# borangundogan/PPO-2DGrid

Measured on AMD Instinct MI355X. Metric: env-steps/sec (rollout+GAE+PPO update), 4096 envs, 16x16 mediumhard, higher is better.
Workload: dtype fp32

## Files before the change

include/merlin_hip.h:

```cpp
#ifndef MERLIN_HIP_H
#define MERLIN_HIP_H

#include <stdint.h>

#ifdef __cplusplus
extern "C" {
#endif

#define MERLIN_ABI_VERSION 3

#define MERLIN_OK 0
#define MERLIN_E_INVALID 1
#define MERLIN_E_HIP 2
#define MERLIN_E_DEVICE 3
#define MERLIN_E_UNSUPPORTED 4

#define MERLIN_EASY 0
#define MERLIN_MEDIUM 1
#define MERLIN_MEDIUMHARD 2
#define MERLIN_HARD 3
#define MERLIN_HARDEST 4

#define MERLIN_DEVERR_BAD_ACTION 1u
#define MERLIN_DEVERR_PLACE_OBJ 2u
#define MERLIN_DEVERR_SLOT_EMPTY 8u
#define MERLIN_DEVERR_BAD_TILE 4u
#define MERLIN_DEVERR_BAD_FRAME 16u

#define MERLIN_LAYOUT_NCHW 0
#define MERLIN_LAYOUT_NHWC 1

#define MERLIN_OBS_WORDS 8
#define MERLIN_OBS_TILES 5
#define MERLIN_TILE_PX 8
#define MERLIN_VIEW 7

typedef struct merlin_env merlin_env;

typedef struct {
    int32_t num_envs;
    int32_t size;
    int32_t difficulty;
    int32_t max_steps;
    int32_t stuck_penalty;
    int32_t max_stay;
    double penalty;
    int32_t exploration_bonus;
    double bonus;
    int32_t reseed_each_reset;
} merlin_env_config;

#define MERLIN_ENV_CONFIG_FIELDS 10
int64_t merlin_env_config_layout(int64_t *offsets_host, int32_t n_fields);

int merlin_version(void);
const char *merlin_last_error(void);
int merlin_tile_atlas(uint8_t *out_host);

int merlin_env_create(const merlin_env_config *cfg, merlin_env **out);
int merlin_env_destroy(merlin_env *env);
int merlin_env_seed(merlin_env *env, const uint64_t *seeds_host, int32_t n, void *stream);
int merlin_env_set_difficulties(merlin_env *env, const int32_t *diff_host, int32_t n, void *stream);
int merlin_env_reset(merlin_env *env, const uint8_t *mask_dev, uint32_t *obs_dev, void *stream);
int merlin_env_step(merlin_env *env, const int64_t *actions_dev, int32_t n_steps,
                    int64_t action_stride, uint32_t *obs_dev, float *reward_dev,
                    uint8_t *terminated_dev, uint8_t *truncated_dev, float *done_dev,
                    double *ep_return_dev, int32_t *ep_length_dev, int32_t autoreset,
                    void *stream);
int merlin_env_act_step(merlin_env *env, const float *head_part_dev, int32_t n_parts, const float *b_actor_dev,
                        const float *b_critic_dev, int32_t act_dim, int32_t deterministic, uint64_t seed,
                        const int64_t *epoch_dev, int64_t step, int64_t env_offset, int64_t *action_dev,
                        float *logp_dev, float *value_dev, uint32_t *obs_dev, float *reward_dev,
                        uint8_t *terminated_dev, uint8_t *truncated_dev, float *done_dev, double *ep_return_dev,
                        int32_t *ep_length_dev, void *stream);
int merlin_group_act(const uint32_t *codes_dev, int32_t groups, const float *T2_dev, const float *b2_dev,
                     const float *W3t_dev, const float *b3_dev, const float *W4p_dev, const float *b4_dev,
                     const float *Wa_dev, const float *ba_dev, const float *Wc_dev, const float *bc_dev,
                     int32_t act_dim, float *a3_ws_dev, float *head_part_dev, int32_t shared_weights, void *stream);
int merlin_env_set_refill_interval(merlin_env *env, int32_t every);
int merlin_env_refill(merlin_env *env, void *stream);
int merlin_env_set_step_fallback(merlin_env *env, int32_t on);
int merlin_env_set_lookahead_depth(merlin_env *env, int32_t depth);
int merlin_env_full_obs(merlin_env *env, uint8_t *out_dev, void *stream);
int merlin_env_get_state(merlin_env *env, uint32_t *walls_host, int32_t *agent_host,
                         uint64_t *rng_host, void *stream);
#define MERLIN_FRAME_TILES 22
int merlin_frame_atlas(int32_t tile_size, uint8_t *out_host);
int merlin_render_frames(const uint32_t *walls_dev, const int32_t *goal_dev, const int32_t *agent_dev,
                         const int32_t *map_index_dev, int64_t n_frames, int32_t size, int32_t tile_size,
                         int32_t highlight, uint8_t *out_dev, void *stream);
int merlin_env_render(merlin_env *env, const int64_t *index_dev, int64_t n, int32_t tile_size,
                      int32_t highlight, uint8_t *out_dev, void *stream);
int merlin_env_snapshot(merlin_env *env, uint32_t *walls_dev, int32_t *goal_dev, int32_t *agent_dev,
                        void *stream);
int merlin_shortest_paths(const uint32_t *walls_dev, const int32_t *goal_dev, const int32_t *agent_dev,
                          const int32_t *map_index_dev, int64_t n, int32_t size, int32_t *dist_dev,
                          int16_t *field_dev, void *stream);
int merlin_env_optimal_steps(merlin_env *env, int32_t *dist_dev, int16_t *field_dev, void *stream);
int merlin_shortest_paths_host(const uint32_t *walls, const int32_t *goal, const int32_t *agent, int64_t n,
                               int32_t size, int32_t *dist, int16_t *field);
int merlin_view_codes(const uint32_t *walls_dev, const int32_t *goal_dev, const int32_t *agent_dev,
                      const int32_t *map_index_dev, int64_t n, int32_t size, uint32_t *codes_dev, void *stream);
int merlin_policy_paths(const uint32_t *walls_dev, const int32_t *goal_dev, const int8_t *action_dev,
                        int64_t n_maps, int32_t size, int16_t *steps_dev, void *stream);
int merlin_policy_paths_host(const uint32_t *walls, const int32_t *goal, const int8_t *action, int64_t n_maps,
                             int32_t size, int16_t *steps);
int merlin_policy_chain(const uint32_t *walls_dev, const int32_t *goal_dev, const float *probs_dev, int64_t n_maps,
                        int32_t size, int32_t horizon, double gamma, double *success_dev, double *ret_dev,
                        double *steps_dev, double *disc_dev, void *stream);
int merlin_policy_occupancy(const uint32_t *walls_dev, const int32_t *goal_dev, const float *probs_dev,
                            const int32_t *agent_dev, int64_t n_maps, int32_t size, int32_t horizon,
                            double *visits_dev, double *hit_dev, void *stream);
int merlin_policy_chain_host(const uint32_t *walls, const int32_t *goal, const float *probs, int64_t n_maps,
                             int32_t size, int32_t horizon, double gamma, double *success, double *ret,
                             double *steps, double *disc);
int merlin_policy_occupancy_host(const uint32_t *walls, const int32_t *goal, const float *probs,
                                 const int32_t *agent, int64_t n_maps, int32_t size, int32_t horizon,
                                 double *visits, double *hit);
int merlin_env_errors(merlin_env *env, uint32_t *flags_host, uint32_t *fallbacks_host,
                      void *stream);
int merlin_env_num_envs(const merlin_env *env);
int merlin_env_size(const merlin_env *env);

int merlin_obs_expand_f32(const uint32_t *codes_dev, const int64_t *index_dev, int64_t n,
                          float *out_dev, float scale, int32_t layout, void *stream);
int merlin_obs_expand_u8(const uint32_t *codes_dev, const int64_t *index_dev, int64_t n,
                         uint8_t *out_dev, void *stream);

int merlin_gae(const float *reward_dev, const float *value_dev, const float *done_dev,
               const float *last_value_dev, float *adv_dev, float *ret_dev, int32_t T, int32_t N,
               double gamma, double lam, double *stats_dev, void *stream);
int merlin_adv_normalize(const float *adv_dev, int64_t n, const double *stats_dev, float *out_dev,
                         void *stream);

int merlin_conv1_lut_fwd(const uint32_t *codes_dev, const int64_t *index_dev, int64_t n,
                         const float *tables_dev, const float *bias_dev, int32_t towers,
                         float *out_dev, void *stream);
int merlin_conv1_lut_bwd(const uint32_t *codes_dev, const int64_t *index_dev, int64_t n,
                         const float *act_dev, const float *grad_dev, int32_t towers,
                         float *dtables_dev, float *dbias_dev, void *stream);

int merlin_tower_conv2_im2col_fwd(const uint32_t *codes_dev, const int64_t *index_dev, int64_t n,
                                  const float *tables_dev, const float *bias_dev, int32_t towers,
                                  float *A2_dev, void *stream);
int merlin_tower_conv2_im2col_bwd(const uint32_t *codes_dev, const int64_t *index_dev, int64_t n,
                                  const float *tables_dev, const float *bias_dev,
                                  const float *dA2_dev, int32_t towers, float *dtables_dev,
                                  float *dbias_dev, void *stream);
int merlin_tower_conv3_im2col_fwd(const float *Z2_dev, const float *b2_dev, int64_t n,
                                  int32_t towers, float *A3_dev, void *stream);
int merlin_tower_conv3_col2im_bwd(const float *dA3_dev, const float *Z2_dev, const float *b2_dev,
                                  int64_t n, int32_t towers, float *dZ2_dev, void *stream);
int merlin_tower_conv3_col2im_bwd_chunked(const float *dA3_dev, const float *Z2_dev,
                                          const float *b2_dev, int64_t n, int32_t towers,
                                          float *dZ2c_dev, uint32_t *absmax_dev, void *stream);

int merlin_tower_conv2_lut_rows(void);
int merlin_tower_conv2_lut_fwd(const uint32_t *codes_dev, const int64_t *index_dev, int64_t n,
                               const float *tables_dev, int32_t towers, float *Z2_dev,
                               void *stream);
int merlin_tower_conv2_lut_bwd(const uint32_t *codes_dev, int64_t n, const float *dZ2c_dev,
                               const uint32_t *absmax_dev, int32_t towers, float *dtables_dev,
                               void *stream);
int merlin_tower_conv2_lut_fwd_grouped(const uint32_t *codes_dev, int64_t n, int64_t group_frames,
                                       const float *tables_dev, int32_t towers, float *Z2_dev, void *stream);
int64_t merlin_tower_conv2_lut_slab_bytes(int32_t towers, int64_t group_frames);
int merlin_tower_conv2_lut_bwd_grouped(const uint32_t *codes_dev, int64_t group_frames, const float *dZ2c_dev,
                                       const uint32_t *absmax_dev, int32_t towers, float *dtables_dev,
                                       void *slabs_dev, void *stream);

int merlin_tower_window_lut(const int32_t *rows_dev, int64_t n_windows, const float *tables_dev,
                            int32_t towers, float *Z2w_dev, void *stream);
int merlin_minibatch_patch_maps(const int32_t *kid_dev, const int64_t *group_keys_dev, int64_t n_groups,
                                int64_t n_frames, const int64_t *group_offsets_dev, int32_t n_patches, int32_t *kmap_dev,
                                int32_t *rmap_dev, int32_t *rep_row_dev, void *stream);
int merlin_tower_window_lut_bias_relu(const int32_t *rows_dev, int64_t n_windows, const float *tables_dev,
                                      int32_t towers, const float *b2_dev, float *a2w_dev, void *stream);
int merlin_tower_window_conv3(const float *Q_dev, int64_t n_windows, const int32_t *wid_dev,
                              const int64_t *groups_dev, int64_t n, const float *b3_dev,
                              int32_t towers, float *Y3_dev, void *stream);
int64_t merlin_tower_all_windows(void);
int merlin_tower_codes_conv3(const uint32_t *codes_dev, int64_t n, const float *Qall_dev,
                             const float *b3_dev, int32_t towers, float *Y3_dev, void *stream);
int merlin_tower_codes_conv3_amax(const uint32_t *codes_dev, int64_t n, const float *Qall_dev,
                                  const float *b3_dev, int32_t towers, float *Y3_dev, uint32_t *amax_dev,
                                  void *stream);
int merlin_tower_errors(uint32_t *flags, void *stream);
int merlin_tower_window_conv3_bits(const float *Q_dev, int64_t n_windows, const int32_t *wid_dev,
                                   const int64_t *groups_dev, int64_t n, const float *b3_dev,
                                   int32_t towers, float *Y3_dev, uint64_t *relu_bits_dev, uint32_t *amax_dev,
                                   void *stream);
int merlin_tower_window_conv3_reuse(const float *Q_dev, int64_t n_windows, const int32_t *wid_dev,
                                    const int64_t *groups_dev, int64_t n, const float *b3_dev,
                                    int32_t towers, float *Y3_dev, uint64_t *relu_bits_dev, uint32_t *amax_dev,
                                    const int32_t *rep_row_dev, int32_t copy, void *stream);
int merlin_tower_window_conv3_planes(const float *Q_dev, int64_t nw, const int32_t *wid_dev, const int64_t *groups_dev,
                                     int64_t n, const float *b3_dev, int32_t towers, void *Y3_planes_dev,
                                     uint64_t *relu_bits_dev, const int32_t *rep_row_dev, uint32_t *colmax_ws_dev,
                                     uint32_t *bound_dev, void *stream);
int merlin_segment_sum(const float *src_dev, int64_t src_rows, const int32_t *idx_dev,
                       const int32_t *key_dev, int64_t nnz, const int32_t *slot_dev, int32_t sub,
                       int64_t item_len, const int32_t *fix_dev, int64_t n_fix, int32_t towers,
                       float *out_dev, int64_t out_rows, float *carry_dev, int32_t accumulate,
                       void *stream);
#define MERLIN_SEG_ACCUMULATE 1
#define MERLIN_SEG_NO_FILL 2
#define MERLIN_SEG_MASK_BITS 4
#define MERLIN_SEG_ROLE_SHIFT 8
#define MERLIN_SEG_ROLE_MASK (7 << MERLIN_SEG_ROLE_SHIFT)
int merlin_segment_sum_masked(const float *src_dev, const void *mask_dev, int64_t src_rows,
                              const int32_t *idx_dev, const int32_t *key_dev, int64_t nnz,
                              const int32_t *slot_dev, int32_t sub, int64_t item_len,
                              const int32_t *fix_dev, int64_t n_fix, int32_t towers, float *out_dev,
                              int64_t out_rows, float *carry_dev, int32_t flags, void *stream);
int merlin_segment_sum_marked(const float *src_dev, const void *mask_dev, int64_t src_rows,
                              const int32_t *idx_dev, const int32_t *key_dev, int64_t nnz,
                              const int32_t *slot_dev, int32_t sub, int64_t item_len,
                              const int32_t *fix_dev, int64_t n_fix, int32_t towers, float *out_dev,
                              int64_t out_rows, float *carry_dev, int32_t flags, int32_t *mark_dev,
                              void *stream);
int merlin_segment_sum_fused(const float *src_dev, const void *mask_dev, int64_t src_rows,
                             const int32_t *idx_dev, const int32_t *key_dev, int64_t nnz,
                             const int32_t *slot_dev, int32_t sub, int64_t item_len,
                             const int32_t *fix_dev, int64_t n_fix, int32_t towers, float *out_dev,
                             int64_t out_rows, float *carry_dev, int32_t flags, int32_t *mark_dev,
                             const int32_t *head_fix_dev, int32_t *counters_dev, void *stream);
int merlin_segment_sum_mask_rows(const float *src_dev, const void *mask_dev, int64_t src_rows, const int32_t *idx_dev,
                                 const int32_t *key_dev, int64_t nnz, const int32_t *slot_dev, int32_t sub,
                                 int64_t item_len, const int32_t *fix_dev, int64_t n_fix, int32_t towers, float *out_dev,
                                 int64_t out_rows, float *carry_dev, int32_t flags, int32_t *mark_dev,
                                 const int32_t *head_fix_dev, int32_t *counters_dev, const int32_t *mask_rows_dev,
                                 void *stream);

int merlin_act_heads(const float *z_dev, const float *b4_dev, int64_t n, int32_t hidden,
                     const float *w_actor_dev, const float *b_actor_dev, const float *w_critic_dev,
                     const float *b_critic_dev, int32_t act_dim, int32_t deterministic, uint64_t seed,
                     const int64_t *epoch_dev, int64_t step, int64_t env_offset, int64_t *action_dev,
                     float *logp_dev,
                     float *value_dev, void *stream);

int64_t merlin_ppo_loss_workspace(int64_t n_samples);
int merlin_ppo_loss(const float *logits_dev, const float *value_dev, const float *bias_actor_dev,
                    const float *bias_critic_dev, int64_t n_frames, int32_t act_dim, const int32_t *offs_dev,
                    const int32_t *order_dev, const int64_t *frame_of_dev, int64_t n_samples,
                    const int64_t *sample_index_dev, const int64_t *actions_dev, const float *logp_old_dev,
                    const float *adv_dev, const float *ret_dev, double clip_eps, double vf_coef, double ent_coef,
                    float *dlogits_dev, float *dvalue_dev, float *dbias_actor_dev, float *dbias_critic_dev,
                    float *loss_dev, double *stats_dev, double *workspace_dev, void *stream);
int merlin_ppo_loss_absmax(const float *logits_dev, const float *value_dev, const float *bias_actor_dev,
                           const float *bias_critic_dev, int64_t n_frames, int32_t act_dim, const int32_t *offs_dev,
                           const int32_t *order_dev, const int64_t *frame_of_dev, int64_t n_samples,
                           const int64_t *sample_index_dev, const int64_t *actions_dev, const float *logp_old_dev,
                           const float *adv_dev, const float *ret_dev, double clip_eps, double vf_coef,
                           double ent_coef, float *dlogits_dev, float *dvalue_dev, float *dbias_actor_dev,
                           float *dbias_critic_dev, float *loss_dev, double *stats_dev, double *workspace_dev,
                           uint32_t *grad_absmax_dev, void *stream);

int merlin_tower_bias_relu(float *z_dev, const float *bias_dev, int64_t rows, int32_t cols, int32_t towers,
                           void *stream);
int merlin_tower_relu_bwd(const float *y_dev, const float *dy_dev, float *dz_dev, int64_t rows, int32_t cols,
                          int32_t towers, float *dbias_dev, void *stream);
int merlin_tower_colsum(const float *x_dev, int64_t rows, int32_t cols, int64_t row_stride, int64_t tower_stride,
                        int32_t towers, float *out_dev, void *stream);
int merlin_tower_head_bwd(const float *h_dev, const float *dlogits_dev, const float *dvalue_dev,
                          const float *w_actor_dev, const float *w_critic_dev, int64_t n, int32_t hidden,
                          int32_t act_dim, float *dz_dev, float *dbias_dev, float *dw_actor_dev,
                          float *dw_critic_dev, uint32_t *amax_dev, void *stream);
int merlin_tower_head_bwd_planes(const float *h_dev, const float *dlogits_dev, const float *dvalue_dev,
                                 const float *w_actor_dev, const float *w_critic_dev, int64_t n, int32_t hidden,
                                 int32_t act_dim, void *dz_planes_dev, float *dbias_dev, float *dw_actor_dev,
                                 float *dw_critic_dev, const uint32_t *grad_absmax_dev, uint32_t *dz_bound_dev,
                                 void *stream);
int merlin_tower_heads_fwd(const float *h_dev, int64_t n, int32_t hidden, const float *w_actor_dev,
                           int32_t act_dim, const float *w_critic_dev, const float *b_actor_dev,
                           const float *b_critic_dev, float *logits_dev, float *value_dev, void *stream);

int merlin_x6_split(const float *x_dev, int64_t n, void *planes_dev, void *stream);
int merlin_x6_join(const void *planes_dev, int64_t n, float *x_dev, void *stream);
int merlin_x6_gemm_nt(const float *A_dev, const void *B_dev, int64_t M, int32_t N, int32_t K, int32_t towers,
                      int64_t a_stride, int64_t b_stride, const float *bias_dev, float *C_dev, int64_t c_stride,
                      int32_t cfg, void *stream);
int64_t merlin_x6_tn_slab_floats(int32_t M, int32_t N, int32_t towers, int32_t splits);
int merlin_x6_gemm_tn(const float *A_dev, const float *B_dev, int64_t Kd, int32_t M, int32_t N, int32_t towers,
                      int64_t a_stride, int64_t b_stride, int32_t splits, float *slab_dev, float *out_dev, int32_t cfg,
                      void *stream);

int merlin_h3_amax(const float *x_dev, int64_t n, int32_t towers, int64_t stride, uint32_t *amax_dev, void *stream);
int merlin_h3_split(const float *x_dev, int64_t n, int32_t towers, const uint32_t *amax_dev, void *planes_dev,
                    void *stream);
int merlin_h3_gemm_nt(const float *A_dev, const uint32_t *amax_a_dev, const void *B_dev, const uint32_t *amax_b_dev,
                      int64_t M, int32_t N, int32_t K, int32_t towers, int64_t a_stride, int64_t b_stride,
                      const float *bias_dev, float *C_dev, int64_t c_stride, void *a_planes_dev, int32_t cfg,
                      void *stream);
int merlin_h3_gemm_tn(const float *A_dev, const uint32_t *amax_a_dev, const float *B_dev, const uint32_t *amax_b_dev,
                      int64_t Kd, int32_t M, int32_t N, int32_t towers, int64_t a_stride, int64_t b_stride,
                      int32_t splits, float *slab_dev, float *out_dev, int32_t cfg, void *stream);
int merlin_h3_gemm_tn_planes(const void *A_planes_dev, const uint32_t *amax_a_dev, const void *B_planes_dev,
                             const uint32_t *amax_b_dev, int64_t Kd, int32_t M, int32_t N, int32_t towers,
                             int64_t a_stride, int64_t b_stride, int32_t splits, float *slab_dev, float *out_dev,
                             int32_t cfg, void *stream);
int merlin_h3_gemm_nt_gather(const float *A_dev, const uint32_t *amax_a_dev, const void *B_dev,
                             const uint32_t *amax_b_dev, int64_t M, int32_t N, int32_t K, int32_t towers,
                             int64_t a_stride, int64_t b_stride, const float *bias_dev, float *C_dev, int64_t c_stride,
                             const int32_t *a_rows_dev, int32_t cfg, void *stream);
int merlin_h3_gemm_nt_heads(const float *A_dev, const uint32_t *amax_a_dev, const void *B_dev,
                            const uint32_t *amax_b_dev, int64_t M, int32_t N, int32_t K, int64_t a_stride,
                            int64_t b_stride, const float *bias_dev, float *C_dev, int64_t c_stride,
                            const int32_t *a_rows_dev, const float *head_w0_dev, int32_t n_actions,
                            const float *head_w1_dev, float *head_partials_dev, int32_t cfg, void *stream);
int32_t merlin_h3_heads_parts(int32_t N, int32_t cfg);
int merlin_h3_walk_blocks(int32_t blocks);
int merlin_h3_gemm_nt_planes(const void *A_planes_dev, const uint32_t *amax_a_dev, const void *B_dev,
                             const uint32_t *amax_b_dev, int64_t M, int32_t N, int32_t K, int32_t towers,
                             int64_t a_stride, int64_t b_stride, const float *bias_dev, float *C_dev, int64_t c_stride,
                             int32_t cfg, void *stream);
int merlin_h3_gemm_nt_heads_planes(const void *A_planes_dev, const uint32_t *amax_a_dev, const void *B_dev,
                                   const uint32_t *amax_b_dev, int64_t M, int32_t N, int32_t K, int64_t a_stride,
                                   int64_t b_stride, const float *bias_dev, float *C_dev, int64_t c_stride,
                                   const int32_t *a_rows_dev, const float *head_w0_dev, int32_t n_actions,
                                   const float *head_w1_dev, float *head_partials_dev, int32_t cfg, void *stream);
int merlin_h3_gemm_tn_gather_planes(const void *A_planes_dev, const uint32_t *amax_a_dev, const void *B_planes_dev,
                                    const uint32_t *amax_b_dev, int64_t Kd, int32_t M, int32_t N, int32_t towers,
                                    int64_t a_stride, int64_t b_stride, int32_t splits, float *slab_dev,
                                    float *out_dev, const int32_t *b_rows_dev, int32_t cfg, void *stream);
int merlin_h3_gemm_tn_gather_planes_a(const void *A_planes_dev, const uint32_t *amax_a_dev, const float *B_dev,
                                      const uint32_t *amax_b_dev, int64_t Kd, int32_t M, int32_t N, int32_t towers,
                                      int64_t a_stride, int64_t b_stride, int32_t splits, float *slab_dev,
                                      float *out_dev, const int32_t *b_rows_dev, int32_t cfg, void *stream);
// ... 73 lines not shown
```

ppo-2dgrid_amd/csrc/merlin_capi.hip:

```cpp
#include <math.h>
#include <string.h>

#include <mutex>
#include <string>
#include <vector>

#include <algorithm>

#include "merlin_internal.h"

struct merlin_env {
    merlin::EnvDev dev;
    int device;
    bool has_state;
    int steps_since_refill;
    int refill_every;
    bool no_fallback = false;
    bool seed_slots_full = false;
    uint8_t *diff_buf = nullptr;
    int32_t *level_log = nullptr;
};

namespace {

// ... 928 lines not shown
    return MERLIN_OK;
}

int merlin_gae(const float *rew, const float *val, const float *done, const float *last, float *adv,
               float *ret, int32_t T, int32_t N, double gamma, double lam, double *stats, void *stream) {
    if (!rew || !val || !done || !last || !adv || !ret) return fail(MERLIN_E_INVALID, "null argument");
    if (T <= 0 || N <= 0) return fail(MERLIN_E_INVALID, "T and N must be > 0");
    DeviceWs *ws = nullptr;
    int rc = device_ws(&ws);
    if (rc) return rc;
    if (stats && merlin::gae_partials_needed(T, N) > ws->max_partials)
        return fail(MERLIN_E_UNSUPPORTED, "too many envs for the GAE stats workspace");
    HIP_TRY(merlin::launch_gae(rew, val, done, last, adv, ret, T, N, gamma, lam, stats, ws->partials,
                               ws->max_partials, (hipStream_t)stream));
    return MERLIN_OK;
}

int merlin_adv_normalize(const float *adv, int64_t n, const double *stats, float *out, void *stream) {
    if (!adv || !stats || !out) return fail(MERLIN_E_INVALID, "null argument");
    HIP_TRY(merlin::launch_adv_normalize(adv, n, stats, out, (hipStream_t)stream));
    return MERLIN_OK;
}

int merlin_conv1_lut_fwd(const uint32_t *codes, const int64_t *index, int64_t n, const float *tables,
                         const float *bias, int32_t towers, float *out, void *stream) {
    if ((!codes || !tables || !bias || !out) && n > 0) return fail(MERLIN_E_INVALID, "null argument");
    if (towers < 1 || towers > 2) return fail(MERLIN_E_INVALID, "towers must be 1 or 2");
    HIP_TRY(merlin::launch_conv1_lut_fwd(codes, index, n, tables, bias, towers, out, (hipStream_t)stream));
    return MERLIN_OK;
}

int merlin_conv1_lut_bwd(const uint32_t *codes, const int64_t *index, int64_t n, const float *act,
                         const float *grad, int32_t towers, float *dtables, float *dbias, void *stream) {
    if (!dtables || !dbias || ((!codes || !act || !grad) && n > 0)) return fail(MERLIN_E_INVALID, "null argument");
    if (towers < 1 || towers > 2) return fail(MERLIN_E_INVALID, "towers must be 1 or 2");
    DeviceWs *ws = nullptr;
    int rc = device_ws(&ws);
    if (rc) return rc;
    HIP_TRY(merlin::launch_conv1_lut_bwd(codes, index, n, act, grad, towers, dtables, dbias, ws->conv1_slabs,
                                         ws->max_slabs, (hipStream_t)stream));
    return MERLIN_OK;
}

int merlin_tower_conv2_im2col_fwd(const uint32_t *codes, const int64_t *index, int64_t n, const float *tables,
                                  const float *bias, int32_t towers, float *A2, void *stream) {
    if ((!codes || !tables || !bias || !A2) && n > 0) return fail(MERLIN_E_INVALID, "null argument");
    if (towers < 1 || towers > 2) return fail(MERLIN_E_INVALID, "towers must be 1 or 2");
    HIP_TRY(merlin::launch_conv1_im2col_fwd(codes, index, n, tables, bias, towers, A2, (hipStream_t)stream));
    return MERLIN_OK;
}

int merlin_tower_conv2_im2col_bwd(const uint32_t *codes, const int64_t *index, int64_t n, const float *tables,
                                  const float *bias, const float *dA2, int32_t towers, float *dtables,
                                  float *dbias, void *stream) {
    if (!dtables || !dbias || ((!codes || !tables || !bias || !dA2) && n > 0))
        return fail(MERLIN_E_INVALID, "null argument");
    if (towers < 1 || towers > 2) return fail(MERLIN_E_INVALID, "towers must be 1 or 2");
    DeviceWs *ws = nullptr;
    int rc = device_ws(&ws);
    if (rc) return rc;
    HIP_TRY(merlin::launch_conv1_im2col_bwd(codes, index, n, tables, bias, dA2, towers, dtables, dbias,
                                            ws->conv1_slabs, ws->max_slabs, (hipStream_t)stream));
    return MERLIN_OK;
}

int merlin_tower_conv3_im2col_fwd(const float *Z2, const float *b2, int64_t n, int32_t towers, float *A3,
                                  void *stream) {
    if ((!Z2 || !b2 || !A3) && n > 0) return fail(MERLIN_E_INVALID, "null argument");
    HIP_TRY(merlin::launch_im2col3_fwd(Z2, b2, n, towers, A3, (hipStream_t)stream));
    return MERLIN_OK;
}

int merlin_tower_conv3_col2im_bwd(const float *dA3, const float *Z2, const float *b2, int64_t n, int32_t towers,
                                  float *dZ2, void *stream) {
    if ((!dA3 || !Z2 || !b2 || !dZ2) && n > 0) return fail(MERLIN_E_INVALID, "null argument");
    HIP_TRY(merlin::launch_col2im3_bwd(dA3, Z2, b2, n, towers, 0, dZ2, nullptr, (hipStream_t)stream));
    return MERLIN_OK;
}

int merlin_tower_conv3_col2im_bwd_chunked(const float *dA3, const float *Z2, const float *b2, int64_t n,
                                          int32_t towers, float *dZ2c, uint32_t *absmax, void *stream) {
    if (!absmax || ((!dA3 || !Z2 || !b2 || !dZ2c) && n > 0)) return fail(MERLIN_E_INVALID, "null argument");
    if (towers < 1) return fail(MERLIN_E_INVALID, "towers must be >= 1");
    HIP_TRY(merlin::launch_col2im3_bwd(dA3, Z2, b2, n, towers, 1, dZ2c, absmax, (hipStream_t)stream));
    return MERLIN_OK;
}

int merlin_tower_conv2_lut_rows(void) { return merlin::conv2_lut_rows(); }

int merlin_tower_conv2_lut_fwd(const uint32_t *codes, const int64_t *index, int64_t n, const float *tables,
                               int32_t towers, float *Z2, void *stream) {
    if ((!codes || !tables || !Z2) && n > 0) return fail(MERLIN_E_INVALID, "null argument");
    if (towers < 1 || towers > 2) return fail(MERLIN_E_INVALID, "towers must be 1 or 2");
    HIP_TRY(merlin::launch_conv2_lut_fwd(codes, index, n, tables, towers, Z2, (hipStream_t)stream));
    return MERLIN_OK;
}

int merlin_tower_conv2_lut_bwd(const uint32_t *codes, int64_t n, const float *dZ2c, const uint32_t *absmax,
                               int32_t towers, float *dtables, void *stream) {
    if (!dtables || ((!codes || !dZ2c || !absmax) && n > 0)) return fail(MERLIN_E_INVALID, "null argument");
    if (towers < 1 || towers > 2) return fail(MERLIN_E_INVALID, "towers must be 1 or 2");
    DeviceWs *ws = nullptr;
    int rc = device_ws(&ws);
    if (rc) return rc;
    HIP_TRY(merlin::launch_conv2_lut_bwd(codes, n, dZ2c, absmax, towers, dtables, ws->lut2_slabs,
                                         (hipStream_t)stream));
    return MERLIN_OK;
}

int merlin_tower_conv2_lut_fwd_grouped(const uint32_t *codes, int64_t n, int64_t group_frames, const float *tables,
                                       int32_t towers, float *Z2, void *stream) {
    if ((!codes || !tables || !Z2) && n > 0) return fail(MERLIN_E_INVALID, "null argument");
    if (towers < 2 || towers % 2 || group_frames <= 0) return fail(MERLIN_E_INVALID, "bad grouping");
    if (n != (int64_t)(towers / 2) * group_frames) return fail(MERLIN_E_INVALID, "n != groups * group_frames");
    HIP_TRY(merlin::launch_conv2_lut_fwd(codes, nullptr, n, tables, towers, Z2, (hipStream_t)stream, group_frames));
    return MERLIN_OK;
}

int64_t merlin_tower_conv2_lut_slab_bytes(int32_t towers, int64_t group_frames) {
    return (int64_t)merlin::conv2_lut_slab_bytes(towers, merlin::conv2_lut_fblocks(group_frames));
}

int merlin_tower_conv2_lut_bwd_grouped(const uint32_t *codes, int64_t group_frames, const float *dZ2c,
                                       const uint32_t *absmax, int32_t towers, float *dtables, void *slabs,
                                       void *stream) {
    if (!dtables || ((!codes || !dZ2c || !absmax || !slabs) && group_frames > 0))
        return fail(MERLIN_E_INVALID, "null argument");
    if (towers < 2 || towers % 2) return fail(MERLIN_E_INVALID, "bad grouping");
    HIP_TRY(merlin::launch_conv2_lut_bwd(codes, group_frames, dZ2c, absmax, towers, dtables, slabs,
                                         (hipStream_t)stream, group_frames));
    return MERLIN_OK;
}

int merlin_tower_window_lut(const int32_t *rows, int64_t nw, const float *tables, int32_t towers, float *Z2w,
                            void *stream) {
    if ((!rows || !tables || !Z2w) && nw > 0) return fail(MERLIN_E_INVALID, "null argument");
    if (towers < 1 || towers > 2) return fail(MERLIN_E_INVALID, "towers must be 1 or 2");
    HIP_TRY(merlin::launch_window_lut(rows, nw, tables, towers, Z2w, (hipStream_t)stream));
    return MERLIN_OK;
}

int merlin_minibatch_patch_maps(const int32_t *kid, const int64_t *group_keys, int64_t n_groups, int64_t n_frames,
                                const int64_t *group_offsets, int32_t n_patches, int32_t *kmap, int32_t *rmap,
                                int32_t *rep_row, void *stream) {
    if (n_groups < 0 || n_frames < 1 || n_patches < 1) return fail(MERLIN_E_INVALID, "bad shape");
    if (n_groups > 0 && (!kid || !group_keys || !group_offsets || !kmap || !rmap || !rep_row))
        return fail(MERLIN_E_INVALID, "null argument");
    if (n_groups * 9 > INT32_MAX) return fail(MERLIN_E_UNSUPPORTED, "more than 2^31 rows");
    HIP_TRY(merlin::launch_patch_maps(kid, group_keys, n_groups, n_frames, group_offsets, n_patches, kmap, rmap,
                                      rep_row, (hipStream_t)stream));
    return MERLIN_OK;
}

int merlin_tower_window_lut_bias_relu(const int32_t *rows, int64_t nw, const float *tables, int32_t towers,
                                      const float *b2, float *a2w, void *stream) {
    if ((!rows || !tables || !a2w || !b2) && nw > 0) return fail(MERLIN_E_INVALID, "null argument");
    if (towers < 1 || towers > 2) return fail(MERLIN_E_INVALID, "towers must be 1 or 2");
    HIP_TRY(merlin::launch_window_lut(rows, nw, tables, towers, a2w, (hipStream_t)stream, b2));
    return MERLIN_OK;
}

int merlin_tower_window_conv3(const float *Q, int64_t nw, const int32_t *wid, const int64_t *groups, int64_t n,
                              const float *b3, int32_t towers, float *Y3, void *stream) {
    if ((!Q || !wid || !b3 || !Y3) && n > 0) return fail(MERLIN_E_INVALID, "null argument");
    if (towers < 1 || towers > 2) return fail(MERLIN_E_INVALID, "towers must be 1 or 2");
    HIP_TRY(merlin::launch_window_conv3(Q, nw, wid, groups, n, b3, towers, Y3, nullptr, nullptr, nullptr, 0,
                                        (hipStream_t)stream));
    return MERLIN_OK;
}

int merlin_tower_window_conv3_bits(const float *Q, int64_t nw, const int32_t *wid, const int64_t *groups, int64_t n,
                                   const float *b3, int32_t towers, float *Y3, uint64_t *relu_bits, uint32_t *amax,
                                   void *stream) {
    if ((!Q || !wid || !b3 || !Y3 || !relu_bits) && n > 0) return fail(MERLIN_E_INVALID, "null argument");
    if (towers < 1 || towers > 2) return fail(MERLIN_E_INVALID, "towers must be 1 or 2");
    HIP_TRY(merlin::launch_window_conv3(Q, nw, wid, groups, n, b3, towers, Y3, relu_bits, amax, nullptr, 0,
                                        (hipStream_t)stream));
    return MERLIN_OK;
}

int merlin_tower_window_conv3_reuse(const float *Q, int64_t nw, const int32_t *wid, const int64_t *groups, int64_t n,
                                    const float *b3, int32_t towers, float *Y3, uint64_t *relu_bits, uint32_t *amax,
                                    const int32_t *rep_row, int32_t copy, void *stream) {
    if ((!rep_row || !Y3 || (!(copy & 4) && (!Q || !wid || !b3))) && n > 0)
        return fail(MERLIN_E_INVALID, "null argument");
    if (towers < 1 || towers > 2) return fail(MERLIN_E_INVALID, "towers must be 1 or 2");
    if (copy < 0 || copy > 7) return fail(MERLIN_E_INVALID, "copy must be 0..7");
    HIP_TRY(merlin::launch_window_conv3(Q, nw, wid, groups, n, b3, towers, Y3, relu_bits, amax, rep_row, copy,
                                        (hipStream_t)stream));
    return MERLIN_OK;
}

int merlin_tower_window_conv3_planes(const float *Q, int64_t nw, const int32_t *wid, const int64_t *groups, int64_t n,
                                     const float *b3, int32_t towers, void *Y3_planes, uint64_t *relu_bits,
                                     const int32_t *rep_row, uint32_t *colmax_ws, uint32_t *bound, void *stream) {
    if ((!rep_row || !Y3_planes || !Q || !wid || !b3 || !relu_bits || !colmax_ws || !bound) && n > 0)
        return fail(MERLIN_E_INVALID, "null argument");
    if (towers < 1 || towers > 2) return fail(MERLIN_E_INVALID, "towers must be 1 or 2");
    if (n > 0 && nw <= 0) return fail(MERLIN_E_INVALID, "no windows");
    HIP_TRY(merlin::launch_window_conv3(Q, nw, wid, groups, n, b3, towers, static_cast<float *>(Y3_planes), relu_bits,
                                        nullptr, rep_row, 0, (hipStream_t)stream, colmax_ws, bound));
    return MERLIN_OK;
}

int64_t merlin_tower_all_windows(void) { return 458752; }

int merlin_tower_codes_conv3_amax(const uint32_t *codes, int64_t n, const float *Qall, const float *b3,
                                  int32_t towers, float *Y3, uint32_t *amax, void *stream) {
    if ((!codes || !Qall || !b3 || !Y3) && n > 0) return fail(MERLIN_E_INVALID, "null argument");
    if (towers < 1 || towers > 2) return fail(MERLIN_E_INVALID, "towers must be 1 or 2");
    DeviceWs *ws = nullptr;
    if (int r = device_ws(&ws)) return r;
    HIP_TRY(merlin::launch_codes_conv3(codes, n, Qall, b3, towers, Y3, amax, ws->tower_err, (hipStream_t)stream));
    return MERLIN_OK;
}

int merlin_tower_errors(uint32_t *flags, void *stream) {
    DeviceWs *ws = nullptr;
    if (int r = device_ws(&ws)) return r;
    hipStream_t s = (hipStream_t)stream;
    uint32_t h = 0;
    HIP_TRY(hipMemcpyAsync(&h, ws->tower_err, sizeof(h), hipMemcpyDeviceToHost, s));
    HIP_TRY(hipStreamSynchronize(s));
    HIP_TRY(merlin::zero_async(ws->tower_err, sizeof(h), s));
    if (flags) *flags = h;
    return MERLIN_OK;
}

int merlin_tower_codes_conv3(const uint32_t *codes, int64_t n, const float *Qall, const float *b3, int32_t towers,
                             float *Y3, void *stream) {
    return merlin_tower_codes_conv3_amax(codes, n, Qall, b3, towers, Y3, nullptr, stream);
}

static int segment_sum_fused(const float *src, const void *mask, int64_t src_rows, const int32_t *idx,
                             const int32_t *key, int64_t nnz, const int32_t *slot, int32_t sub, int64_t item_len,
                             const int32_t *fix, int64_t n_fix, int32_t towers, float *out, int64_t out_rows,
                             float *carry, int32_t flags, int32_t *mark, const int32_t *head_fix, int32_t *counters,
                             const int32_t *mask_rows, void *stream) {
    if (!out && out_rows > 0) return fail(MERLIN_E_INVALID, "null output");
    if (nnz > 0 && (!src || !idx || !key || !carry)) return fail(MERLIN_E_INVALID, "null argument");
    if (n_fix > 0 && !fix) return fail(MERLIN_E_INVALID, "null fix-up list");
    if ((head_fix == nullptr) != (counters == nullptr)) return fail(MERLIN_E_INVALID, "head_fix and counters go together");
    if (counters && nnz > 0 && n_fix != (nnz + item_len - 1) / item_len)
        return fail(MERLIN_E_INVALID, "in-launch fix-ups need one fix row per item");
    if (towers < 1 || towers > 2) return fail(MERLIN_E_INVALID, "towers must be 1 or 2");
    if (item_len <= 0 || sub <= 0) return fail(MERLIN_E_INVALID, "item_len and sub must be > 0");
    if (flags & ~(MERLIN_SEG_ACCUMULATE | MERLIN_SEG_NO_FILL | MERLIN_SEG_MASK_BITS | MERLIN_SEG_ROLE_MASK))
        return fail(MERLIN_E_INVALID, "unknown flags");
    HIP_TRY(merlin::launch_seg_sum(src, mask, (flags & MERLIN_SEG_MASK_BITS) ? 1 : 0, src_rows, idx, key, nnz, slot,
                                   sub, item_len, fix, n_fix, towers, out, out_rows, carry,
                                   (flags & MERLIN_SEG_ACCUMULATE) ? 1 : 0, (flags & MERLIN_SEG_NO_FILL) ? 0 : 1,
                                   (flags & MERLIN_SEG_ROLE_MASK) >> MERLIN_SEG_ROLE_SHIFT, mark, head_fix, counters,
                                   (hipStream_t)stream, mask_rows));
    return MERLIN_OK;
}

int merlin_segment_sum_fused(const float *src, const void *mask, int64_t src_rows, const int32_t *idx,
                             const int32_t *key, int64_t nnz, const int32_t *slot, int32_t sub, int64_t item_len,
                             const int32_t *fix, int64_t n_fix, int32_t towers, float *out, int64_t out_rows,
                             float *carry, int32_t flags, int32_t *mark, const int32_t *head_fix, int32_t *counters,
                             void *stream) {
    return segment_sum_fused(src, mask, src_rows, idx, key, nnz, slot, sub, item_len, fix, n_fix, towers, out,
                             out_rows, carry, flags, mark, head_fix, counters, nullptr, stream);
}

int merlin_segment_sum_mask_rows(const float *src, const void *mask, int64_t src_rows, const int32_t *idx,
                                 const int32_t *key, int64_t nnz, const int32_t *slot, int32_t sub, int64_t item_len,
                                 const int32_t *fix, int64_t n_fix, int32_t towers, float *out, int64_t out_rows,
                                 float *carry, int32_t flags, int32_t *mark, const int32_t *head_fix,
                                 int32_t *counters, const int32_t *mask_rows, void *stream) {
    if (nnz > 0 && (!mask || !mask_rows || !(flags & MERLIN_SEG_MASK_BITS)))
        return fail(MERLIN_E_INVALID, "mask_rows needs MERLIN_SEG_MASK_BITS words");
    return segment_sum_fused(src, mask, src_rows, idx, key, nnz, slot, sub, item_len, fix, n_fix, towers, out,
                             out_rows, carry, flags, mark, head_fix, counters, mask_rows, stream);
}

int merlin_segment_sum_marked(const float *src, const void *mask, int64_t src_rows, const int32_t *idx,
                              const int32_t *key, int64_t nnz, const int32_t *slot, int32_t sub, int64_t item_len,
                              const int32_t *fix, int64_t n_fix, int32_t towers, float *out, int64_t out_rows,
                              float *carry, int32_t flags, int32_t *mark, void *stream) {
    return merlin_segment_sum_fused(src, mask, src_rows, idx, key, nnz, slot, sub, item_len, fix, n_fix, towers, out,
                                    out_rows, carry, flags, mark, nullptr, nullptr, stream);
}

int merlin_segment_sum_masked(const float *src, const void *mask, int64_t src_rows, const int32_t *idx,
                              const int32_t *key, int64_t nnz, const int32_t *slot, int32_t sub, int64_t item_len,
                              const int32_t *fix, int64_t n_fix, int32_t towers, float *out, int64_t out_rows,
                              float *carry, int32_t flags, void *stream) {
    return merlin_segment_sum_marked(src, mask, src_rows, idx, key, nnz, slot, sub, item_len, fix, n_fix, towers, out,
                                     out_rows, carry, flags, nullptr, stream);
}

int merlin_segment_sum(const float *src, int64_t src_rows, const int32_t *idx, const int32_t *key, int64_t nnz,
                       const int32_t *slot, int32_t sub, int64_t item_len, const int32_t *fix, int64_t n_fix,
                       int32_t towers, float *out, int64_t out_rows, float *carry, int32_t accumulate,
                       void *stream) {
    return merlin_segment_sum_masked(src, nullptr, src_rows, idx, key, nnz, slot, sub, item_len, fix, n_fix, towers,
                                     out, out_rows, carry, accumulate ? MERLIN_SEG_ACCUMULATE : 0, stream);
}

int merlin_act_heads(const float *z, const float *b4, int64_t n, int32_t hidden, const float *w_actor,
                     const float *b_actor, const float *w_critic, const float *b_critic, int32_t act_dim,
                     int32_t deterministic, uint64_t seed, const int64_t *epoch, int64_t step, int64_t env_offset,
                     int64_t *action, float *logp, float *value, void *stream) {
    if (n < 0) return fail(MERLIN_E_INVALID, "negative size");
    if (act_dim < 1 || act_dim > 8) return fail(MERLIN_E_INVALID, "act_dim must be in [1, 8]");
// ... 540 lines not shown
```

ppo-2dgrid_amd/csrc/merlin_internal.h:

```cpp
#pragma once

#include <hip/hip_runtime.h>
#include <stdint.h>

#include "merlin_hip.h"

namespace merlin {

struct EnvDev {
    int n, size, sp, difficulty, max_steps;
    int stuck_on, max_stay;
    double penalty;
    int explore_on;
    double bonus;
    int reseed;
    uint32_t *walls;
    uint4 *agent;
    ulonglong2 *rng_s;
    ulonglong2 *rng_i;
    uint2 *rng_b;
    double *ep_ret;
    int32_t *ep_len;
    uint32_t *visited;
    uint32_t *err;
// ... 179 lines not shown
        ty = ay - 3;
    } else {
        tx = ax - 3;
        ty = ay - 6;
    }
    const uint64_t hi_ones = ~0ULL << (S + 8);
    uint32_t win[7];
#pragma unroll
    for (int r = 0; r < 7; r++) {
        const int y = ty + r;
        const bool in = (y >= 0) && (y < S);
        const uint32_t bits = in ? row(in ? y : 0) : 0xffffffffu;
        const uint64_t w = ((uint64_t)bits << 8) | 0xffULL | hi_ones;
        win[r] = (uint32_t)(w >> (tx + 8)) & 0x7fu;
    }
    uint32_t tr[7];
#pragma unroll
    for (int x = 0; x < 7; x++) {
        uint32_t v = 0u;
#pragma unroll
        for (int y = 0; y < 7; y++) v |= ((win[y] >> x) & 1u) << y;
        tr[x] = v;
    }
    const int k = (dir + 1) & 3;
    const bool odd = k & 1, flip = (k == 1) || (k == 2), rev = (k >= 2);
#pragma unroll
    for (int b = 0; b < 7; b++) {
        uint32_t t = flip ? (odd ? tr[6 - b] : win[6 - b]) : (odd ? tr[b] : win[b]);
        V[b] = rev ? bitrev7(t) : t;
    }
#pragma unroll
    for (int j = 0; j < 7; j++) m[j] = 0u;
    m[6] = 1u << 3;
#pragma unroll
    for (int j = 6; j >= 0; j--) {
        const uint32_t T = ~V[j] & 0x7fu;
        uint32_t M = m[j];
#pragma unroll
        for (int s = 0; s < 6; s++) M |= (M & T & 0x3fu) << 1;
        const uint32_t e1 = M & T & 0x3fu;
#pragma unroll
        for (int s = 0; s < 6; s++) M |= (M & T & 0x7eu) >> 1;
        const uint32_t e2 = M & T & 0x7eu;
        m[j] = M;
        if (j > 0) m[j - 1] |= e1 | (e1 << 1) | e2 | (e2 >> 1);
    }
}

struct StepOut {
    const int64_t *actions;
    int64_t action_stride;
    int n_steps;
    int autoreset;
    uint32_t *obs;
    float *reward;
    uint8_t *term;
    uint8_t *trunc;
    float *done;
    double *ep_ret_out;
    int32_t *ep_len_out;
    ActIn act;
    int no_fallback;
    int32_t *level_log;
};

hipError_t zero_async(void *p, size_t bytes, hipStream_t s);
hipError_t launch_group_act(const uint32_t *codes, int G, const float *T2, const float *b2, const float *W3t,
                            const float *b3, const float *W4p, const float *b4, const float *Wa, const float *ba,
                            const float *Wc, const float *bc, int A, float *a3, float *part, bool shared, hipStream_t s);
hipError_t launch_h3p_gemm_nt(const void *A, const uint32_t *amaxA, const void *B, const uint32_t *amaxB, int64_t M,
                              int N, int K, int T, int64_t a_stride, int64_t b_stride, const float *bias, float *C,
                              int64_t c_stride, int cfg, hipStream_t s, const int32_t *a_rows = nullptr,
                              const float *head_w0 = nullptr, int n_actions = 0, const float *head_w1 = nullptr,
                              float *head_part = nullptr);
void set_h3p_walk_blocks(int n);
hipError_t launch_h3p_gemm_tn_gather(const void *A, const uint32_t *amaxA, const void *B, const uint32_t *amaxB,
                                     int64_t Kd, int M, int N, int T, int64_t a_stride, int64_t b_stride, int splits,
                                     float *slab, const int32_t *b_rows, int cfg, int *S_out, hipStream_t s);
hipError_t launch_env_reset(const EnvDev &E, const uint8_t *mask, uint32_t *obs, bool refill, hipStream_t s);
hipError_t launch_env_step(const EnvDev &E, const StepOut &O, bool refill, hipStream_t s);
hipError_t launch_env_full_obs(const EnvDev &E, uint8_t *out, hipStream_t s);
hipError_t launch_env_refill(const EnvDev &E, bool full, hipStream_t s);
hipError_t launch_level_bind(const EnvDev &E, const uint32_t *walls, const int32_t *goal, const int32_t *agent,
                             hipStream_t s);
hipError_t launch_env_levels(const EnvDev &E, int32_t *cur, uint32_t *count, hipStream_t s);
hipError_t launch_level_scores(const float *adv, const int32_t *level, int T, int N, int L, int kind, int64_t *sum,
                               int64_t *count, int accumulate, hipStream_t s);
void level_scores_host(const float *adv, const int32_t *level, int T, int N, int L, int kind, int64_t *sum,
                       int64_t *count, int accumulate);
hipError_t upload_atlas(const uint8_t *atlas_host);
hipError_t launch_render_frames(const uint32_t *walls, const int32_t *goal, const int32_t *agent,
                                const int32_t *map_index, int64_t n_frames, int size, int ts, int highlight,
                                const uint8_t *atlas, uint8_t *out, uint32_t *err, hipStream_t s);
hipError_t launch_env_render(const EnvDev &E, const int64_t *index, int64_t n_frames, int ts, int highlight,
                             const uint8_t *atlas, uint8_t *out, hipStream_t s);
hipError_t launch_env_snapshot(const EnvDev &E, uint32_t *walls, int32_t *goal, int32_t *agent, hipStream_t s);
hipError_t launch_shortest_paths(const uint32_t *walls, const int32_t *goal, const int32_t *agent,
                                 const int32_t *map_index, int64_t n, int size, int32_t *dist, int16_t *field,
                                 hipStream_t s);
hipError_t launch_env_optimal_steps(const EnvDev &E, int32_t *dist, int16_t *field, hipStream_t s);
void shortest_paths_host(const uint32_t *walls, const int32_t *goal, const int32_t *agent, int64_t n, int S,
                         int32_t *dist, int16_t *field);
hipError_t launch_view_codes(const uint32_t *walls, const int32_t *goal, const int32_t *agent,
                             const int32_t *map_index, int64_t n, int size, uint32_t *codes, uint32_t *err,
                             hipStream_t s);
hipError_t launch_policy_paths(const uint32_t *walls, const int32_t *goal, const int8_t *action, int64_t n_maps,
                               int size, int16_t *steps, hipStream_t s);
void policy_paths_host(const uint32_t *walls, const int32_t *goal, const int8_t *action, int64_t n_maps, int S,
                       int16_t *steps);
hipError_t launch_policy_chain(const uint32_t *walls, const int32_t *goal, const float *probs, int64_t n_maps, int size,
                               int horizon, double gamma, double *success, double *ret, double *steps, double *disc,
                               hipStream_t s);
hipError_t launch_policy_occupancy(const uint32_t *walls, const int32_t *goal, const float *probs,
                                   const int32_t *agent, int64_t n_maps, int size, int horizon, double *visits,
                                   double *hit, uint32_t *err, hipStream_t s);
void policy_chain_host(const uint32_t *walls, const int32_t *goal, const float *probs, int64_t n_maps, int S, int T,
                       double gamma, double *success, double *ret, double *steps, double *disc);
void policy_occupancy_host(const uint32_t *walls, const int32_t *goal, const float *probs, const int32_t *agent,
                           int64_t n_maps, int S, int T, double *visits, double *hit);
hipError_t launch_obs_expand_f32(const uint32_t *codes, const int64_t *index, int64_t n, float *out,
                                 float scale, int layout, hipStream_t s);
hipError_t launch_obs_expand_u8(const uint32_t *codes, const int64_t *index, int64_t n, uint8_t *out,
                                hipStream_t s);
hipError_t launch_gae(const float *rew, const float *val, const float *done, const float *last,
                      float *adv, float *ret, int T, int N, double gamma, double lam, double *stats,
                      double *partials, int max_partials, hipStream_t s);
hipError_t launch_adv_normalize(const float *adv, int64_t n, const double *stats, float *out,
                                hipStream_t s);
int gae_partials_needed(int T, int N);
int conv1_slab_floats(int towers);
hipError_t launch_conv1_lut_fwd(const uint32_t *codes, const int64_t *index, int64_t n, const float *tables,
                                const float *bias, int towers, float *out, hipStream_t s);
hipError_t launch_conv1_lut_bwd(const uint32_t *codes, const int64_t *index, int64_t n, const float *act,
                                const float *grad, int towers, float *dtables, float *dbias, float *slabs,
                                int max_slabs, hipStream_t s);
hipError_t launch_conv1_im2col_fwd(const uint32_t *codes, const int64_t *index, int64_t n, const float *tables,
                                   const float *bias, int T, float *A2, hipStream_t s);
hipError_t launch_conv1_im2col_bwd(const uint32_t *codes, const int64_t *index, int64_t n, const float *tables,
                                   const float *bias, const float *dA2, int T, float *dtables, float *dbias,
                                   float *slabs, int max_slabs, hipStream_t s);
hipError_t launch_im2col3_fwd(const float *Z2, const float *b2, int64_t n, int T, float *A3, hipStream_t s);
hipError_t launch_col2im3_bwd(const float *dA3, const float *Z2, const float *b2, int64_t n, int T, int chunked,
                              float *dZ2, uint32_t *absmax, hipStream_t s);
int conv2_lut_rows();
int conv2_lut_fblocks(int64_t n);
size_t conv2_lut_slab_bytes(int towers, int fblocks);
hipError_t launch_conv2_lut_fwd(const uint32_t *codes, const int64_t *index, int64_t n, const float *tables,
                                int towers, float *Z2, hipStream_t s, int64_t gstride = 0);
hipError_t launch_conv2_lut_bwd(const uint32_t *codes, int64_t n, const float *dZ2c, const uint32_t *absmax,
                                int towers, float *dT, void *slabs, hipStream_t s, int64_t gstride = 0);

hipError_t launch_patch_maps(const int32_t *kid, const int64_t *gkey, int64_t G, int64_t F, const int64_t *goff, int K,
                             int32_t *kmap, int32_t *rmap, int32_t *rep_row, hipStream_t s);
hipError_t launch_window_lut(const int32_t *rows, int64_t nw, const float *tab, int T, float *Z2w, hipStream_t s,
                             const float *b2 = nullptr);
hipError_t launch_window_conv3(const float *Q, int64_t nw, const int32_t *wid, const int64_t *groups, int64_t n,
                               const float *b3, int T, float *Y3, uint64_t *bits, uint32_t *amax,
                               const int32_t *rrow, int copy, hipStream_t s, uint32_t *colmax = nullptr,
                               uint32_t *bound = nullptr);
hipError_t launch_act_heads(const float *z, const float *b4, int64_t n, int H, const float *wa, const float *ba,
                            const float *wc, const float *bc, int A, int det, uint64_t seed, const int64_t *epoch,
                            int64_t step, int64_t env_offset, int64_t *action, float *logp, float *value,
                            hipStream_t s);
hipError_t launch_act_draw(const float *part, int P, int64_t n, const float *ba, const float *bc, int A, int det,
                           uint64_t seed, const int64_t *epoch, int64_t step, int64_t env_offset, int64_t *action,
                           float *logp, float *value, hipStream_t s);
int64_t ppo_loss_workspace_doubles(int64_t n_samples);
hipError_t launch_ppo_loss(const float *logits, const float *value, const float *bias_a, const float *bias_c,
                           int64_t U, int A, const int32_t *offs, const int32_t *order, const int64_t *inv, int64_t n,
                           const int64_t *sample_index, const int64_t *actions, const float *lp_old, const float *adv,
                           const float *ret, double clip_eps, double vf_coef, double ent_coef, float *dlogits,
                           float *dvalue, float *dbias_a, float *dbias_c, float *loss, double *stats,
                           double *workspace, hipStream_t s, uint32_t *dmax = nullptr);
hipError_t launch_codes_conv3(const uint32_t *codes, int64_t n, const float *Q, const float *b3, int T, float *Y3,
                              uint32_t *amax, uint32_t *err, hipStream_t s);
hipError_t launch_x6_gemm_nt32(const float *A, const void *B, int64_t M, int N, int K, int T, int64_t a_stride,
                               int64_t b_stride, const float *bias, float *C, int64_t c_stride, int cfg, hipStream_t s);
hipError_t launch_x6_gemm_tn32(const float *A, const float *B, int64_t Kd, int M, int N, int T, int64_t a_stride,
                               int64_t b_stride, int splits, float *slab, int cfg, hipStream_t s, int *S_out);
hipError_t launch_stage_fwd(const float *W1, const float *b1, const float *W2, const float *atlas, const int16_t *idx,
                            int T, float *HT, float *T2, hipStream_t s);
hipError_t launch_stage_bwd(const float *W2, const float *HT, const float *dT2, const float *atlas,
                            const int16_t *koff, const int16_t *kv, int T, float *dH, float *dW1, float *db1,
                            float *dW2, double *ws, hipStream_t s);
hipError_t launch_stage_fwd_planes(const float *W1, const float *b1, const float *W2, const float *atlas,
                                   const int16_t *idx, int T, float *HT, float *T2, const float *x0, const float *x1,
                                   int64_t n, const uint32_t *amax, void *planes0, void *planes1, hipStream_t s);
hipError_t launch_stage_bwd_scatter(const float *W2, const float *HT, const float *dT2, const float *atlas,
                                    const int16_t *koff, const int16_t *kv, int T, float *dH, float *DG, int64_t w1,
                                    int64_t b1, int64_t w2, const int32_t *map, int64_t n, float *flat, double *ws,
                                    hipStream_t s);
hipError_t launch_stage_gather(const float *src, const int32_t *map, int64_t n, float *dst, hipStream_t s);
int64_t winbwd_work_floats(int T, int64_t nw);
hipError_t launch_winbwd(const float *a2w, const float *dQ, const float *W3r, int T, int64_t nw, float *da2w,
                         float *db2, float *dW3r, float *work, hipStream_t s, float *db3 = nullptr);
hipError_t launch_winfwd(const float *a2w, const float *W3r, int T, int64_t nw, float *Q, hipStream_t s);
constexpr size_t STAGE_WS_DOUBLES = 2 * 4 * 10 * 2048;
hipError_t launch_heads_fwd(const float *h, int64_t n, int H, const float *wa, int A, const float *wc, const float *ba,
                            const float *bc, float *logits, float *value, hipStream_t s);
hipError_t launch_seg_sum(const float *src, const void *mask, int mask_bits, int64_t src_rows, const int32_t *idx,
                          const int32_t *key, int64_t nnz, const int32_t *slot, int S, int64_t L, const int32_t *fix,
                          int64_t nfix, int T, float *out, int64_t out_rows, float *carry, int acc_out, int fill, int role,
                          int32_t *mark, const int32_t *hfix, int32_t *cnt, hipStream_t s,
                          const int32_t *mrow = nullptr);

constexpr int EPI_MAX_BLOCKS = 512;
size_t epilogue_work_floats();
bool epilogue_cols_ok(int cols);
int epilogue_max_act();
hipError_t launch_bias_relu(float *Z, const float *b, int64_t rows, int cols, int T, hipStream_t s);
hipError_t launch_relu_bwd_colsum(const float *Y, const float *dY, float *dZ, int64_t rows, int cols, int T,
                                  float *dbias, float *work, hipStream_t s);
hipError_t launch_colsum(const float *X, int64_t rows, int cols, int64_t row_stride, int64_t tower_stride, int T,
                         float *out, float *work, hipStream_t s);
hipError_t launch_head_bwd(const float *h, const float *dlogits, const float *dvalue, const float *wa,
                           const float *wc, int64_t n, int H, int A, float *dz, float *db4, float *dwa, float *dwc,
                           float *work, uint32_t *amax, hipStream_t s, const uint32_t *dmax = nullptr,
                           void *dz_planes = nullptr);

__device__ __forceinline__ void block_amax2(const uint32_t mx[2], int T, uint32_t *amax) {
    __shared__ uint32_t red[2][4];
    uint32_t m0 = mx[0], m1 = mx[1];
    for (int o = 32; o > 0; o >>= 1) {
        m0 = max(m0, (uint32_t)__shfl_xor((int)m0, o));
        m1 = max(m1, (uint32_t)__shfl_xor((int)m1, o));
    }
    if ((threadIdx.x & 63) == 0) {
        red[0][threadIdx.x >> 6] = m0;
        red[1][threadIdx.x >> 6] = m1;
    }
    __syncthreads();
    if (threadIdx.x < (unsigned)T) {
        const uint32_t *r = red[threadIdx.x];
        const uint32_t m = max(max(r[0], r[1]), max(r[2], r[3]));
        if (m && m > __hip_atomic_load(amax + threadIdx.x, __ATOMIC_RELAXED, __HIP_MEMORY_SCOPE_AGENT))
            atomicMax(amax + threadIdx.x, m);
    }
}

constexpr float H3_LO_SCALE = 2048.0f, H3_LO_INV = 1.0f / H3_LO_SCALE;
__device__ __forceinline__ int h3_exp(uint32_t amax) {
    if (amax == 0u) return 0;
    const int e = (int)((amax >> 23) & 0xffu) - 127;
    return min(max(14 - e, -120), 115);
}
__device__ __forceinline__ float pow2f(int e) { return __uint_as_float((uint32_t)(e + 127) << 23); }
__device__ __forceinline__ uint32_t load_amax(const uint32_t *p) {
    return __hip_atomic_load(p, __ATOMIC_RELAXED, __HIP_MEMORY_SCOPE_AGENT);
}
__device__ __forceinline__ int xcd_tile(int b, int nb) {
    const int xcd = b & 7, q = nb >> 3, r = nb & 7;
    return (xcd < r ? xcd * (q + 1) : r * (q + 1) + (xcd - r) * q) + (b >> 3);
}

__device__ __forceinline__ void h3_pair(float a, float b, float sc, float sc2, uint32_t &hi, uint32_t &lo) {
    const float m2048 = -H3_LO_SCALE, za = a * sc2, zb = b * sc2;
    uint32_t h, l;
    asm("v_fma_mixlo_f16 %0, %1, %2, 0" : "=v"(h) : "v"(a), "v"(sc));
    asm("v_fma_mixhi_f16 %0, %1, %2, 0" : "+v"(h) : "v"(b), "v"(sc));
    asm("v_fma_mixlo_f16 %0, %1, %2, %3 op_sel_hi:[1,0,0]" : "=v"(l) : "v"(h), "v"(m2048), "v"(za));
    asm("v_fma_mixhi_f16 %0, %1, %2, %3 op_sel:[1,0,0] op_sel_hi:[1,0,0]" : "+v"(l) : "v"(h), "v"(m2048), "v"(zb));
    hi = h;
    lo = l;
}

__device__ __forceinline__ void h3_store4(uint2 *__restrict__ row, int q, const float4 v, float sc, float sc2) {
    uint32_t h0, h1, l0, l1;
    h3_pair(v.x, v.y, sc, sc2, h0, l0);
    h3_pair(v.z, v.w, sc, sc2, h1, l1);
    const int o = 4 * (q >> 1) + (q & 1);
    row[o] = make_uint2(h0, h1);
    row[o + 2] = make_uint2(l0, l1);
}

__device__ __forceinline__ void h3_store4_pair(uint4 *__restrict__ row, int q, const float4 v, float sc, float sc2) {
    uint32_t h0, h1, l0, l1;
    h3_pair(v.x, v.y, sc, sc2, h0, l0);
    h3_pair(v.z, v.w, sc, sc2, h1, l1);
    const bool odd = q & 1;
    const uint32_t r0 = (uint32_t)__shfl_xor((int)(odd ? h0 : l0), 1);
    const uint32_t r1 = (uint32_t)__shfl_xor((int)(odd ? h1 : l1), 1);
    row[q] = odd ? make_uint4(r0, r1, l0, l1) : make_uint4(h0, h1, r0, r1);
}

hipError_t launch_x6_split(const float *x, int64_t n, void *planes, hipStream_t s);
hipError_t launch_x6_join(const void *planes, int64_t n, float *x, hipStream_t s);
hipError_t launch_x6_gemm_nt(const float *A, const void *B, int64_t M, int N, int K, int T, int64_t a_stride,
                             int64_t b_stride, const float *bias, float *C, int64_t c_stride, int cfg, hipStream_t s);
hipError_t launch_x6_gemm_tn(const float *A, const float *B, int64_t Kd, int M, int N, int T, int64_t a_stride,
                             int64_t b_stride, int splits, float *slab, float *out, int cfg, hipStream_t s);
int x6_tn_max_splits();
hipError_t launch_x6_fold(const float *slab, int S, int64_t total, float *out, hipStream_t s);
hipError_t launch_h3_amax(const float *x, int64_t n, int T, int64_t stride, uint32_t *amax, hipStream_t s);
hipError_t launch_h3_split(const float *x, int64_t n, int T, const uint32_t *amax, void *planes, hipStream_t s);
hipError_t launch_h3_gemm_nt(const float *A, const uint32_t *amaxA, const void *B, const uint32_t *amaxB, int64_t M,
                             int N, int K, int T, int64_t a_stride, int64_t b_stride, const float *bias, float *C,
                             int64_t c_stride, void *a_planes, int cfg, hipStream_t s,
                             const int32_t *a_rows = nullptr, const float *head_w0 = nullptr, int n_actions = 0,
                             const float *head_w1 = nullptr, float *head_part = nullptr, bool a_is_planes = false);
int h3_heads_parts(int N, int cfg);
hipError_t launch_heads_combine(const float *part, int P, int64_t M, int na, float *logits, float *value,
                                hipStream_t s);
hipError_t launch_h3_gemm_tn(const void *A, const uint32_t *amaxA, const void *B, const uint32_t *amaxB, int64_t Kd,
                             int M, int N, int T, int64_t a_stride, int64_t b_stride, int splits, float *slab,
                             float *out, bool planes, int cfg, hipStream_t s, const int32_t *b_rows = nullptr,
                             bool a_planes = false, bool b_planes = false);
// ... 33 lines not shown
```

ppo-2dgrid_amd/merlin/_native.py:

```python
from __future__ import annotations

import contextlib
import ctypes as C
import gc
import os

import torch

PKG_ROOT = os.path.dirname(os.path.dirname(os.path.abspath(__file__)))
LIB_PATH = os.environ.get("MERLIN_HIP_LIB", os.path.join(PKG_ROOT, "lib", "libmerlin_hip.so"))

MERLIN_OK = 0
E_INVALID, E_HIP, E_DEVICE, E_UNSUPPORTED = 1, 2, 3, 4
LAYOUT_NCHW = 0
LAYOUT_NHWC = 1
OBS_WORDS = 8
DEVERR_BAD_ACTION = 1
DEVERR_PLACE_OBJ = 2
DEVERR_BAD_TILE = 4
DEVERR_SLOT_EMPTY = 8
DEVERR_BAD_FRAME = 16
FRAME_TILES = 22

DIFFICULTY_IDS = {"easy": 0, "medium": 1, "mediumhard": 2, "hard": 3, "hardest": 4}


class MerlinNativeError(RuntimeError):
    code = None


class EnvConfig(C.Structure):
    _fields_ = [
        ("num_envs", C.c_int32),
        ("size", C.c_int32),
        ("difficulty", C.c_int32),
        ("max_steps", C.c_int32),
        ("stuck_penalty", C.c_int32),
        ("max_stay", C.c_int32),
        ("penalty", C.c_double),
        ("exploration_bonus", C.c_int32),
        ("bonus", C.c_double),
        ("reseed_each_reset", C.c_int32),
    ]


_lib = None
ABI_VERSION = 3


def lib():
    global _lib
    if _lib is not None:
        return _lib
    if not os.path.exists(LIB_PATH):
        raise MerlinNativeError(
            f"HIP library not found at {LIB_PATH}; build it with "
            f"`make -C {PKG_ROOT}` (hipcc --offload-arch=gfx950)")
    try:
        L = C.CDLL(LIB_PATH)
    except OSError as e:
        raise MerlinNativeError(f"failed to load {LIB_PATH}: {e}") from e
    vp, i32, i64, u64p = C.c_void_p, C.c_int32, C.c_int64, C.POINTER(C.c_uint64)
    L.merlin_version.restype = C.c_int
    if L.merlin_version() != ABI_VERSION:
        raise MerlinNativeError(f"{LIB_PATH} has ABI version {L.merlin_version()}, this package binds version "
                                f"{ABI_VERSION} (include/merlin_hip.h MERLIN_ABI_VERSION); rebuild it")
    L.merlin_last_error.restype = C.c_char_p
    L.merlin_tile_atlas.argtypes = [vp]
    L.merlin_env_config_layout.argtypes = [C.POINTER(C.c_int64), i32]
    L.merlin_env_config_layout.restype = i64
    L.merlin_env_create.argtypes = [C.POINTER(EnvConfig), C.POINTER(vp)]
    L.merlin_env_destroy.argtypes = [vp]
    L.merlin_env_seed.argtypes = [vp, u64p, i32, vp]
    L.merlin_env_set_difficulties.argtypes = [vp, C.POINTER(C.c_int32), i32, vp]
    L.merlin_env_reset.argtypes = [vp, vp, vp, vp]
    L.merlin_env_step.argtypes = [vp, vp, i32, i64, vp, vp, vp, vp, vp, vp, vp, i32, vp]
    L.merlin_group_act.argtypes = [vp, i32, vp, vp, vp, vp, vp, vp, vp, vp, vp, vp, i32, vp, vp, i32, vp]
    L.merlin_env_act_step.argtypes = [vp, vp, i32, vp, vp, i32, i32, C.c_uint64, vp, i64, i64, vp, vp, vp, vp, vp,
                                      vp, vp, vp, vp, vp, vp]
    L.merlin_env_set_refill_interval.argtypes = [vp, i32]
    L.merlin_env_set_step_fallback.argtypes = [vp, i32]
    L.merlin_env_refill.argtypes = [vp, vp]
    L.merlin_env_set_lookahead_depth.argtypes = [vp, i32]
    L.merlin_env_get_state.argtypes = [vp, vp, vp, vp, vp]
    L.merlin_env_full_obs.argtypes = [vp, vp, vp]
    L.merlin_env_errors.argtypes = [vp, C.POINTER(C.c_uint32), C.POINTER(C.c_uint32), vp]
    L.merlin_obs_expand_f32.argtypes = [vp, vp, i64, vp, C.c_float, i32, vp]
    L.merlin_obs_expand_u8.argtypes = [vp, vp, i64, vp, vp]
    L.merlin_gae.argtypes = [vp, vp, vp, vp, vp, vp, i32, i32, C.c_double, C.c_double, vp, vp]
    L.merlin_adv_normalize.argtypes = [vp, i64, vp, vp, vp]
    L.merlin_conv1_lut_fwd.argtypes = [vp, vp, i64, vp, vp, i32, vp, vp]
    L.merlin_conv1_lut_bwd.argtypes = [vp, vp, i64, vp, vp, i32, vp, vp, vp]
    L.merlin_tower_conv2_im2col_fwd.argtypes = [vp, vp, i64, vp, vp, i32, vp, vp]
    L.merlin_tower_conv2_im2col_bwd.argtypes = [vp, vp, i64, vp, vp, vp, i32, vp, vp, vp]
    L.merlin_tower_conv3_im2col_fwd.argtypes = [vp, vp, i64, i32, vp, vp]
    L.merlin_tower_conv3_col2im_bwd.argtypes = [vp, vp, vp, i64, i32, vp, vp]
    L.merlin_tower_conv3_col2im_bwd_chunked.argtypes = [vp, vp, vp, i64, i32, vp, vp, vp]
    L.merlin_tower_conv2_lut_rows.restype = C.c_int
    L.merlin_tower_conv2_lut_fwd.argtypes = [vp, vp, i64, vp, i32, vp, vp]
    L.merlin_tower_conv2_lut_bwd.argtypes = [vp, i64, vp, vp, i32, vp, vp]
    L.merlin_tower_conv2_lut_fwd_grouped.argtypes = [vp, i64, i64, vp, i32, vp, vp]
    L.merlin_tower_conv2_lut_slab_bytes.argtypes = [i32, i64]
    L.merlin_tower_conv2_lut_slab_bytes.restype = i64
    L.merlin_tower_conv2_lut_bwd_grouped.argtypes = [vp, i64, vp, vp, i32, vp, vp, vp]
    L.merlin_tower_window_lut.argtypes = [vp, i64, vp, i32, vp, vp]
    L.merlin_tower_window_conv3.argtypes = [vp, i64, vp, vp, i64, vp, i32, vp, vp]
    L.merlin_tower_window_lut_bias_relu.argtypes = [vp, i64, vp, i32, vp, vp, vp]
    L.merlin_minibatch_patch_maps.argtypes = [vp, vp, i64, i64, vp, i32, vp, vp, vp, vp]
    L.merlin_tower_window_conv3_bits.argtypes = [vp, i64, vp, vp, i64, vp, i32, vp, vp, vp, vp]
    L.merlin_tower_window_conv3_reuse.argtypes = [vp, i64, vp, vp, i64, vp, i32, vp, vp, vp, vp, i32, vp]
    L.merlin_tower_all_windows.restype = i64
    L.merlin_tower_codes_conv3.argtypes = [vp, i64, vp, vp, i32, vp, vp]
    L.merlin_tower_codes_conv3_amax.argtypes = [vp, i64, vp, vp, i32, vp, vp, vp]
    L.merlin_tower_errors.argtypes = [C.POINTER(C.c_uint32), vp]
    L.merlin_segment_sum.argtypes = [vp, i64, vp, vp, i64, vp, i32, i64, vp, i64, i32, vp, i64, vp, i32, vp]
    L.merlin_segment_sum_masked.argtypes = [vp, vp, i64, vp, vp, i64, vp, i32, i64, vp, i64, i32, vp, i64, vp, i32,
                                            vp]
    L.merlin_tower_heads_fwd.argtypes = [vp, i64, i32, vp, i32, vp, vp, vp, vp, vp, vp]
    L.merlin_segment_sum_marked.argtypes = [vp, vp, i64, vp, vp, i64, vp, i32, i64, vp, i64, i32, vp, i64, vp, i32,
                                            vp, vp]
    L.merlin_segment_sum_fused.argtypes = [vp, vp, i64, vp, vp, i64, vp, i32, i64, vp, i64, i32, vp, i64, vp, i32,
                                           vp, vp, vp, vp]
    L.merlin_segment_sum_mask_rows.argtypes = [vp, vp, i64, vp, vp, i64, vp, i32, i64, vp, i64, i32, vp, i64, vp, i32,
                                               vp, vp, vp, vp, vp]
    L.merlin_tower_bias_relu.argtypes = [vp, vp, i64, i32, i32, vp]
    L.merlin_tower_relu_bwd.argtypes = [vp, vp, vp, i64, i32, i32, vp, vp]
    L.merlin_tower_colsum.argtypes = [vp, i64, i32, i64, i64, i32, vp, vp]
    L.merlin_tower_head_bwd.argtypes = [vp, vp, vp, vp, vp, i64, i32, i32, vp, vp, vp, vp, vp, vp]
    L.merlin_tower_head_bwd_planes.argtypes = [vp, vp, vp, vp, vp, i64, i32, i32, vp, vp, vp, vp, vp, vp, vp]
    L.merlin_act_heads.argtypes = [vp, vp, i64, i32, vp, vp, vp, vp, i32, i32, C.c_uint64, vp, i64, i64, vp, vp, vp,
                                   vp]
    L.merlin_ppo_loss_workspace.argtypes = [i64]
    L.merlin_ppo_loss_workspace.restype = i64
    L.merlin_clip_adam_workspace.argtypes = [i32, vp]
    L.merlin_clip_adam_workspace.restype = i64
    L.merlin_clip_adam.argtypes = [i32, vp, vp, vp, vp, vp, vp, C.c_double, C.c_double, C.c_double, C.c_double, C.c_float,
                                   vp, vp, vp]
    L.merlin_ppo_loss.argtypes = [vp, vp, vp, vp, i64, i32, vp, vp, vp, i64, vp, vp, vp, vp, vp, C.c_double,
                                  C.c_double, C.c_double, vp, vp, vp, vp, vp, vp, vp, vp]
    L.merlin_ppo_loss_absmax.argtypes = [vp, vp, vp, vp, i64, i32, vp, vp, vp, i64, vp, vp, vp, vp, vp, C.c_double,
                                         C.c_double, C.c_double, vp, vp, vp, vp, vp, vp, vp, vp, vp]
    L.merlin_x6_split.argtypes = [vp, i64, vp, vp]
    L.merlin_x6_join.argtypes = [vp, i64, vp, vp]
    L.merlin_x6_gemm_nt.argtypes = [vp, vp, i64, i32, i32, i32, i64, i64, vp, vp, i64, i32, vp]
    L.merlin_x6_tn_slab_floats.argtypes = [i32, i32, i32, i32]
    L.merlin_x6_tn_slab_floats.restype = i64
    L.merlin_x6_gemm_tn.argtypes = [vp, vp, i64, i32, i32, i32, i64, i64, i32, vp, vp, i32, vp]
    L.merlin_h3_amax.argtypes = [vp, i64, i32, i64, vp, vp]
    L.merlin_h3_split.argtypes = [vp, i64, i32, vp, vp, vp]
    L.merlin_h3_gemm_nt.argtypes = [vp, vp, vp, vp, i64, i32, i32, i32, i64, i64, vp, vp, i64, vp, i32, vp]
    L.merlin_h3_gemm_tn.argtypes = [vp, vp, vp, vp, i64, i32, i32, i32, i64, i64, i32, vp, vp, i32, vp]
    L.merlin_h3_gemm_tn_planes.argtypes = [vp, vp, vp, vp, i64, i32, i32, i32, i64, i64, i32, vp, vp, i32, vp]
    L.merlin_h3_gemm_nt_gather.argtypes = [vp, vp, vp, vp, i64, i32, i32, i32, i64, i64, vp, vp, i64, vp, i32, vp]
    L.merlin_h3_gemm_tn_gather.argtypes = [vp, vp, vp, vp, i64, i32, i32, i32, i64, i64, i32, vp, vp, vp, i32, vp]
    L.merlin_h3_gemm_tn_gather_planes_a.argtypes = [vp, vp, vp, vp, i64, i32, i32, i32, i64, i64, i32, vp, vp, vp, i32,
                                                    vp]
    L.merlin_h3_gemm_nt_planes.argtypes = [vp, vp, vp, vp, i64, i32, i32, i32, i64, i64, vp, vp, i64, i32, vp]
    L.merlin_h3_gemm_nt_heads_planes.argtypes = [vp, vp, vp, vp, i64, i32, i32, i64, i64, vp, vp, i64, vp, vp, i32,
                                                 vp, vp, i32, vp]
    L.merlin_h3_gemm_tn_gather_planes.argtypes = [vp, vp, vp, vp, i64, i32, i32, i32, i64, i64, i32, vp, vp, vp, i32,
                                                  vp]
    L.merlin_tower_window_conv3_planes.argtypes = [vp, i64, vp, vp, i64, vp, i32, vp, vp, vp, vp, vp, vp]
    L.merlin_h3_gemm_nt_heads.argtypes = [vp, vp, vp, vp, i64, i32, i32, i64, i64, vp, vp, i64, vp, vp, i32, vp, vp,
                                          i32, vp]
    L.merlin_h3_heads_parts.argtypes = [i32, i32]
    L.merlin_h3_heads_parts.restype = i32
    L.merlin_heads_combine.argtypes = [vp, i32, i64, i32, vp, vp, vp]
    L.merlin_act_draw.argtypes = [vp, i32, i64, vp, vp, i32, i32, C.c_uint64, vp, i64, i64, vp, vp, vp, vp]
    L.merlin_stage_tables_fwd.argtypes = [vp, vp, vp, vp, vp, i32, vp, vp, vp]
    L.merlin_stage_tables_bwd.argtypes = [vp, vp, vp, vp, vp, vp, i32, vp, vp, vp, vp, vp]
    L.merlin_stage_fwd_planes.argtypes = [vp, vp, vp, vp, vp, i32, vp, vp, vp, vp, i64, vp, vp, vp, vp]
    L.merlin_stage_bwd_scatter.argtypes = [vp, vp, vp, vp, vp, vp, i32, vp, vp, i64, i64, i64, vp, i64, vp, vp]
    L.merlin_gather_f32.argtypes = [vp, vp, i64, vp, vp]
    L.merlin_clip_adam_chain.argtypes = [i32, vp, vp, vp, vp, vp, vp, C.c_double, C.c_double, C.c_double, C.c_double,
                                         C.c_float, vp, vp, vp, i32, vp, i32, vp, i64, vp, vp, vp, vp, vp, vp]
    L.merlin_window_gemm_fwd.argtypes = [vp, vp, i32, i64, vp, vp]
    L.merlin_window_gemm_bwd_work.argtypes = [i32, i64]
    L.merlin_window_gemm_bwd_work.restype = i64
    L.merlin_window_gemm_bwd.argtypes = [vp, vp, vp, i32, i64, vp, vp, vp, vp, vp, i64, vp]
    L.merlin_group_clip_sgd_workspace.argtypes = [i32, vp, i32]
    L.merlin_group_clip_sgd_workspace.restype = i64
    L.merlin_group_clip_sgd.argtypes = [i32, vp, vp, vp, i32, C.c_float, C.c_float, vp, vp, vp]
    L.merlin_episode_loss.argtypes = [vp, vp, vp, vp, vp, i32, i32, C.c_double, C.c_double, vp, vp, vp]
    L.merlin_episode_class_stats.argtypes = [vp, vp, vp, vp, i32, i32, i32, vp, i32, vp]
    L.merlin_frame_atlas.argtypes = [i32, vp]
    L.merlin_render_frames.argtypes = [vp, vp, vp, vp, i64, i32, i32, i32, vp, vp]
    L.merlin_env_render.argtypes = [vp, vp, i64, i32, i32, vp, vp]
    L.merlin_env_snapshot.argtypes = [vp, vp, vp, vp, vp]
    L.merlin_shortest_paths.argtypes = [vp, vp, vp, vp, i64, i32, vp, vp, vp]
    L.merlin_env_optimal_steps.argtypes = [vp, vp, vp, vp]
    L.merlin_shortest_paths_host.argtypes = [vp, vp, vp, i64, i32, vp, vp]
    L.merlin_view_codes.argtypes = [vp, vp, vp, vp, i64, i32, vp, vp]
    L.merlin_policy_paths.argtypes = [vp, vp, vp, i64, i32, vp, vp]
    L.merlin_policy_paths_host.argtypes = [vp, vp, vp, i64, i32, vp]
    L.merlin_policy_chain.argtypes = [vp, vp, vp, i64, i32, i32, C.c_double, vp, vp, vp, vp, vp]
    L.merlin_policy_chain_host.argtypes = [vp, vp, vp, i64, i32, i32, C.c_double, vp, vp, vp, vp]
    L.merlin_policy_occupancy.argtypes = [vp, vp, vp, vp, i64, i32, i32, vp, vp, vp]
    L.merlin_policy_occupancy_host.argtypes = [vp, vp, vp, vp, i64, i32, i32, vp, vp]
    L.merlin_env_set_levels.argtypes = [vp, vp, vp, vp, i64, C.c_uint64, i64, vp]
    L.merlin_env_set_level_cdf.argtypes = [vp, vp, vp]
    L.merlin_env_levels.argtypes = [vp, vp, vp, vp]
    L.merlin_env_set_level_log.argtypes = [vp, vp]
    L.merlin_level_draw_host.argtypes = [C.c_uint64, i64, i64, i64, i64, vp, i64, vp]
    L.merlin_level_scores.argtypes = [vp, vp, i32, i32, i64, i32, vp, vp, i32, vp]
    L.merlin_level_scores_host.argtypes = [vp, vp, i32, i32, i64, i32, vp, vp, i32]
    check_env_config_layout(L)
    _lib = L
    return L


def env_config_layout(L=None):
    L = L or lib()
    nf = len(EnvConfig._fields_)
    offs = (C.c_int64 * nf)()
    size = int(L.merlin_env_config_layout(offs, nf))
    return size, [int(o) for o in offs]


def check_env_config_layout(L) -> None:
    size, offs = env_config_layout(L)
    mine = [getattr(EnvConfig, f).offset for f, _ in EnvConfig._fields_]
    if size != C.sizeof(EnvConfig) or offs != mine:
        raise MerlinNativeError(f"EnvConfig layout mismatch: C sizeof {size} offsets {offs}, "
                                f"ctypes sizeof {C.sizeof(EnvConfig)} offsets {mine}")


EXPORTED_SYMBOLS = (
    "merlin_version", "merlin_last_error", "merlin_tile_atlas", "merlin_env_config_layout", "merlin_env_create",
    "merlin_env_destroy", "merlin_env_seed", "merlin_env_reset", "merlin_env_step", "merlin_env_act_step", "merlin_group_act",
    "merlin_env_set_refill_interval", "merlin_env_refill", "merlin_env_set_lookahead_depth",
    "merlin_env_get_state", "merlin_env_full_obs", "merlin_env_errors", "merlin_env_set_step_fallback", "merlin_env_num_envs", "merlin_env_size",
    "merlin_obs_expand_f32", "merlin_obs_expand_u8", "merlin_gae", "merlin_adv_normalize",
    "merlin_conv1_lut_fwd", "merlin_conv1_lut_bwd", "merlin_tower_conv2_im2col_fwd",
    "merlin_tower_conv2_im2col_bwd", "merlin_tower_conv3_im2col_fwd", "merlin_tower_conv3_col2im_bwd",
    "merlin_tower_conv3_col2im_bwd_chunked", "merlin_tower_conv2_lut_rows", "merlin_tower_conv2_lut_fwd",
    "merlin_tower_conv2_lut_bwd", "merlin_tower_conv2_lut_fwd_grouped", "merlin_tower_conv2_lut_slab_bytes",
    "merlin_tower_conv2_lut_bwd_grouped", "merlin_tower_window_lut", "merlin_tower_window_lut_bias_relu", "merlin_minibatch_patch_maps", "merlin_segment_sum_mask_rows", "merlin_tower_window_conv3",
    "merlin_tower_window_conv3_bits", "merlin_tower_window_conv3_reuse", "merlin_tower_all_windows", "merlin_tower_codes_conv3",
    "merlin_tower_codes_conv3_amax", "merlin_tower_errors",
    "merlin_segment_sum", "merlin_segment_sum_masked", "merlin_segment_sum_marked", "merlin_segment_sum_fused", "merlin_tower_heads_fwd", "merlin_tower_bias_relu", "merlin_tower_relu_bwd", "merlin_tower_head_bwd",
    "merlin_tower_colsum",
    "merlin_ppo_loss_workspace", "merlin_ppo_loss", "merlin_act_heads",
    "merlin_x6_split", "merlin_x6_join", "merlin_x6_gemm_nt", "merlin_x6_tn_slab_floats", "merlin_x6_gemm_tn",
    "merlin_clip_adam_workspace", "merlin_clip_adam", "merlin_clip_adam_chain",
    "merlin_stage_fwd_planes", "merlin_stage_bwd_scatter", "merlin_gather_f32",
    "merlin_h3_amax", "merlin_h3_split", "merlin_h3_gemm_nt", "merlin_h3_gemm_tn",
    "merlin_h3_gemm_tn_planes", "merlin_h3_gemm_nt_gather", "merlin_h3_gemm_tn_gather",
    "merlin_h3_gemm_nt_heads", "merlin_h3_heads_parts", "merlin_heads_combine", "merlin_act_draw",
    "merlin_ppo_loss_absmax", "merlin_tower_head_bwd_planes", "merlin_h3_gemm_nt_planes",
    "merlin_h3_gemm_tn_gather_planes_a", "merlin_h3_gemm_nt_heads_planes", "merlin_h3_gemm_tn_gather_planes",
    "merlin_tower_window_conv3_planes", "merlin_window_gemm_bwd_work", "merlin_window_gemm_bwd",
    "merlin_window_gemm_fwd",
    "merlin_group_clip_sgd_workspace", "merlin_group_clip_sgd", "merlin_episode_loss",
    "merlin_env_set_difficulties", "merlin_episode_class_stats",
    "merlin_frame_atlas", "merlin_render_frames", "merlin_env_render", "merlin_env_snapshot",
    "merlin_shortest_paths", "merlin_env_optimal_steps", "merlin_shortest_paths_host",
    "merlin_h3_walk_blocks",
    "merlin_view_codes", "merlin_policy_paths", "merlin_policy_paths_host",
    "merlin_policy_chain", "merlin_policy_chain_host", "merlin_policy_occupancy", "merlin_policy_occupancy_host",
    "merlin_env_set_levels", "merlin_env_set_level_cdf", "merlin_env_levels", "merlin_env_set_level_log",
    "merlin_level_draw_host",
    "merlin_level_scores", "merlin_level_scores_host",
)


_CAPTURE_DEPTH = 0
_DEFERRED: list = []

_hip_rt = None
_cu_streams = []


def cu_masked_stream(device, keep) -> torch.cuda.ExternalStream:
    global _hip_rt
    if _hip_rt is None:
        _hip_rt = C.CDLL("libamdhip64.so")
        _hip_rt.hipExtStreamCreateWithCUMask.argtypes = [C.POINTER(C.c_void_p), C.c_uint32, C.POINTER(C.c_uint32)]
    dev = torch.device(device)
    n = torch.cuda.get_device_properties(dev).multi_processor_count
    words = (n + 31) // 32
    mask = (C.c_uint32 * words)()
    for i in range(n):
        if keep(i):
            mask[i // 32] |= 1 << (i % 32)
    if not any(mask):
        raise MerlinNativeError("cu_masked_stream: empty CU mask")
    h = C.c_void_p()
    with torch.cuda.device(dev):
        err = _hip_rt.hipExtStreamCreateWithCUMask(C.byref(h), words, mask)
    if err != 0:
        raise MerlinNativeError(f"hipExtStreamCreateWithCUMask failed ({err})")
    _cu_streams.append(h.value)
    return torch.cuda.ExternalStream(h.value, device=dev)



@contextlib.contextmanager
def capture_guard():
    global _CAPTURE_DEPTH
    drain_deferred()
    gc.collect()
    was_enabled = gc.isenabled()
    gc.disable()
    _CAPTURE_DEPTH += 1
    try:
        yield
    finally:
        _CAPTURE_DEPTH -= 1
        if _CAPTURE_DEPTH == 0:
            if was_enabled:
                gc.enable()
            run_deferred()


def capturing() -> bool:
    if _CAPTURE_DEPTH > 0:
        return True
    try:
        return torch.cuda.is_available() and torch.cuda.is_current_stream_capturing()
    except Exception:
        return False


def defer_release(fn) -> None:
    if capturing():
        _DEFERRED.append(fn)
    else:
        run_deferred()
        fn()


def run_deferred() -> None:
    while _DEFERRED:
        _DEFERRED.pop(0)()


def drain_deferred() -> None:
    if _DEFERRED and not capturing():
        run_deferred()


H3_SPANS: set = set()
X6_SPANS: set = set()


class KernelTimer:

    records: list | None = None
    every = 1
    counts: dict = {}

    @classmethod
    def start(cls, every: int = 1):
        cls.records, cls.every, cls.counts = [], max(1, int(every)), {}

    @classmethod
    def stop(cls):
        recs, cls.records = cls.records, None
        return [(n, e0, e1, nb() if callable(nb) else nb, fl) for n, e0, e1, nb, fl in (recs or [])]

    @classmethod
    def active(cls) -> bool:
        return cls.records is not None

    @classmethod
    def span(cls, name: str, nbytes: int, flops: int = 0):
        if cls.records is None or torch.cuda.is_current_stream_capturing():
            return _NULL_SPAN
        c = cls.counts.get(name, 0)
        cls.counts[name] = c + 1
        if c % cls.every:
            return _NULL_SPAN
        return _Span(name, nbytes, flops)


class _Span:
    def __init__(self, name, nbytes, flops=0):
        self.name, self.nbytes, self.flops = name, nbytes, flops

    def __enter__(self):
        self.e0 = torch.cuda.Event(enable_timing=True)
        self.e0.record()
        return self

    def __exit__(self, *exc):
        e1 = torch.cuda.Event(enable_timing=True)
        e1.record()
        KernelTimer.records.append((self.name, self.e0, e1, self.nbytes, self.flops))
        return False


class _NullSpan:
    def __enter__(self):
        return self

    def __exit__(self, *exc):
        return False


_NULL_SPAN = _NullSpan()


def check(rc: int, what: str = "") -> None:
    if rc != MERLIN_OK:
        msg = lib().merlin_last_error().decode(errors="replace")
        err = MerlinNativeError(f"{what or 'merlin call'} failed (code {rc}): {msg}")
        err.code = int(rc)
        raise err


def ptr(t: torch.Tensor | None):
    if t is None:
        return None
    if not t.is_cuda:
        raise MerlinNativeError("merlin HIP kernels need device (cuda/hip) tensors; got a CPU tensor")
# ... 420 lines not shown
    with KernelTimer.span("k_conv2_lut_fwd", n * (T * 25 * 64 * 4 + 32 + (8 if index is not None else 0))):
        check(lib().merlin_tower_conv2_lut_fwd(ptr(codes), ptr(index), n, ptr(tables), T, ptr(out),
                                               stream_of(codes)), "merlin_tower_conv2_lut_fwd")
    return out


def conv2_lut_fwd_grouped(codes, tables, group_frames: int):
    T = int(tables.shape[0])
    n = int(codes.shape[0])
    assert T % 2 == 0 and n == (T // 2) * group_frames, (T, n, group_frames)
    assert tables.shape == (T, LUT2_ROWS, 64) and tables.dtype == torch.float32 and tables.is_contiguous()
    assert codes.dtype == torch.int32 and codes.shape[-1] == OBS_WORDS and codes.is_contiguous()
    out = torch.empty((T, group_frames * 25, 64), dtype=torch.float32, device=codes.device)
    with KernelTimer.span("k_conv2_lut_fwd", n * (2 * 25 * 64 * 4 + 32)):
        check(lib().merlin_tower_conv2_lut_fwd_grouped(ptr(codes), n, int(group_frames), ptr(tables), T, ptr(out),
                                                       stream_of(codes)), "merlin_tower_conv2_lut_fwd_grouped")
    return out


_SLABS = {}


def conv2_lut_bwd_grouped(codes, dZ2c, absmax):
    T = int(dZ2c.shape[0])
    F = int(dZ2c.shape[2]) // 25
    assert codes.dtype == torch.int32 and codes.shape == ((T // 2) * F, OBS_WORDS) and codes.is_contiguous()
    nbytes = int(lib().merlin_tower_conv2_lut_slab_bytes(T, F))
    key = dZ2c.device
    slabs = _SLABS.get(key)
    if slabs is None or slabs.numel() < nbytes:
        slabs = _SLABS[key] = torch.empty(nbytes, dtype=torch.uint8, device=dZ2c.device)
    dt = torch.empty((T, LUT2_ROWS, 64), dtype=torch.float32, device=dZ2c.device)
    with KernelTimer.span("k_conv2_lut_hist", F * (T * 25 * 64 * 4 + 16 * T * 32)):
        check(lib().merlin_tower_conv2_lut_bwd_grouped(ptr(codes), F, ptr(dZ2c), ptr(absmax), T, ptr(dt), ptr(slabs),
                                                       stream_of(dZ2c)), "merlin_tower_conv2_lut_bwd_grouped")
    return dt


def conv2_lut_bwd(codes, dZ2c, absmax=None):
    T = int(dZ2c.shape[0])
    n = int(dZ2c.shape[2]) // 25
    assert codes.dtype == torch.int32 and codes.shape[-1] == OBS_WORDS and codes.shape[0] >= n
    if absmax is None:
        absmax = dZ2c.abs().amax().reshape(1).view(torch.int32) if dZ2c.numel() else \
            torch.zeros(1, dtype=torch.int32, device=dZ2c.device)
    dt = torch.empty((T, LUT2_ROWS, 64), dtype=torch.float32, device=dZ2c.device)
    with KernelTimer.span("k_conv2_lut_hist", n * (T * 25 * 64 * 4 + 16 * T * 32)):
        check(lib().merlin_tower_conv2_lut_bwd(ptr(codes), n, ptr(dZ2c), ptr(absmax), T, ptr(dt),
                                               stream_of(dZ2c)), "merlin_tower_conv2_lut_bwd")
    return dt


def window_lut(rows, tables, bias=None):
    T, nw = int(tables.shape[0]), int(rows.shape[0])
    assert tables.shape == (T, LUT2_ROWS, 64) and tables.dtype == torch.float32
    assert rows.dtype == torch.int32 and rows.shape == (nw, 16)
    out = torch.empty((T, nw, 64), dtype=torch.float32, device=tables.device)
    with KernelTimer.span("k_window_lut_all" if nw == ALL_WINDOWS else "k_window_lut", nw * (64 + T * 256)):
        if bias is not None:
            assert bias.shape == (T, 64) and bias.dtype == torch.float32 and bias.is_contiguous()
            check(lib().merlin_tower_window_lut_bias_relu(ptr(rows), nw, ptr(tables), T, ptr(bias), ptr(out),
                                                          stream_of(tables)), "merlin_tower_window_lut_bias_relu")
        else:
            check(lib().merlin_tower_window_lut(ptr(rows), nw, ptr(tables), T, ptr(out), stream_of(tables)),
                  "merlin_tower_window_lut")
    return out


_COLMAX_WS: dict = {}


def window_conv3_planes(Q, wid, groups, b3, rep_row, bound, n_reps=None):
    T, nw = int(Q.shape[0]), int(Q.shape[1])
    n = int(groups.numel())
    assert Q.shape[2] == 576 and Q.dtype == torch.float32 and Q.is_contiguous() and b3.shape == (T, 64) and T <= 2
    assert wid.dtype == torch.int32 and wid.shape[1] == 25 and groups.dtype == torch.int64
    assert rep_row.dtype == torch.int32 and rep_row.is_contiguous() and rep_row.numel() == n * 9
    assert bound.dtype == torch.int32 and bound.numel() >= T
    dev = Q.device
    ws = _COLMAX_WS.get(dev)
    if ws is None:
        ws = _COLMAX_WS[dev] = torch.empty(2 * 64 * 576, dtype=torch.int32, device=dev)
    out = torch.empty((T, n * 9, 128), dtype=torch.int16, device=dev)
    mask = torch.empty((T, n * 9), dtype=torch.int64, device=dev)
    if POISON_PARTIAL:
        out.fill_(-1)
        mask.fill_(-1)
    fixed = n * 144 + 2 * T * nw * 576 * 4
    nb = (lambda: T * int(n_reps) * 264 + fixed) if n_reps is not None else T * n * 9 * 264 + fixed
    with KernelTimer.span("k_window_conv3", nb):
        check(lib().merlin_tower_window_conv3_planes(ptr(Q), nw, ptr(wid), ptr(groups), n, ptr(b3), T, ptr(out),
                                                     ptr(mask), ptr(rep_row), ptr(ws), ptr(bound), stream_of(Q)),
              "merlin_tower_window_conv3_planes")
    return out, mask


def window_conv3(Q, wid, groups, b3, bits: bool = False, rows: int | None = None, amax=None, rep_row=None,
                 copy: int = 3, n_reps=None):
    T, nw = int(Q.shape[0]), int(Q.shape[1])
    n = int(groups.numel())
    R = n if rows is None else int(rows)
    assert Q.shape[2] == 576 and Q.dtype == torch.float32 and b3.shape == (T, 64) and R >= n
    assert wid.dtype == torch.int32 and wid.shape[1] == 25 and groups.dtype == torch.int64
    out = torch.empty((T, R * 9, 64), dtype=torch.float32, device=Q.device)
    if R > n:
        out[:, n * 9:].zero_()
    if rep_row is not None:
        assert bits and R == n and T <= 2
        assert rep_row.dtype == torch.int32 and rep_row.is_contiguous() and rep_row.numel() == n * 9
        mask = torch.empty((T, R * 9), dtype=torch.int64, device=Q.device)
        if POISON_PARTIAL and copy < 3:
            out.fill_(float("nan"))
            mask.fill_(-1)
        fixed = n * 144 + T * nw * 576 * 4
        if copy < 3 and n_reps is not None:
            nb = (lambda: T * int(n_reps) * 264 + fixed)
        else:
            nb = T * n * 9 * 264 + fixed
        with KernelTimer.span("k_window_conv3", nb):
            check(lib().merlin_tower_window_conv3_reuse(ptr(Q), nw, ptr(wid), ptr(groups), n, ptr(b3), T, ptr(out),
                                                        ptr(mask), ptr(amax), ptr(rep_row), int(copy),
                                                        stream_of(Q)),
                  "merlin_tower_window_conv3_reuse")
        return out, mask
    if bits:
        mask = torch.empty((T, R * 9), dtype=torch.int64, device=Q.device)
        with KernelTimer.span("k_window_conv3", T * n * 9 * 264 + n * 108 + T * nw * 576 * 4):
            check(lib().merlin_tower_window_conv3_bits(ptr(Q), nw, ptr(wid), ptr(groups), n, ptr(b3), T, ptr(out),
                                                       ptr(mask), ptr(amax), stream_of(Q)),
                  "merlin_tower_window_conv3_bits")
        return out, mask
    with KernelTimer.span("k_window_conv3", T * n * 9 * 256 + n * 108 + T * nw * 576 * 4):
        check(lib().merlin_tower_window_conv3(ptr(Q), nw, ptr(wid), ptr(groups), n, ptr(b3), T, ptr(out),
                                              stream_of(Q)), "merlin_tower_window_conv3")
    return out


ALL_WINDOWS = 4 ** 9 + 3 * 4 ** 8
POISON_PARTIAL = os.environ.get("MERLIN_POISON_PARTIAL", "0") == "1"


def minibatch_patch_maps(kid, group_keys, num_frames, group_offsets, nmb, num_patches):
    G, K = int(group_keys.numel()), int(num_patches)
    dev = group_keys.device
    assert kid.dtype == torch.int32 and kid.is_contiguous() and group_keys.dtype == torch.int64
    assert group_offsets.dtype == torch.int64 and group_offsets.numel() >= nmb
    kmap = torch.full((nmb, K), -1, dtype=torch.int32, device=dev)
    rmap = torch.empty((nmb, K), dtype=torch.int32, device=dev)
    rep_row = torch.empty(G * 9, dtype=torch.int32, device=dev)
    check(lib().merlin_minibatch_patch_maps(ptr(kid), ptr(group_keys), G, int(num_frames), ptr(group_offsets), K,
                                            ptr(kmap), ptr(rmap), ptr(rep_row), stream_of(group_keys)),
          "merlin_minibatch_patch_maps")
    return kmap, rep_row


def window_conv3_copy_masks(Y3, bits, rep_row):
    T, rows = int(bits.shape[0]), int(bits.shape[1])
    n = rows // 9
    assert bits.dtype == torch.int64 and rep_row.dtype == torch.int32 and rep_row.numel() == rows
    with KernelTimer.span("k_window_conv3_copy", T * rows * 12):
        check(lib().merlin_tower_window_conv3_reuse(None, 0, None, None, n, None, T, ptr(Y3), ptr(bits), None,
                                                    ptr(rep_row), 6, stream_of(bits)),
              "merlin_tower_window_conv3_reuse")
    return bits


def codes_conv3(codes, Qall, b3, amax=None):
    T, n = int(Qall.shape[0]), int(codes.shape[0])
    assert Qall.shape == (T, ALL_WINDOWS, 576) and Qall.dtype == torch.float32 and Qall.is_contiguous()
    assert codes.dtype == torch.int32 and codes.shape[1] == 8 and codes.is_contiguous() and b3.shape == (T, 64)
    if amax is not None:
        assert amax.dtype == torch.int32 and amax.numel() >= T
    out = torch.empty((T, n * 9, 64), dtype=torch.float32, device=Qall.device)
    with KernelTimer.span("k_codes_conv3", n * 32 + T * n * 9 * 256):
        check(lib().merlin_tower_codes_conv3_amax(ptr(codes), n, ptr(Qall), ptr(b3), T, ptr(out), ptr(amax),
                                                  stream_of(Qall)), "merlin_tower_codes_conv3_amax")
    return out


SEG_ACCUMULATE, SEG_NO_FILL, SEG_MASK_BITS = 1, 2, 4
SEG_ROLE_SHIFT = 8
SEG_ROLES = {"k_seg_sum_R": 1, "k_seg_sum_S": 2, "k_seg_sum_dQ": 3, "k_seg_sum_dT2": 4}


SEG_FUSED = True



def tower_errors(device=None, raise_on_error: bool = True) -> int:
    flags = C.c_uint32()
    dev = torch.device("cuda", torch.cuda.current_device()) if device is None else torch.device(device)
    with torch.cuda.device(dev):
        check(lib().merlin_tower_errors(C.byref(flags), C.c_void_p(torch.cuda.current_stream(dev).cuda_stream)),
              "merlin_tower_errors")
    if raise_on_error and flags.value & DEVERR_BAD_TILE:
        raise MerlinNativeError("merlin_tower_codes_conv3: a frame without the agent tile at view cell (3, 6), or with "
                                "it elsewhere -- not an observation; its windows were read as other windows")
    if raise_on_error and flags.value & DEVERR_BAD_FRAME:
        raise MerlinNativeError("merlin_render_frames: an agent outside the grid, on a wall or with a direction outside "
                                "0..3; its frame was drawn without the agent (merlin_view_codes: its codes are zero)")
    return flags.value

def segment_sum(src, plan, out_rows: int, slot=None, sub: int = 1, name: str = "k_seg_sum", out=None,
                accumulate: bool = False, carry=None, mask=None, fill: bool = True, mark=None, mask_rows=None):
    T, src_rows = int(src.shape[0]), int(src.shape[1])
    assert src.shape[2] == 64 and src.dtype == torch.float32 and src.is_contiguous()
    mask_bits = mask is not None and mask.dtype == torch.int64
    if mask_bits:
        assert mask.shape == (T, src_rows) and mask.is_contiguous()
    elif mask is not None:
        assert mask.shape == src.shape and mask.dtype == torch.float32 and mask.is_contiguous()
    if slot is not None:
        assert slot.dtype == torch.int32
    if out is None:
        assert not accumulate
        out = torch.empty((T, out_rows, 64), dtype=torch.float32, device=src.device)
    assert out.shape == (T, out_rows, 64) and out.dtype == torch.float32 and out.is_contiguous()
    need = T * max(plan.nitems, 1) * 128
    if carry is None or carry.numel() < need:
        carry = torch.empty(need, dtype=torch.float32, device=src.device)
    mrow = 0 if mask is None else (8 if mask_bits else 256)
    nb = plan.nnz * (8 + (4 if slot is not None else 0)) + T * (src_rows * (256 + mrow) + out_rows * 256)
    flags = (SEG_ACCUMULATE if accumulate else 0) | (0 if fill else SEG_NO_FILL) | (SEG_MASK_BITS if mask_bits else 0)
    flags |= SEG_ROLES.get(name, 0) << SEG_ROLE_SHIFT
    if mark is not None:
        assert mark.dtype == torch.int32 and mark.shape == (out_rows,) and mark.is_contiguous()
    fused = SEG_FUSED and getattr(plan, "counters", None) is not None
    if mask_rows is not None:
        assert mask_bits and mask_rows.dtype == torch.int32 and mask_rows.numel() == src_rows
        with KernelTimer.span(name, nb):
            check(lib().merlin_segment_sum_mask_rows(ptr(src), ptr(mask), src_rows, ptr(plan.idx), ptr(plan.key),
                                                     plan.nnz, ptr(slot), int(sub), plan.item_len, ptr(plan.fix),
                                                     int(plan.fix.shape[0]), T, ptr(out), int(out_rows), ptr(carry),
                                                     flags, ptr(mark), ptr(plan.head_fix) if fused else None,
                                                     ptr(plan.counters) if fused else None,
                                                     ptr(mask_rows), stream_of(src)), "merlin_segment_sum_mask_rows")
        return out
    with KernelTimer.span(name, nb):
        check(lib().merlin_segment_sum_fused(ptr(src), ptr(mask), src_rows, ptr(plan.idx), ptr(plan.key), plan.nnz,
                                             ptr(slot), int(sub), plan.item_len, ptr(plan.fix),
                                             int(plan.fix.shape[0]), T, ptr(out), int(out_rows), ptr(carry), flags,
                                             ptr(mark), ptr(plan.head_fix) if fused else None,
                                             ptr(plan.counters) if fused else None, stream_of(src)),
              "merlin_segment_sum_fused")
    return out


def bias_relu_(z, bias):
    T, rows, cols = (int(x) for x in z.shape)
    assert z.dtype == torch.float32 and bias.shape == (T, cols) and bias.dtype == torch.float32
    with KernelTimer.span("k_bias_relu", 2 * z.numel() * 4):
        check(lib().merlin_tower_bias_relu(ptr(z), ptr(bias), rows, cols, T, stream_of(z)), "merlin_tower_bias_relu")
    return z


def relu_bwd(y, dy, out=None, out_bias=None):
    T, rows, cols = (int(x) for x in y.shape)
    assert dy.shape == y.shape and y.dtype == dy.dtype == torch.float32
    dz = torch.empty_like(dy) if out is None else out
    db = torch.empty((T, cols), dtype=torch.float32, device=y.device) if out_bias is None else out_bias
    assert db.shape == (T, cols) and db.is_contiguous()
    with KernelTimer.span("k_relu_bwd_colsum", 3 * y.numel() * 4):
        check(lib().merlin_tower_relu_bwd(ptr(y), ptr(dy), ptr(dz), rows, cols, T, ptr(db), stream_of(y)),
              "merlin_tower_relu_bwd")
    return dz, db


def window_gemm_fwd(a2w, W3r, out=None):
    T, nw, ci = (int(v) for v in a2w.shape)
    assert ci == 64 and W3r.shape == (T, 64, 576) and a2w.dtype == W3r.dtype == torch.float32
    assert a2w.is_contiguous() and W3r.is_contiguous()
    Q = torch.empty((T, nw, 576), dtype=torch.float32, device=a2w.device) if out is None else out
    assert Q.shape == (T, nw, 576) and Q.is_contiguous()
    with KernelTimer.span("gemm_window_fwd", 0, flops=2 * T * nw * 64 * 576):
        check(lib().merlin_window_gemm_fwd(ptr(a2w), ptr(W3r), T, nw, ptr(Q), stream_of(a2w)),
              "merlin_window_gemm_fwd")
    return Q


_WINBWD_WORK = {}


def window_gemm_bwd(a2w, dQ, W3r, out_da2w=None, out_db2=None, out_dW3r=None, out_db3=None):
    T, nw, ci = (int(v) for v in a2w.shape)
    assert ci == 64 and dQ.shape == (T, nw, 576) and W3r.shape == (T, 64, 576)
    assert all(x.dtype == torch.float32 and x.is_contiguous() for x in (a2w, dQ, W3r))
    dev = a2w.device
    da2w = torch.empty_like(a2w) if out_da2w is None else out_da2w
    db2 = torch.empty((T, 64), dtype=torch.float32, device=dev) if out_db2 is None else out_db2
    dW3r = torch.empty((T, 64, 576), dtype=torch.float32, device=dev) if out_dW3r is None else out_dW3r
    assert da2w.shape == a2w.shape and db2.shape == (T, 64) and dW3r.shape == (T, 64, 576)
    assert all(x.dtype == torch.float32 and x.is_contiguous() for x in (da2w, db2, dW3r))
    need = int(lib().merlin_window_gemm_bwd_work(T, nw))
    key = (dev, T)
    work = _WINBWD_WORK.get(key)
    if work is None or work.numel() < need:
        work = _WINBWD_WORK[key] = torch.empty(max(need, 1 << 20), dtype=torch.float32, device=dev)
    with KernelTimer.span("k_winbwd", (2 * T * nw * (64 + 576) + T * 64 * 576) * 4):
        if out_db3 is not None:
            assert out_db3.shape == (T, 64) and out_db3.dtype == torch.float32 and out_db3.is_contiguous()
        check(lib().merlin_window_gemm_bwd(ptr(a2w), ptr(dQ), ptr(W3r), T, nw, ptr(da2w), ptr(db2), ptr(dW3r),
                                           ptr(out_db3), ptr(work), int(work.numel()), stream_of(a2w)),
              "merlin_window_gemm_bwd")
    return da2w, db2, dW3r


# ... 675 lines not shown
```

ppo-2dgrid_amd/merlin/ppo.py:

```python
from __future__ import annotations

import time

import warnings

import numpy as np
import torch
import torch.optim as optim

from . import _native as nat
from .actor_critic import CNNActorCritic, MLPActorCritic
from .distributed import DataParallel
from .envs import MerlinEnv, MerlinVecEnv
from .metrics.ppo_metrics import aggregate_ppo_update_metrics
from .rollout_buffer import CodeRolloutBuffer, RolloutBuffer
from .windows import deferred_fc1_wgrad

INV255 = 1.0 / 255.0


class _PPOLoss(torch.autograd.Function):

    @staticmethod
    def forward(ctx, logits, value, bias_actor, bias_critic, mb, sample_index, actions, logp_old, adv, ret, clip_eps,
# ... 259 lines not shown

    def _act(self, codes, pack, step, out=None):
        if pack is not None:
            return self.ac.act_codes_packed(codes, pack, seed=self._act_seed, epoch=self._act_epoch, step=step,
                                            out=out, env_offset=self.vec.env_offset)
        nat.expand_obs(codes, out=self._obs_step, scale=INV255)
        res = self.ac.act(self._obs_step, prescaled=True)
        if out is not None:
            for dst, src in zip(out, res):
                dst.copy_(src)
        return res

    def _record_episodes(self):
        done = self.buf.dones > 0
        rets = self.buf.ep_return[done]
        lens = self.buf.ep_length[done]
        self.episode_returns.extend(rets.cpu().tolist())
        self.episode_lengths.extend(int(x) for x in lens.cpu().tolist())

    def episode_class_stats(self, out=None, accumulate=False) -> torch.Tensor:
        if self.vec is None:
            raise ValueError("per-difficulty episode statistics need the vector env")
        buf = self.buf
        return nat.episode_class_stats(buf.dones, buf.ep_return, buf.ep_length, self.vec.class_ids,
                                       len(nat.DIFFICULTY_IDS), out=out, accumulate=accumulate)

    def episode_stats_by_difficulty(self) -> dict:
        rows = self.episode_class_stats().cpu().tolist()
        out = {}
        for name, cid in nat.DIFFICULTY_IDS.items():
            if name not in self.vec.difficulties:
                continue
            n, s1, s2, sl = rows[cid]
            if n > 0:
                mean = s1 / n
                out[name] = (int(n), mean, max(s2 / n - mean * mean, 0.0) ** 0.5, sl / n)
            else:
                out[name] = (0, float("nan"), float("nan"), float("nan"))
        return out

    def _collect_rollouts_single(self):
        state, _ = self.env.reset()
        total_steps, ep_return, ep_length = 0, 0.0, 0
        while total_steps < self.batch_size:
            state_t = self._obs_to_tensor(state)
            with torch.no_grad():
                action, logp, value = self.ac.act(state_t, deterministic=False)
            next_state, reward, terminated, truncated, _ = self.env.step(action.item())
            done = terminated or truncated
            self.buffer.add(state_t.squeeze(0), action.squeeze(), logp.squeeze(), value.squeeze(),
                            torch.tensor(reward, dtype=torch.float32, device=self.device),
                            torch.tensor(done, dtype=torch.float32, device=self.device))
            ep_return += reward
            ep_length += 1
            state = next_state
            total_steps += 1
            if done:
                self.episode_returns.append(ep_return)
                self.episode_lengths.append(ep_length)
                state, _ = self.env.reset()
                ep_return, ep_length = 0.0, 0
        with torch.no_grad():
            _, _, v = self.ac.act(self._obs_to_tensor(state))
        return v.item()

    def _flat_obs_at(self, t=None, index=None):
        buf = self.buf
        if self._full_obs is not None:
            x = self._full_obs[t] if index is None else self._full_obs[:buf.T].reshape(buf.T * buf.N, -1)[index]
            return x.reshape(x.shape[0], -1).float()
        codes = buf.codes[t] if index is None else buf.flat_codes
        return self.vec.flat_obs(codes, index=index)

    @torch.no_grad()
    def _collect_rollouts_flat(self):
        buf, env = self.buf, self.vec
        T = buf.T
        env.reset(out=buf.codes[0])
        if self._full_obs is not None:
            env.render_full(out=self._full_obs[0])
        for t in range(T):
            action, logp, value = self.ac.act(self._flat_obs_at(t))
            buf.actions[t].copy_(action)
            buf.logprobs[t].copy_(logp)
            buf.values[t].copy_(value)
            env.step_into(buf.actions[t], buf.codes[t + 1], buf.rewards[t], None, None, buf.dones[t],
                          buf.ep_return[t], buf.ep_length[t])
            if self._full_obs is not None:
                env.render_full(out=self._full_obs[t + 1])
        _, _, last_value = self.ac.act(self._flat_obs_at(T))
        buf.last_value.copy_(last_value)
        self._record_episodes()
        env.errors()
        return buf.last_value

    def compute_gae(self, rewards, values, dones, last_value, stats=None):
        lv = torch.as_tensor(last_value, dtype=torch.float32, device=rewards.device).reshape(-1)
        return nat.gae(rewards.contiguous(), values.contiguous(), dones.contiguous(), lv, self.gamma,
                       self.lam, stats=stats)

    def _advantages(self, rewards, values, dones, last_value, adv_out=None, ret_out=None):
        stats = torch.zeros(3, dtype=torch.float64, device=rewards.device)
        lv = torch.as_tensor(last_value, dtype=torch.float32, device=rewards.device).reshape(-1)
        adv, ret = nat.gae(rewards, values, dones, lv, self.gamma, self.lam, adv=adv_out, ret=ret_out,
                           stats=stats)
        self.dp.allreduce_sum_(stats)
        return nat.adv_normalize(adv, stats), ret

    def update(self, last_value=None):
        if self.vec is not None:
            buf = self.buf
            lv = buf.last_value if last_value is None else last_value
            adv_n, ret = self._advantages(buf.rewards, buf.values, buf.dones, lv, buf.adv, buf.returns)
            self.last_adv_normalized = adv_n
            if self.level_set is not None:
                self._update_levels()
            B = buf.T * buf.N
            return self._sgd(B, buf.flat_codes, None, buf.actions.reshape(B), buf.logprobs.reshape(B),
                             adv_n.reshape(B), ret.reshape(B))
        states, actions, logp_old, rewards, values_old, dones = self.buffer.get()
        adv_n, ret = self._advantages(rewards, values_old, dones, last_value)
        return self._sgd(states.shape[0], None, states, actions, logp_old, adv_n, ret)

    def _update_levels(self):
        buf, sampler = self.buf, self.level_sampler
        L = len(self.level_set)
        s, c = nat.level_scores(buf.adv, buf.levels, L, sampler.score_kind)
        self.dp.allreduce_sum_(s)
        self.dp.allreduce_sum_(c)
        self.level_iteration += 1
        sampler.update(s, c, self.level_iteration)
        cdf = sampler.cdf()
        self.vec.set_level_cdf(cdf)
        self.last_level_scores, self.last_level_cdf = (s, c), cdf

    def _minibatch_obs(self, codes, states, mb_idx):
        if codes is None:
            return states[mb_idx], False
        if not self.use_cnn:
            return self._flat_obs_at(index=mb_idx), False
        n = mb_idx.numel()
        if self._mb_obs is None or self._mb_obs.shape[0] < n:
            self._mb_obs = torch.empty((n, 3, 56, 56), dtype=torch.float32, device=self.device)
        out = self._mb_obs[:n]
        nat.expand_obs(codes, index=mb_idx, out=out, scale=INV255)
        return out, True

    def _sgd(self, B, codes, states, actions, logp_old, adv, returns):
        totals = torch.zeros(6, dtype=torch.float64, device=self.device)
        nb = 0
        use_codes = codes is not None and self.conv1_from_codes
        groups = plan = None
        if use_codes and self.dedup:
            from .dedup import FrameGroups

            groups = FrameGroups(codes)
            if not groups.ok:
                groups = None
            elif self.windows:
                from .windows import WindowPlan

                plan = WindowPlan(codes, groups)
                self.last_num_windows = plan.num_windows
        distinct = 0
        host_mb = []
        t_host = time.perf_counter()
        perms = [self._perm(B, epoch) for epoch in range(self.update_epochs)]
        fast = plan is not None and self.fast_step and getattr(self.ac, "fc1_impl", None) in ("x6", "h3")
        if fast and not all(p.requires_grad for p in self.ac.parameters()):
            fast = False
            for p in self.ac.parameters():
                if not p.requires_grad:
                    p.grad = None
        if fast:
            if self._wstep is None or not self._wstep.valid():
                from .fast_step import WindowStep

                if not self._params_on_flat():
                    self._rehome_parameters()
                self._wstep = WindowStep(self)
            self._wstep.bind_grads()
        chain = self._wstep.begin_update(totals) if fast else None
        if self._clip_adam is not None:
            self._clip_adam.chain = chain
        all_mbws = plan.update_minibatches(perms, self.minibatch_size, bulk=fast) if plan is not None else None
        for epoch in range(self.update_epochs):
            idxs = perms[epoch]
            mbws = all_mbws[epoch] if all_mbws is not None else None
            for k, start in enumerate(range(0, B, self.minibatch_size)):
                mb_idx = idxs[start:start + self.minibatch_size]
                if plan is not None:
                    mbw = mbws[k]
                    distinct += int(mbw.groups.numel())
                    if fast:
                        self._wstep.step(plan, mbw, mb_idx, actions, logp_old, adv, returns, totals)
                    else:
                        with deferred_fc1_wgrad():
                            logits, values = self.ac.heads_windows(plan, mbw, head_bias=False)
                        loss = _PPOLoss.apply(logits, values, self.ac.actor[2].bias, self.ac.critic[2].bias, mbw,
                                              mb_idx, actions, logp_old, adv, returns, self.clip_eps, self.vf_coef,
                                              self.ent_coef, totals)
                else:
                    lp_old, a_mb, ret_mb = logp_old[mb_idx], adv[mb_idx], returns[mb_idx]
                    if use_codes:
                        g = groups.minibatch(mb_idx) if groups is not None else None
                        if g is not None:
                            distinct += int(g[0].numel())
                        logp_new, entropy, values = self.ac.evaluate_codes(codes, actions[mb_idx], index=mb_idx,
                                                                           groups=g)
                    else:
                        obs, pre = self._minibatch_obs(codes, states, mb_idx)
                        logp_new, entropy, values = self.ac.evaluate(obs, actions[mb_idx], prescaled=pre)
                    values = values.squeeze(-1)
                    ratio = torch.exp(logp_new - lp_old)
                    surr1 = ratio * a_mb
                    surr2 = torch.clamp(ratio, 1 - self.clip_eps, 1 + self.clip_eps) * a_mb
                    pi_loss = -torch.min(surr1, surr2).mean()
                    v_loss = ((values - ret_mb) ** 2).mean()
                    ent = entropy.mean()
                    loss = pi_loss + self.vf_coef * v_loss - self.ent_coef * ent
                    with torch.no_grad():
                        approx_kl = (lp_old - logp_new).mean()
                        clipfrac = (torch.abs(ratio - 1.0) > self.clip_eps).float().mean()
                        totals[:5] += torch.stack([pi_loss.detach(), v_loss.detach(), ent.detach(), approx_kl,
                                                   clipfrac]).double()
                if not fast:
                    self.dp.zero_grad(self.optimizer)
                    loss.backward()
                self.dp.allreduce_grads()
                if self._clip_adam is not None:
                    grad_norm = self._clip_adam.step()
                else:
                    grad_norm = torch.nn.utils.clip_grad_norm_(self._params, 0.5)
                    self.optimizer.step()
                    if chain is not None:
                        self._wstep.refresh()
                if chain is None or self._clip_adam is None:
                    totals[5:].add_(grad_norm.detach())
                nb += 1
                host_mb.append(time.perf_counter())
        if self._clip_adam is not None:
            self._clip_adam.chain = None
        self.last_host_loop_ms = (time.perf_counter() - t_host) * 1e3
        self.last_host_mb_ms = [(b - a) * 1e3 for a, b in zip([t_host] + host_mb[:-1], host_mb)]
        t = totals.cpu().tolist()
        if groups is not None:
            self.last_distinct_frac = float(distinct) / float(self.update_epochs * B)
        return aggregate_ppo_update_metrics(*t, nb)

    def train(self, total_steps=100_000):
        steps_done = 0
        while steps_done < total_steps:
            last_value = self.collect_rollouts()
            self.update(last_value)
            steps_done += self.batch_size
```

ppo-2dgrid_amd/merlin/windows.py:

```python
from __future__ import annotations

import contextlib
import threading

import torch

from . import _native as nat

P2_OF = [[(p // 3 + k // 3) * 5 + p % 3 + k % 3 for k in range(9)] for p in range(9)]


def auto_item_len(nnz: int) -> int:
    L = 32
    while L < 1024 and L * 2 * 16384 <= nnz:
        L *= 2
    return L


def unpack_classes(codes: torch.Tensor) -> torch.Tensor:
    shifts = torch.arange(0, 32, 4, dtype=torch.int32, device=codes.device)
    nib = (codes.unsqueeze(-1) >> shifts) & 0xF
    return nib.reshape(codes.shape[0], 64)[:, :49].to(torch.int64).clamp_(max=4).view(-1, 7, 7)


def window_keys(cls: torch.Tensor) -> torch.Tensor:
    r = cls[:, :, 0:5] * 25 + cls[:, :, 1:6] * 5 + cls[:, :, 2:7]
    return (r[:, 0:5] * 15625 + r[:, 1:6] * 125 + r[:, 2:7]).reshape(-1, 25)


def patch_keys(cls: torch.Tensor) -> torch.Tensor:
    r = cls[:, :, 0:3]
    for b in range(1, 5):
        r = r * 5 + cls[:, :, b:b + 3]
    k = r[:, 0:3]
    for a in range(1, 5):
        k = k * 3125 + r[:, a:a + 3]
    return k.reshape(-1, 9)


def base5(digits: torch.Tensor) -> torch.Tensor:
    k = torch.zeros(digits.shape[0], dtype=torch.int64, device=digits.device)
    for i in range(digits.shape[1]):
        k = k * 5 + digits[:, i]
    return k


def digits5(keys: torch.Tensor, m: int) -> torch.Tensor:
    return torch.stack([(keys // 5 ** (m - 1 - i)) % 5 for i in range(m)], 1)


def window_rows(keys: torch.Tensor) -> torch.Tensor:
    d = [(keys // 5 ** (8 - i)) % 5 for i in range(9)]
    rows = []
    for ky in range(4):
        for kx in range(4):
            i, j = 3 * (ky >> 1) + (kx >> 1), 2 * (ky >> 1) + (kx >> 1)
            if not ky & 1 and not kx & 1:
                r = 4 * d[i] + j
            elif not ky & 1:
                r = 20 + 4 * (5 * d[i] + d[i + 1]) + j
            elif not kx & 1:
                r = 120 + 4 * (5 * d[i] + d[i + 3]) + j
            else:
                r = 220 + 4 * (125 * d[i] + 25 * d[i + 1] + 5 * d[i + 3] + d[i + 4]) + j
            rows.append(r)
    return torch.stack(rows, 1).to(torch.int32)


def compact_window_keys(device) -> torch.Tensor:
    d9 = torch.arange(4 ** 9, dtype=torch.int64, device=device)
    digits = [(d9 // 4 ** (8 - i)) % 4 for i in range(9)]
    out = [sum(digits[i] * 5 ** (8 - i) for i in range(9))]
    m = torch.arange(4 ** 8, dtype=torch.int64, device=device)
    d8 = [(m // 4 ** (7 - i)) % 4 for i in range(8)]
    for wx in (1, 2, 3):
        skip = 9 - wx
        cls, j = [], 0
        for i in range(9):
            if i == skip:
                cls.append(torch.full_like(m, 4))
            else:
                cls.append(d8[j])
                j += 1
        out.append(sum(cls[i] * 5 ** (8 - i) for i in range(9)))
    return torch.cat(out)


class SegmentPlan:

    def __init__(self, key_sorted: torch.Tensor, idx_sorted: torch.Tensor, item_len: int | None = None):
        dev = key_sorted.device
        n = int(key_sorted.numel())
        L = auto_item_len(n) if item_len is None else int(item_len)
        self.nnz, self.item_len = n, L
        self.nitems = (n + L - 1) // L
        self.key = key_sorted.to(torch.int32).contiguous()
        self.idx = idx_sorted.to(torch.int32).contiguous()
        if n == 0:
            self.fix = torch.zeros((0, 4), dtype=torch.int32, device=dev)
            self.head_fix = torch.zeros(0, dtype=torch.int32, device=dev)
            self.counters = torch.zeros(0, dtype=torch.int32, device=dev)
            return
        j = torch.arange(self.nitems, dtype=torch.int64, device=dev)
        p = torch.clamp((j + 1) * L, max=n) - 1
        kp = self.key[p].contiguous()
        s = torch.searchsorted(self.key, kp, side="left")
        e = torch.searchsorted(self.key, kp, side="right")
        live = (e > (j + 1) * L) & (s >= j * L)
        dst = torch.where(live, self.key[p].long(), torch.full_like(j, -1))
        self.fix = torch.stack([dst, j, (e - 1) // L, (s != j * L).long()], 1).to(torch.int32).contiguous()
        kf = self.key[j * L].contiguous()
        sf = torch.searchsorted(self.key, kf, side="left")
        self.head_fix = torch.where(sf < j * L, sf // L, torch.full_like(j, -1)).to(torch.int32).contiguous()
        self.counters = torch.zeros(self.nitems, dtype=torch.int32, device=dev)


class MinibatchWindows:

    def __init__(self, groups: torch.Tensor, inv: torch.Tensor, slot, order=None, offs=None, lazy=None):
        self.groups = groups
        self._inv, self._slot, self._order, self._offs = inv, slot, order, offs
        self._lazy = lazy

    def _derive(self):
        F, inv, perm, starts, lo, hi, off = self._lazy
        g, dev = self.groups, self.groups.device
        c = g.numel()
        s = torch.full((F,), -1, dtype=torch.int32, device=dev)
        s[g] = torch.arange(c, dtype=torch.int32, device=dev)
        self._slot = s
        self._inv = inv[lo:hi] - off
        self._order = (perm[lo:hi] - lo).to(torch.int32)
        self._offs = _frame_csr(starts[off:off + c] - lo, hi - lo)
        self._lazy = None

    @property
    def slot(self) -> torch.Tensor:
        if self._lazy is not None:
            self._derive()
        return self._slot

    @property
    def inv(self) -> torch.Tensor:
        if self._lazy is not None:
            self._derive()
        return self._inv

    @property
    def order(self):
        if self._lazy is not None:
            self._derive()
        return self._order

    @property
    def offs(self):
        if self._lazy is not None:
            self._derive()
        return self._offs


def _frame_csr(starts: torch.Tensor, n: int) -> torch.Tensor:
    out = torch.empty(starts.numel() + 1, dtype=torch.int32, device=starts.device)
    out[:-1] = starts
    out[-1:].fill_(n)
    return out


class WindowPlan:

    def __init__(self, codes: torch.Tensor, frame_groups, item_len: int | None = None,
                 hist_item_len: int | None = None):
        dev = codes.device
        self.frame_groups = frame_groups
        rep = codes.index_select(0, frame_groups.rep)
        F = int(rep.shape[0])
        cls = unpack_classes(rep)
        uniq, inv = torch.unique(window_keys(cls).reshape(-1).to(torch.int32), return_inverse=True)
        nw = int(uniq.numel())
        self.num_frames, self.num_windows = F, nw
        self.wid = inv.view(F, 25).to(torch.int32).contiguous()
        self.rows = window_rows(uniq).contiguous()
        assert int(self.rows.max()) < nat.LUT2_ROWS
        hk, ho = torch.sort(self.rows.reshape(-1), stable=True)
        self.hist = SegmentPlan(hk, ho // 16, hist_item_len)
        pk, kid = torch.unique(patch_keys(cls).reshape(-1), return_inverse=True)
        self.num_patches = int(pk.numel())
        self.kid = kid.view(F, 9).to(torch.int32).contiguous()
        ks, ko = torch.sort(kid.to(torch.int32), stable=True)
        self.patch_plan = SegmentPlan(ks, ko, item_len)
        K = self.num_patches
        B15 = 5 ** 15
        ky3 = torch.arange(3, dtype=torch.int64, device=dev)
        bkeys = ky3.unsqueeze(1) * B15 + (pk.unsqueeze(0) // (5 ** (10 - 5 * ky3)).unsqueeze(1)) % B15
        ub, bid = torch.unique(bkeys.reshape(-1), return_inverse=True)
        self.num_bands = int(ub.numel())
        bk, bo = torch.sort(bid.to(torch.int32), stable=True)
        self.band_plan = SegmentPlan(bk, (bo % K), item_len)
        bky, bkey = ub // B15, ub % B15
        brow = (bkey.unsqueeze(1) // (3125 ** (2 - ky3)).unsqueeze(0)) % 3125
        jb = torch.arange(self.num_bands, dtype=torch.int64, device=dev)
        ddst, dsrc = [], []
        for kx in range(3):
            c = (brow // 5 ** (2 - kx)) % 125
            w = torch.searchsorted(uniq, ((c[:, 0] * 125 + c[:, 1]) * 125 + c[:, 2]).to(torch.int32))
            ddst.append(w * 9 + bky * 3 + kx)
            dsrc.append(jb)
        dk, do = torch.sort(torch.cat(ddst).to(torch.int32), stable=True)
        self.dq_plan = SegmentPlan(dk, torch.cat(dsrc)[do], item_len)

    def update_minibatches(self, perms: list, minibatch_size: int, bulk: bool = False) -> list:
        B = int(perms[0].numel())
        flat = self.epoch_minibatches(torch.cat(perms), minibatch_size, period=B, bulk=bulk)
        nmb = (B + minibatch_size - 1) // minibatch_size
        return [flat[e * nmb:(e + 1) * nmb] for e in range(len(perms))]

    def _bulk_minibatches(self, uniq, inv, perm, starts, mb_of, counts, P, per, minibatch_size) -> list:
        dev, F, K = uniq.device, self.num_frames, self.num_patches
        nmb, G = len(counts), int(uniq.numel())
        goff_h = [0]
        for c in counts:
            goff_h.append(goff_h[-1] + c)
        lo_h = [(m // per) * P + (m % per) * minibatch_size for m in range(nmb)]
        hi_h = [(m // per) * P + min(P, (m % per + 1) * minibatch_size) for m in range(nmb)]
        goff = torch.tensor(goff_h, dtype=torch.int64).to(dev, non_blocking=True)
        lo = torch.tensor(lo_h, dtype=torch.int64).to(dev, non_blocking=True)
        span = torch.tensor([h - l for h, l in zip(hi_h, lo_h)], dtype=torch.int32).to(dev, non_blocking=True)
        mbg = uniq // F
        gall = uniq - mbg * F
        j = torch.arange(G, device=dev) - goff[mbg]
        slot = torch.full((nmb, F), -1, dtype=torch.int32, device=dev)
        slot.view(-1)[mbg * F + gall] = j.to(torch.int32)
        inv_local = inv - goff[mb_of]
        order = ((perm % P) % minibatch_size).to(torch.int32)
        offs = torch.empty(G + nmb, dtype=torch.int32, device=dev)
        offs[torch.arange(G, device=dev) + mbg] = (starts - lo[mbg]).to(torch.int32)
        offs[goff[1:] + torch.arange(nmb, device=dev)] = span
        kmap, rep_row = nat.minibatch_patch_maps(self.kid, uniq, F, goff, nmb, K)
        n_reps = (kmap >= 0).sum(dim=1) if nat.KernelTimer.active() else None
        out = []
        for m, c in enumerate(counts):
            g0 = goff_h[m]
            mw = MinibatchWindows(gall[g0:g0 + c], inv_local[lo_h[m]:hi_h[m]], slot[m], order[lo_h[m]:hi_h[m]],
                                  offs[g0 + m:g0 + m + c + 1])
            mw.kmap = kmap[m]
            mw.rep_row = rep_row[g0 * 9:(g0 + c) * 9]
            mw.n_reps = n_reps[m] if n_reps is not None else None
            out.append(mw)
        return out

    def epoch_minibatches(self, idxs: torch.Tensor, minibatch_size: int, period: int | None = None,
                          bulk: bool = False) -> list:
        dev, B, F = idxs.device, int(idxs.numel()), self.num_frames
        P = B if period is None else int(period)
        per = (P + minibatch_size - 1) // minibatch_size
        nmb = (B // P) * per
        pos = torch.arange(B, device=dev)
        mb_of = (pos // P) * per + (pos % P) // minibatch_size
        key = mb_of * F + self.frame_groups.uid[idxs]
        if nmb * F < 2 ** 31:
            key = key.to(torch.int32)
        sk, perm = torch.sort(key, stable=True)
        new = torch.ones(B, dtype=torch.bool, device=dev)
        new[1:] = sk[1:] != sk[:-1]
        inv = torch.empty(B, dtype=torch.int64, device=dev)
        inv[perm] = torch.cumsum(new, 0) - 1
        starts = torch.nonzero(new).squeeze(1)
        uniq = sk[starts].long()
        counts = torch.bincount(uniq // F, minlength=nmb).tolist()
        if bulk:
            return self._bulk_minibatches(uniq, inv, perm, starts, mb_of, counts, P, per, minibatch_size)
        out, off = [], 0
        gall = uniq % F
        for m, c in enumerate(counts):
            e, k = divmod(m, per)
            lo, hi = e * P + k * minibatch_size, e * P + min(P, (k + 1) * minibatch_size)
            out.append(MinibatchWindows(gall[off:off + c], None, None, lazy=(F, inv, perm, starts, lo, hi, off)))
            off += c
        return out

    def minibatch(self, mb_idx: torch.Tensor) -> MinibatchWindows:
        n = int(mb_idx.numel())
        sk, perm = torch.sort(self.frame_groups.uid[mb_idx], stable=True)
        new = torch.ones(n, dtype=torch.bool, device=mb_idx.device)
        new[1:] = sk[1:] != sk[:-1]
        starts = torch.nonzero(new).squeeze(1)
        g = sk[starts]
        inv = torch.empty(n, dtype=torch.int64, device=mb_idx.device)
        inv[perm] = torch.cumsum(new, 0) - 1
        slot = torch.full((self.num_frames,), -1, dtype=torch.int32, device=g.device)
        slot[g] = torch.arange(g.numel(), dtype=torch.int32, device=g.device)
        return MinibatchWindows(g, inv, slot, perm.to(torch.int32), _frame_csr(starts, n))


class _WindowConv2(torch.autograd.Function):

    @staticmethod
    def forward(ctx, T2, plan, nw_pad):
        ctx.plan = plan
        Z = nat.window_lut(plan.rows, T2.detach().contiguous())
        if nw_pad > Z.shape[1]:
            Zp = Z.new_zeros((Z.shape[0], nw_pad, 64))
            Zp[:, :Z.shape[1]] = Z
            Z = Zp
        return Z

    @staticmethod
    def backward(ctx, dZ2w):
        dT2 = nat.segment_sum(dZ2w.contiguous(), ctx.plan.hist, nat.LUT2_ROWS, name="k_seg_sum_dT2")
        return dT2, None, None


def _colsum(x):
    return nat.colsum(x)


class _BiasRelu(torch.autograd.Function):

    @staticmethod
    def forward(ctx, Z, b):
        A = torch.relu(Z + b.unsqueeze(1))
        ctx.save_for_backward(A)
        return A

    @staticmethod
    def backward(ctx, dA):
        (A,) = ctx.saved_tensors
        return nat.relu_bwd(A, dA.contiguous())


class _TunedBmm(torch.autograd.Function):

    @staticmethod
    def forward(ctx, A, B):
        from .gemm_tuning import tuned

        ctx.save_for_backward(A, B)
        with tuned("window"):
            return torch.bmm(A, B)

    @staticmethod
    def backward(ctx, dC):
        from .gemm_tuning import tuned

        A, B = ctx.saved_tensors
        dC = dC.contiguous()
        with tuned("window"):
            dA = torch.bmm(dC, B.transpose(1, 2)) if ctx.needs_input_grad[0] else None
            dB = torch.bmm(A.transpose(1, 2), dC) if ctx.needs_input_grad[1] else None
        return dA, dB


class _WindowGemm(torch.autograd.Function):

    @staticmethod
    def forward(ctx, a2w, W3r):
        ctx.save_for_backward(a2w, W3r)
        return torch.bmm(a2w, W3r)

    @staticmethod
    def backward(ctx, dQ):
        from .actor_critic import _splitk_bmm_tn

        a2w, W3r = ctx.saved_tensors
        dQ = dQ.contiguous()
        da2w = torch.bmm(dQ, W3r.transpose(1, 2)) if ctx.needs_input_grad[0] else None
        chunks = max(1, a2w.shape[1] // 256)
        dW3r = _splitk_bmm_tn(a2w, dQ, chunks, min_chunk=128, name="gemm_window_wgrad") if ctx.needs_input_grad[1] \
# ... 195 lines not shown
```

Baseline: 4.965 million.

## Build window/patch/band plans and minibatch groupings natively with rocPRIM kernels

Replaces the torch-based construction of frame dedup groups, window, patch, band and dq segment plans, and per-minibatch groupings with dedicated HIP kernels that use rocPRIM sorts and scans. The goal is to cut the many small torch launches, unique/sort calls and host syncs during plan building each PPO update. It adds a native code path, on by default and switchable off with an environment variable. Host readbacks of counts remain, and the new kernels carry correctness risk.

Measured after the change: 5.115 million (median of 6 runs). 1.03x the previous value.

```diff
diff --git a/include/merlin_hip.h b/include/merlin_hip.h
--- a/include/merlin_hip.h
+++ b/include/merlin_hip.h
@@ -174,6 +174,30 @@
 int merlin_minibatch_patch_maps(const int32_t *kid_dev, const int64_t *group_keys_dev, int64_t n_groups,
                                 int64_t n_frames, const int64_t *group_offsets_dev, int32_t n_patches, int32_t *kmap_dev,
                                 int32_t *rmap_dev, int32_t *rep_row_dev, void *stream);
+int64_t merlin_plan_minibatches_workspace(int64_t n, int64_t period, int64_t minibatch, int64_t n_frames);
+int64_t merlin_plan_sort_workspace(int64_t n, int32_t key_bytes);
+int merlin_plan_frames(const uint32_t *codes_dev, int64_t n, const uint64_t *mult_host, void *workspace_dev,
+                       int64_t workspace_bytes, int64_t *uid_dev, int64_t *rep_dev, int32_t *wkey_dev,
+                       uint64_t *pkey_dev, int32_t *mark_dev, int32_t *wrank_dev, int64_t *counts_dev, void *stream);
+int merlin_plan_windows(int64_t n_frames, int64_t n_windows, const int32_t *wkey_dev, const int32_t *mark_dev,
+                        const int32_t *wrank_dev, int32_t lut_rows, int64_t item_len, void *workspace_dev,
+                        int64_t workspace_bytes, int32_t *wid_dev, int32_t *rows_dev, int32_t *key_dev,
+                        int32_t *idx_dev, int32_t *fix_dev, int32_t *head_fix_dev, int64_t *counts_dev, void *stream);
+int merlin_plan_patches(int64_t n_frames, const uint64_t *pkey_dev, int64_t item_len, void *workspace_dev,
+                        int64_t workspace_bytes, int32_t *kid_dev, uint64_t *pk_dev, int32_t *key_dev,
+                        int32_t *idx_dev, int32_t *fix_dev, int32_t *head_fix_dev, int64_t *counts_dev, void *stream);
+int merlin_plan_bands(int64_t n_patches, const uint64_t *pk_dev, int64_t item_len, void *workspace_dev,
+                      int64_t workspace_bytes, uint64_t *ub_dev, int32_t *key_dev, int32_t *idx_dev, int32_t *fix_dev,
+                      int32_t *head_fix_dev, int64_t *counts_dev, void *stream);
+int merlin_plan_dq(int64_t n_bands, int64_t n_windows, const uint64_t *ub_dev, const int32_t *mark_dev,
+                   const int32_t *wrank_dev, int64_t item_len, void *workspace_dev, int64_t workspace_bytes,
+                   int32_t *key_dev, int32_t *idx_dev, int32_t *fix_dev, int32_t *head_fix_dev, int64_t *counts_dev,
+                   void *stream);
+int merlin_plan_minibatches(const int64_t *idxs_dev, int64_t n, int64_t period, int64_t minibatch,
+                            const int64_t *uid_dev, int64_t n_samples, int64_t n_frames, void *workspace_dev,
+                            int64_t workspace_bytes, int64_t *group_keys_dev, int64_t *groups_dev, int64_t *inv_dev,
+                            int32_t *slot_dev, int32_t *order_dev, int32_t *offs_dev, int64_t *group_offsets_dev,
+                            void *stream);
 int merlin_tower_window_lut_bias_relu(const int32_t *rows_dev, int64_t n_windows, const float *tables_dev,
                                       int32_t towers, const float *b2_dev, float *a2w_dev, void *stream);
 int merlin_tower_window_conv3(const float *Q_dev, int64_t n_windows, const int32_t *wid_dev,
diff --git a/ppo-2dgrid_amd/csrc/merlin_capi.hip b/ppo-2dgrid_amd/csrc/merlin_capi.hip
--- a/ppo-2dgrid_amd/csrc/merlin_capi.hip
+++ b/ppo-2dgrid_amd/csrc/merlin_capi.hip
@@ -1104,6 +1104,134 @@
     return MERLIN_OK;
 }
 
+namespace {
+int64_t plan_key_span(int64_t n, int64_t period, int64_t mbs, int64_t n_frames, int *rc) {
+    *rc = MERLIN_OK;
+    if (n < 1 || period < 1 || mbs < 1 || n_frames < 1 || n % period) {
+        *rc = fail(MERLIN_E_INVALID, "bad shape: n must be a positive multiple of period");
+        return 0;
+    }
+    const int64_t nmb = (n / period) * ((period + mbs - 1) / mbs);
+    if (n > INT32_MAX || nmb > INT32_MAX / n_frames) {
+        *rc = fail(MERLIN_E_UNSUPPORTED, "more than 2^31 samples or (minibatch, frame) keys");
+        return 0;
+    }
+    return nmb * n_frames;
+}
+}
+
+int64_t merlin_plan_sort_workspace(int64_t n, int32_t key_bytes) {
+    if (n < 1 || n > INT32_MAX || (key_bytes != 4 && key_bytes != 8)) {
+        fail(MERLIN_E_INVALID, "bad sort shape");
+        return -1;
+    }
+    const int64_t bytes = merlin::plan_sort_workspace(n, key_bytes);
+    if (bytes < 0) fail(MERLIN_E_HIP, "rocprim scratch size query failed");
+    return bytes;
+}
+
+namespace {
+int plan_stage_args(int64_t n, int32_t key_bytes, const void *ws, int64_t ws_bytes, int64_t item_len, bool ptrs) {
+    if (n < 1 || item_len < 1) return fail(MERLIN_E_INVALID, "bad shape");
+    if (n > INT32_MAX) return fail(MERLIN_E_UNSUPPORTED, "more than 2^31 list entries");
+    if (!ws || !ptrs) return fail(MERLIN_E_INVALID, "null argument");
+    const int64_t need = merlin_plan_sort_workspace(n, key_bytes);
+    if (need < 0) return MERLIN_E_HIP;
+    if (ws_bytes < need) return fail(MERLIN_E_INVALID, "workspace smaller than merlin_plan_sort_workspace");
+    return MERLIN_OK;
+}
+}
+
+int merlin_plan_frames(const uint32_t *codes, int64_t n, const uint64_t *mult_host, void *ws, int64_t ws_bytes,
+                       int64_t *uid, int64_t *rep, int32_t *wkey, uint64_t *pkey, int32_t *mark, int32_t *wrank,
+                       int64_t *counts, void *stream) {
+    if (n > INT32_MAX / 25) return fail(MERLIN_E_UNSUPPORTED, "more than 2^31 / 25 frames");
+    const int rc = plan_stage_args(n, 8, ws, ws_bytes, 1,
+                                   codes && mult_host && uid && rep && wkey && pkey && mark && wrank && counts);
+    if (rc != MERLIN_OK) return rc;
+    HIP_TRY(merlin::launch_plan_frames(codes, n, mult_host, ws, ws_bytes, uid, rep, wkey, pkey, mark, wrank, counts,
+                                       (hipStream_t)stream));
+    return MERLIN_OK;
+}
+
+int merlin_plan_windows(int64_t n_frames, int64_t n_windows, const int32_t *wkey, const int32_t *mark,
+                        const int32_t *wrank, int32_t lut_rows, int64_t item_len, void *ws, int64_t ws_bytes,
+                        int32_t *wid, int32_t *rows, int32_t *key, int32_t *idx, int32_t *fix, int32_t *head_fix,
+                        int64_t *counts, void *stream) {
+    if (n_frames < 1 || n_frames > INT32_MAX / 25 || n_windows > 1953125 || lut_rows < 1)
+        return fail(MERLIN_E_INVALID, "bad shape");
+    const int rc = plan_stage_args(n_windows * 16, 4, ws, ws_bytes, item_len,
+                                   wkey && mark && wrank && wid && rows && key && idx && fix && head_fix && counts);
+    if (rc != MERLIN_OK) return rc;
+    HIP_TRY(merlin::launch_plan_windows(n_frames, n_windows, wkey, mark, wrank, lut_rows, item_len, ws, ws_bytes, wid,
+                                        rows, key, idx, fix, head_fix, counts, (hipStream_t)stream));
+    return MERLIN_OK;
+}
+
+int merlin_plan_patches(int64_t n_frames, const uint64_t *pkey, int64_t item_len, void *ws, int64_t ws_bytes,
+                        int32_t *kid, uint64_t *pk, int32_t *key, int32_t *idx, int32_t *fix, int32_t *head_fix,
+                        int64_t *counts, void *stream) {
+    if (n_frames < 1 || n_frames > INT32_MAX / 25) return fail(MERLIN_E_INVALID, "bad shape");
+    const int rc = plan_stage_args(n_frames * 9, 8, ws, ws_bytes, item_len,
+                                   pkey && kid && pk && key && idx && fix && head_fix && counts);
+    if (rc != MERLIN_OK) return rc;
+    HIP_TRY(merlin::launch_plan_patches(n_frames, pkey, item_len, ws, ws_bytes, kid, pk, key, idx, fix, head_fix,
+                                        counts, (hipStream_t)stream));
+    return MERLIN_OK;
+}
+
+int merlin_plan_bands(int64_t n_patches, const uint64_t *pk, int64_t item_len, void *ws, int64_t ws_bytes,
+                      uint64_t *ub, int32_t *key, int32_t *idx, int32_t *fix, int32_t *head_fix, int64_t *counts,
+                      void *stream) {
+    if (n_patches < 1 || n_patches > INT32_MAX / 3) return fail(MERLIN_E_INVALID, "bad shape");
+    const int rc = plan_stage_args(n_patches * 3, 8, ws, ws_bytes, item_len,
+                                   pk && ub && key && idx && fix && head_fix && counts);
+    if (rc != MERLIN_OK) return rc;
+    HIP_TRY(merlin::launch_plan_bands(n_patches, pk, item_len, ws, ws_bytes, ub, key, idx, fix, head_fix, counts,
+                                      (hipStream_t)stream));
+    return MERLIN_OK;
+}
+
+int merlin_plan_dq(int64_t n_bands, int64_t n_windows, const uint64_t *ub, const int32_t *mark, const int32_t *wrank,
+                   int64_t item_len, void *ws, int64_t ws_bytes, int32_t *key, int32_t *idx, int32_t *fix,
+                   int32_t *head_fix, int64_t *counts, void *stream) {
+    if (n_bands < 1 || n_bands > INT32_MAX / 3 || n_windows < 1 || n_windows > 1953125)
+        return fail(MERLIN_E_INVALID, "bad shape");
+    const int rc = plan_stage_args(n_bands * 3, 4, ws, ws_bytes, item_len,
+                                   ub && mark && wrank && key && idx && fix && head_fix && counts);
+    if (rc != MERLIN_OK) return rc;
+    HIP_TRY(merlin::launch_plan_dq(n_bands, n_windows, ub, mark, wrank, item_len, ws, ws_bytes, key, idx, fix,
+                                   head_fix, counts, (hipStream_t)stream));
+    return MERLIN_OK;
+}
+
+int64_t merlin_plan_minibatches_workspace(int64_t n, int64_t period, int64_t minibatch, int64_t n_frames) {
+    int rc;
+    const int64_t span = plan_key_span(n, period, minibatch, n_frames, &rc);
+    if (rc != MERLIN_OK) return -1;
+    const int64_t bytes = merlin::plan_minibatches_workspace(n, span);
+    if (bytes < 0) fail(MERLIN_E_HIP, "rocprim scratch size query failed");
+    return bytes;
+}
+
+int merlin_plan_minibatches(const int64_t *idxs, int64_t n, int64_t period, int64_t minibatch, const int64_t *uid,
+                            int64_t n_samples, int64_t n_frames, void *workspace, int64_t workspace_bytes,
+                            int64_t *group_keys, int64_t *groups, int64_t *inv, int32_t *slot, int32_t *order,
+                            int32_t *offs, int64_t *group_offsets, void *stream) {
+    int rc;
+    plan_key_span(n, period, minibatch, n_frames, &rc);
+    if (rc != MERLIN_OK) return rc;
+    if (n_samples < 1) return fail(MERLIN_E_INVALID, "bad shape");
+    if (!idxs || !uid || !workspace || !group_keys || !groups || !inv || !slot || !order || !offs || !group_offsets)
+        return fail(MERLIN_E_INVALID, "null argument");
+    if (workspace_bytes < merlin_plan_minibatches_workspace(n, period, minibatch, n_frames))
+        return fail(MERLIN_E_INVALID, "workspace smaller than merlin_plan_minibatches_workspace");
+    HIP_TRY(merlin::launch_plan_minibatches(idxs, n, period, minibatch, uid, n_samples, n_frames, workspace,
+                                            workspace_bytes, group_keys, groups, inv, slot, order, offs,
+                                            group_offsets, (hipStream_t)stream));
+    return MERLIN_OK;
+}
+
 int merlin_tower_window_lut_bias_relu(const int32_t *rows, int64_t nw, const float *tables, int32_t towers,
                                       const float *b2, float *a2w, void *stream) {
     if ((!rows || !tables || !a2w || !b2) && nw > 0) return fail(MERLIN_E_INVALID, "null argument");
diff --git a/ppo-2dgrid_amd/csrc/merlin_internal.h b/ppo-2dgrid_amd/csrc/merlin_internal.h
--- a/ppo-2dgrid_amd/csrc/merlin_internal.h
+++ b/ppo-2dgrid_amd/csrc/merlin_internal.h
@@ -355,6 +355,28 @@
 
 hipError_t launch_patch_maps(const int32_t *kid, const int64_t *gkey, int64_t G, int64_t F, const int64_t *goff, int K,
                              int32_t *kmap, int32_t *rmap, int32_t *rep_row, hipStream_t s);
+int64_t plan_minibatches_workspace(int64_t N, int64_t key_span);
+hipError_t launch_plan_minibatches(const int64_t *idxs, int64_t N, int64_t P, int64_t mbs, const int64_t *uid,
+                                   int64_t B0, int64_t F, void *ws, int64_t ws_bytes, int64_t *gkey, int64_t *gall,
+                                   int64_t *inv, int32_t *slot, int32_t *order, int32_t *offs, int64_t *goff,
+                                   hipStream_t s);
+int64_t plan_sort_workspace(int64_t n, int key_bytes);
+hipError_t launch_plan_frames(const uint32_t *codes, int64_t B, const uint64_t *mult, void *ws, int64_t ws_bytes,
+                              int64_t *uid, int64_t *rep, int32_t *wkey, uint64_t *pkey, int32_t *mark,
+                              int32_t *wrank, int64_t *counts, hipStream_t st);
+hipError_t launch_plan_windows(int64_t F, int64_t nw, const int32_t *wkey, const int32_t *mark, const int32_t *wrank,
+                               int lut_rows, int64_t L, void *ws, int64_t ws_bytes, int32_t *wid, int32_t *rows,
+                               int32_t *key, int32_t *idx, int32_t *fix, int32_t *head_fix, int64_t *counts,
+                               hipStream_t st);
+hipError_t launch_plan_patches(int64_t F, const uint64_t *pkey, int64_t L, void *ws, int64_t ws_bytes, int32_t *kid,
+                               uint64_t *pk, int32_t *key, int32_t *idx, int32_t *fix, int32_t *head_fix,
+                               int64_t *counts, hipStream_t st);
+hipError_t launch_plan_bands(int64_t K, const uint64_t *pk, int64_t L, void *ws, int64_t ws_bytes, uint64_t *ub,
+                             int32_t *key, int32_t *idx, int32_t *fix, int32_t *head_fix, int64_t *counts,
+                             hipStream_t st);
+hipError_t launch_plan_dq(int64_t nb, int64_t nw, const uint64_t *ub, const int32_t *mark, const int32_t *wrank,
+                          int64_t L, void *ws, int64_t ws_bytes, int32_t *key, int32_t *idx, int32_t *fix,
+                          int32_t *head_fix, int64_t *counts, hipStream_t st);
 hipError_t launch_window_lut(const int32_t *rows, int64_t nw, const float *tab, int T, float *Z2w, hipStream_t s,
                              const float *b2 = nullptr);
 hipError_t launch_window_conv3(const float *Q, int64_t nw, const int32_t *wid, const int64_t *groups, int64_t n,
diff --git a/ppo-2dgrid_amd/csrc/merlin_plan.hip b/ppo-2dgrid_amd/csrc/merlin_plan.hip
--- /dev/null
+++ b/ppo-2dgrid_amd/csrc/merlin_plan.hip
@@ -0,0 +1,544 @@
+#include <cstring>
+
+#include <rocprim/rocprim.hpp>
+
+#include "merlin_internal.h"
+
+namespace merlin {
+namespace {
+
+constexpr int64_t ALIGN = 256;
+inline int64_t aligned(int64_t bytes) { return (bytes + ALIGN - 1) / ALIGN * ALIGN; }
+
+struct MbGeom {
+    int64_t N, P, mbs, per, F, B0;
+    int nmb;
+};
+
+__device__ __forceinline__ int64_t mb_lo(const MbGeom &g, int m) { return (m / g.per) * g.P + (m % g.per) * g.mbs; }
+__device__ __forceinline__ int64_t mb_hi(const MbGeom &g, int m) {
+    const int64_t e = m / g.per, k = m % g.per;
+    return e * g.P + (g.P < (k + 1) * g.mbs ? g.P : (k + 1) * g.mbs);
+}
+
+__global__ __launch_bounds__(256) void k_plan_keys(MbGeom g, const int64_t *__restrict__ idxs,
+                                                   const int64_t *__restrict__ uid, uint32_t *__restrict__ key,
+                                                   uint32_t *__restrict__ val, int64_t *__restrict__ err) {
+    const int64_t pos = (int64_t)blockIdx.x * 256 + threadIdx.x;
+    if (pos >= g.N) return;
+    const int64_t e = pos / g.P, r = pos - e * g.P;
+    const int64_t m = e * g.per + r / g.mbs;
+    const int64_t i = idxs[pos];
+    int64_t u = 0;
+    if (i < 0 || i >= g.B0) {
+        *err = 1;
+    } else {
+        u = uid[i];
+        if (u < 0 || u >= g.F) {
+            *err = 1;
+            u = 0;
+        }
+    }
+    key[pos] = (uint32_t)(m * g.F + u);
+    val[pos] = (uint32_t)pos;
+}
+
+__global__ __launch_bounds__(256) void k_plan_heads(int64_t N, const uint32_t *__restrict__ sk,
+                                                    int32_t *__restrict__ head) {
+    const int64_t i = (int64_t)blockIdx.x * 256 + threadIdx.x;
+    if (i >= N) return;
+    head[i] = (i == 0 || sk[i] != sk[i - 1]) ? 1 : 0;
+}
+
+__global__ __launch_bounds__(256) void k_plan_derive(MbGeom g, const uint32_t *__restrict__ sk,
+                                                     const uint32_t *__restrict__ sv, const int32_t *__restrict__ rank,
+                                                     int64_t *__restrict__ gkey, int64_t *__restrict__ gall,
+                                                     int64_t *__restrict__ inv, int32_t *__restrict__ slot,
+                                                     int32_t *__restrict__ order, int32_t *__restrict__ offs,
+                                                     int64_t *__restrict__ goff) {
+    const int64_t i = (int64_t)blockIdx.x * 256 + threadIdx.x;
+    if (i >= g.N) return;
+    const int64_t key = sk[i], pos = sv[i];
+    const int m = (int)(key / g.F);
+    const int64_t frame = key - (int64_t)m * g.F;
+    const int64_t lo = mb_lo(g, m), hi = mb_hi(g, m);
+    const int64_t grp = rank[i] - 1, g0 = rank[lo] - 1;
+    inv[pos] = grp - g0;
+    order[i] = (int32_t)((pos % g.P) % g.mbs);
+    if (i == 0 || sk[i - 1] != (uint32_t)key) {
+        gkey[grp] = key;
+        gall[grp] = frame;
+        slot[(int64_t)m * g.F + frame] = (int32_t)(grp - g0);
+        offs[grp + m] = (int32_t)(i - lo);
+    }
+    if (i == lo) goff[m] = grp;
+    if (i == hi - 1) {
+        offs[grp + 1 + m] = (int32_t)(hi - lo);
+        if (m == g.nmb - 1) goff[g.nmb] = grp + 1;
+    }
+}
+
+int key_bits(int64_t span) {
+    int b = 1;
+    while (b < 32 && ((int64_t)1 << b) < span) ++b;
+    return b;
+}
+
+struct PlanScratch {
+    int64_t key_in, val_in, key_out, val_out, rank, temp, temp_bytes, total;
+};
+
+hipError_t plan_scratch(int64_t N, int bits, PlanScratch &s) {
+    size_t sort_bytes = 0, scan_bytes = 0;
+    hipError_t e = rocprim::radix_sort_pairs(nullptr, sort_bytes, (uint32_t *)nullptr, (uint32_t *)nullptr,
+                                             (uint32_t *)nullptr, (uint32_t *)nullptr, (size_t)N, 0u, (unsigned)bits);
+    if (e != hipSuccess) return e;
+    e = rocprim::inclusive_scan(nullptr, scan_bytes, (int32_t *)nullptr, (int32_t *)nullptr, (size_t)N,
+                                rocprim::plus<int32_t>());
+    if (e != hipSuccess) return e;
+    const int64_t a = aligned(N * 4);
+    s.key_in = 0;
+    s.val_in = a;
+    s.key_out = 2 * a;
+    s.val_out = 3 * a;
+    s.rank = 4 * a;
+    s.temp = 5 * a;
+    s.temp_bytes = aligned((int64_t)std::max(sort_bytes, scan_bytes));
+    s.total = s.temp + s.temp_bytes;
+    return hipSuccess;
+}
+
+
+constexpr int64_t W9 = 1953125;
+constexpr int64_t B15 = 30517578125LL;
+
+template <class K>
+struct SortBufs {
+    K *kin, *kout;
+    uint32_t *vin, *vout;
+    int32_t *rank;
+    void *temp;
+    size_t temp_bytes;
+    int64_t n;
+
+    static hipError_t bytes(int64_t n, int64_t &total, size_t &temp_bytes) {
+        size_t sort_bytes = 0, scan_bytes = 0;
+        hipError_t e = rocprim::radix_sort_pairs(nullptr, sort_bytes, (K *)nullptr, (K *)nullptr, (uint32_t *)nullptr,
+                                                 (uint32_t *)nullptr, (size_t)n, 0u, (unsigned)(8 * sizeof(K)));
+        if (e != hipSuccess) return e;
+        e = rocprim::inclusive_scan(nullptr, scan_bytes, (int32_t *)nullptr, (int32_t *)nullptr, (size_t)n,
+                                    rocprim::plus<int32_t>());
+        if (e != hipSuccess) return e;
+        size_t table_bytes = 0;
+        e = rocprim::exclusive_scan(nullptr, table_bytes, (int32_t *)nullptr, (int32_t *)nullptr, (int32_t)0,
+                                    (size_t)W9, rocprim::plus<int32_t>());
+        if (e != hipSuccess) return e;
+        temp_bytes = (size_t)aligned((int64_t)std::max(std::max(sort_bytes, scan_bytes), table_bytes));
+        total = 2 * aligned(n * (int64_t)sizeof(K)) + 4 * aligned(n * 4) + (int64_t)temp_bytes;
+        return hipSuccess;
+    }
+
+    hipError_t carve(void *ws, int64_t ws_bytes, int64_t n_) {
+        n = n_;
+        int64_t total;
+        hipError_t e = bytes(n, total, temp_bytes);
+        if (e != hipSuccess) return e;
+        if (ws_bytes < total) return hipErrorInvalidValue;
+        char *w = (char *)ws;
+        const int64_t ak = aligned(n * (int64_t)sizeof(K)), av = aligned(n * 4);
+        kin = (K *)w, kout = (K *)(w + ak);
+        vin = (uint32_t *)(w + 2 * ak), vout = (uint32_t *)(w + 2 * ak + av);
+        rank = (int32_t *)(w + 2 * ak + 2 * av);
+        temp = w + 2 * ak + 4 * av;
+        return hipSuccess;
+    }
+    int32_t *head() const { return (int32_t *)((char *)rank + aligned(n * 4)); }
+};
+
+template <class K>
+__global__ __launch_bounds__(256) void k_plan_run_heads(int64_t n, const K *__restrict__ sk,
+                                                        int32_t *__restrict__ head) {
+    const int64_t i = (int64_t)blockIdx.x * 256 + threadIdx.x;
+    if (i >= n) return;
+    head[i] = (i == 0 || sk[i] != sk[i - 1]) ? 1 : 0;
+}
+
+template <class K>
+hipError_t sort_and_rank(SortBufs<K> &b, int bits, bool want_rank, hipStream_t st) {
+    size_t tb = b.temp_bytes;
+    hipError_t e = rocprim::radix_sort_pairs(b.temp, tb, b.kin, b.kout, b.vin, b.vout, (size_t)b.n, 0u,
+                                             (unsigned)bits, st);
+    if (e != hipSuccess || !want_rank) return e;
+    const dim3 grid((unsigned)((b.n + 255) / 256));
+    hipLaunchKernelGGL(k_plan_run_heads<K>, grid, dim3(256), 0, st, b.n, b.kout, b.head());
+    if ((e = hipGetLastError()) != hipSuccess) return e;
+    tb = b.temp_bytes;
+    return rocprim::inclusive_scan(b.temp, tb, b.head(), b.rank, (size_t)b.n, rocprim::plus<int32_t>(), st);
+}
+
+struct Mult8 {
+    uint64_t m[8];
+};
+
+__global__ __launch_bounds__(256) void k_plan_hash(const uint32_t *__restrict__ codes, int64_t B, Mult8 mu,
+                                                   int64_t *__restrict__ key, uint32_t *__restrict__ val) {
+    const int64_t i = (int64_t)blockIdx.x * 256 + threadIdx.x;
+    if (i >= B) return;
+    uint64_t h = 0;
+#pragma unroll
+    for (int k = 0; k < 8; ++k) {
+        h = (h ^ (uint64_t)codes[i * 8 + k]) * mu.m[k];
+        h ^= h >> 29;
+    }
+    key[i] = (int64_t)h;
+    val[i] = (uint32_t)i;
+}
+
+__device__ __forceinline__ int tile_class(const uint32_t (&w)[8], int r, int c) {
+    const int cell = r * 7 + c;
+    const int v = (int)((w[cell >> 3] >> ((cell & 7) * 4)) & 0xF);
+    return v > 4 ? 4 : v;
+}
+
+enum { CNT_F = 0, CNT_BAD = 1, CNT_NW = 2, CNT_ROWS = 3, CNT_K = 4, CNT_NB = 5, CNT_NOWIN = 6, CNT_N = 8 };
+
+__global__ __launch_bounds__(256) void k_plan_frames(int64_t B, const int64_t *__restrict__ sh,
+                                                     const uint32_t *__restrict__ sidx,
+                                                     const int32_t *__restrict__ rank,
+                                                     const uint32_t *__restrict__ codes, int64_t *__restrict__ uid,
+                                                     int64_t *__restrict__ rep, int32_t *__restrict__ wkey,
+                                                     uint64_t *__restrict__ pkey, int32_t *__restrict__ mark,
+                                                     int64_t *__restrict__ counts) {
+    const int64_t i = (int64_t)blockIdx.x * 256 + threadIdx.x;
+    if (i >= B) return;
+    const int64_t u = rank[i] - 1, frame = sidx[i];
+    uid[frame] = u;
+    if (i == B - 1) counts[CNT_F] = u + 1;
+    if (i > 0 && sh[i] == sh[i - 1]) return;
+    rep[u] = frame;
+    uint32_t w[8];
+#pragma unroll
+    for (int k = 0; k < 8; ++k) w[k] = codes[frame * 8 + k];
+    int r3[7][5], r5[7][3];
+#pragma unroll
+    for (int r = 0; r < 7; ++r) {
+        int c[7];
+#pragma unroll
+        for (int x = 0; x < 7; ++x) c[x] = tile_class(w, r, x);
+#pragma unroll
+        for (int x = 0; x < 5; ++x) r3[r][x] = c[x] * 25 + c[x + 1] * 5 + c[x + 2];
+#pragma unroll
+        for (int x = 0; x < 3; ++x) r5[r][x] = (((c[x] * 5 + c[x + 1]) * 5 + c[x + 2]) * 5 + c[x + 3]) * 5 + c[x + 4];
+    }
+#pragma unroll
+    for (int py = 0; py < 5; ++py)
+#pragma unroll
+        for (int px = 0; px < 5; ++px) {
+            const int k = r3[py][px] * 15625 + r3[py + 1][px] * 125 + r3[py + 2][px];
+            wkey[u * 25 + py * 5 + px] = k;
+            mark[k] = 1;
+        }
+#pragma unroll
+    for (int oy = 0; oy < 3; ++oy)
+#pragma unroll
+        for (int ox = 0; ox < 3; ++ox) {
+            uint64_t k = 0;
+#pragma unroll
+            for (int a = 0; a < 5; ++a) k = k * 3125 + (uint64_t)r5[oy + a][ox];
+            pkey[u * 9 + oy * 3 + ox] = k;
+        }
+}
+
+__global__ __launch_bounds__(256) void k_plan_verify(int64_t B, const uint32_t *__restrict__ codes,
+                                                     const int64_t *__restrict__ uid, const int64_t *__restrict__ rep,
+                                                     int64_t *__restrict__ counts) {
+    const int64_t i = (int64_t)blockIdx.x * 256 + threadIdx.x;
+    if (i >= B) return;
+    const int64_t r = rep[uid[i]];
+    bool same = true;
+#pragma unroll
+    for (int k = 0; k < 8; ++k) same = same && codes[i * 8 + k] == codes[r * 8 + k];
+    if (!same) counts[CNT_BAD] = 1;
+}
+
+__global__ __launch_bounds__(256) void k_plan_count_windows(const int32_t *__restrict__ mark,
+                                                            const int32_t *__restrict__ wrank,
+                                                            int64_t *__restrict__ counts) {
+    if (blockIdx.x == 0 && threadIdx.x == 0) counts[CNT_NW] = (int64_t)wrank[W9 - 1] + mark[W9 - 1];
+}
+
+__device__ __forceinline__ int window_row(int key, int ky, int kx) {
+    int d[9], q = key;
+#pragma unroll
+    for (int i = 8; i >= 0; --i) {
+        d[i] = q % 5;
+        q /= 5;
+    }
+    const int i = 3 * (ky >> 1) + (kx >> 1), j = 2 * (ky >> 1) + (kx >> 1);
+    if (!(ky & 1) && !(kx & 1)) return 4 * d[i] + j;
+    if (!(ky & 1)) return 20 + 4 * (5 * d[i] + d[i + 1]) + j;
+    if (!(kx & 1)) return 120 + 4 * (5 * d[i] + d[i + 3]) + j;
+    return 220 + 4 * (125 * d[i] + 25 * d[i + 1] + 5 * d[i + 3] + d[i + 4]) + j;
+}
+
+__global__ __launch_bounds__(256) void k_plan_window_rows(const int32_t *__restrict__ mark,
+                                                          const int32_t *__restrict__ wrank, int lut_rows,
+                                                          int32_t *__restrict__ rows, uint32_t *__restrict__ hkey,
+                                                          uint32_t *__restrict__ hval, int64_t *__restrict__ counts) {
+    const int64_t t = (int64_t)blockIdx.x * 256 + threadIdx.x;
+    if (t >= W9 * 16) return;
+    const int key = (int)(t >> 4), tap = (int)(t & 15);
+    if (!mark[key]) return;
+    const int w = wrank[key], r = window_row(key, tap >> 2, tap & 3);
+    if (r >= lut_rows) counts[CNT_ROWS] = 1;
+    rows[w * 16 + tap] = r;
+    hkey[w * 16 + tap] = (uint32_t)r;
+    hval[w * 16 + tap] = (uint32_t)(w * 16 + tap);
+}
+
+__global__ __launch_bounds__(256) void k_plan_wid(int64_t n, const int32_t *__restrict__ wkey,
+                                                  const int32_t *__restrict__ wrank, int32_t *__restrict__ wid) {
+    const int64_t e = (int64_t)blockIdx.x * 256 + threadIdx.x;
+    if (e < n) wid[e] = wrank[wkey[e]];
+}
+
+template <int MODE, class K>
+__global__ __launch_bounds__(256) void k_plan_list(int64_t n, const K *__restrict__ sk,
+                                                   const uint32_t *__restrict__ sv, const int32_t *__restrict__ rank,
+                                                   int64_t div, int32_t *__restrict__ key, int32_t *__restrict__ idx,
+                                                   int32_t *__restrict__ inverse, uint64_t *__restrict__ uniq,
+                                                   int64_t *__restrict__ count) {
+    const int64_t i = (int64_t)blockIdx.x * 256 + threadIdx.x;
+    if (i >= n) return;
+    const uint32_t e = sv[i];
+    if (MODE == 0 || MODE == 3) {
+        key[i] = (int32_t)sk[i];
+        idx[i] = MODE == 0 ? (int32_t)(e >> 4) : (int32_t)(e % (uint32_t)div);
+    } else {
+        const int32_t run = rank[i] - 1;
+        key[i] = run;
+        idx[i] = MODE == 1 ? (int32_t)e : (int32_t)(e % (uint32_t)div);
+        if (MODE == 1) inverse[e] = run;
+        if (i == 0 || sk[i] != sk[i - 1]) uniq[run] = (uint64_t)sk[i];
+        if (i == n - 1) *count = run + 1;
+    }
+}
+
+__global__ __launch_bounds__(256) void k_plan_band_keys(int64_t K, const uint64_t *__restrict__ pk,
+                                                        uint64_t *__restrict__ key, uint32_t *__restrict__ val) {
+    const int64_t e = (int64_t)blockIdx.x * 256 + threadIdx.x;
+    if (e >= 3 * K) return;
+    const int ky = (int)(e / K);
+    const int64_t k = e - ky * K;
+    const uint64_t div = ky == 0 ? 9765625ULL : ky == 1 ? 3125ULL : 1ULL;
+    key[e] = (uint64_t)ky * (uint64_t)B15 + (pk[k] / div) % (uint64_t)B15;
+    val[e] = (uint32_t)e;
+}
+
+__global__ __launch_bounds__(256) void k_plan_dq_keys(int64_t nb, const uint64_t *__restrict__ ub,
+                                                      const int32_t *__restrict__ mark,
+                                                      const int32_t *__restrict__ wrank, uint32_t *__restrict__ key,
+                                                      uint32_t *__restrict__ val, int64_t *__restrict__ counts) {
+    const int64_t e = (int64_t)blockIdx.x * 256 + threadIdx.x;
+    if (e >= 3 * nb) return;
+    const int kx = (int)(e / nb);
+    const int64_t j = e - kx * nb;
+    const uint64_t b = ub[j], bky = b / (uint64_t)B15, bkey = b % (uint64_t)B15;
+    const int p5 = kx == 0 ? 25 : kx == 1 ? 5 : 1;
+    const int c0 = (int)((bkey / 9765625ULL) % 3125) / p5 % 125, c1 = (int)((bkey / 3125ULL) % 3125) / p5 % 125,
+              c2 = (int)(bkey % 3125) / p5 % 125;
+    const int wk = (c0 * 125 + c1) * 125 + c2;
+    if (!mark[wk]) counts[CNT_NOWIN] = 1;
+    key[e] = (uint32_t)(wrank[wk] * 9 + (int)bky * 3 + kx);
+    val[e] = (uint32_t)e;
+}
+
+__device__ __forceinline__ int64_t plan_bound(const int32_t *key, int64_t n, int32_t x, bool upper) {
+    int64_t lo = 0, hi = n;
+    while (lo < hi) {
+        const int64_t mid = (lo + hi) >> 1;
+        if (upper ? key[mid] <= x : key[mid] < x)
+            lo = mid + 1;
+        else
+            hi = mid;
+    }
+    return lo;
+}
+
+__global__ __launch_bounds__(256) void k_plan_segfix(const int32_t *__restrict__ key, int64_t n, int64_t L,
+                                                     int64_t nitems, int4 *__restrict__ fix,
+                                                     int32_t *__restrict__ head_fix) {
+    const int64_t j = (int64_t)blockIdx.x * 256 + threadIdx.x;
+    if (j >= nitems) return;
+    const int64_t p = ((j + 1) * L < n ? (j + 1) * L : n) - 1;
+    const int32_t kp = key[p];
+    const int64_t s = plan_bound(key, n, kp, false), e = plan_bound(key, n, kp, true);
+    const bool live = e > (j + 1) * L && s >= j * L;
+    fix[j] = make_int4(live ? kp : -1, (int)j, (int)((e - 1) / L), s != j * L ? 1 : 0);
+    const int64_t sf = plan_bound(key, n, key[j * L], false);
+    head_fix[j] = sf < j * L ? (int32_t)(sf / L) : -1;
+}
+
+__global__ __launch_bounds__(256) void k_plan_copy_keys(int64_t n, const uint64_t *__restrict__ src,
+                                                        uint64_t *__restrict__ key, uint32_t *__restrict__ val) {
+    const int64_t e = (int64_t)blockIdx.x * 256 + threadIdx.x;
+    if (e >= n) return;
+    key[e] = src[e];
+    val[e] = (uint32_t)e;
+}
+
+hipError_t launch_segfix(const int32_t *key, int64_t n, int64_t L, int32_t *fix, int32_t *head_fix, hipStream_t st) {
+    const int64_t nitems = (n + L - 1) / L;
+    hipLaunchKernelGGL(k_plan_segfix, dim3((unsigned)((nitems + 255) / 256)), dim3(256), 0, st, key, n, L, nitems,
+                       (int4 *)fix, head_fix);
+    return hipGetLastError();
+}
+
+inline dim3 grid_of(int64_t n) { return dim3((unsigned)((n + 255) / 256)); }
+
+}
+
+int64_t plan_sort_workspace(int64_t n, int key_bytes) {
+    int64_t total = -1;
+    size_t tb;
+    if (n <= 0) return -1;
+    const hipError_t e = key_bytes == 8 ? SortBufs<uint64_t>::bytes(n, total, tb) : SortBufs<uint32_t>::bytes(n, total, tb);
+    return e == hipSuccess ? total : -1;
+}
+
+hipError_t launch_plan_frames(const uint32_t *codes, int64_t B, const uint64_t *mult, void *ws, int64_t ws_bytes,
+                              int64_t *uid, int64_t *rep, int32_t *wkey, uint64_t *pkey, int32_t *mark,
+                              int32_t *wrank, int64_t *counts, hipStream_t st) {
+    SortBufs<int64_t> b;
+    hipError_t e = b.carve(ws, ws_bytes, B);
+    if (e != hipSuccess) return e;
+    Mult8 mu;
+    for (int k = 0; k < 8; ++k) mu.m[k] = mult[k];
+    if ((e = hipMemsetAsync(counts, 0, CNT_N * 8, st)) != hipSuccess) return e;
+    if ((e = hipMemsetAsync(mark, 0, W9 * 4, st)) != hipSuccess) return e;
+    hipLaunchKernelGGL(k_plan_hash, grid_of(B), dim3(256), 0, st, codes, B, mu, b.kin, b.vin);
+    if ((e = hipGetLastError()) != hipSuccess) return e;
+    if ((e = sort_and_rank(b, 64, true, st)) != hipSuccess) return e;
+    hipLaunchKernelGGL(k_plan_frames, grid_of(B), dim3(256), 0, st, B, b.kout, b.vout, b.rank, codes, uid, rep, wkey,
+                       pkey, mark, counts);
+    if ((e = hipGetLastError()) != hipSuccess) return e;
+    hipLaunchKernelGGL(k_plan_verify, grid_of(B), dim3(256), 0, st, B, codes, uid, rep, counts);
+    if ((e = hipGetLastError()) != hipSuccess) return e;
+    size_t tb = b.temp_bytes, need = 0;
+    e = rocprim::exclusive_scan(nullptr, need, mark, wrank, (int32_t)0, (size_t)W9, rocprim::plus<int32_t>());
+    if (e != hipSuccess) return e;
+    if (need > tb) return hipErrorInvalidValue;
+    e = rocprim::exclusive_scan(b.temp, tb, mark, wrank, (int32_t)0, (size_t)W9, rocprim::plus<int32_t>(), st);
+    if (e != hipSuccess) return e;
+    hipLaunchKernelGGL(k_plan_count_windows, dim3(1), dim3(256), 0, st, mark, wrank, counts);
+    return hipGetLastError();
+}
+
+hipError_t launch_plan_windows(int64_t F, int64_t nw, const int32_t *wkey, const int32_t *mark, const int32_t *wrank,
+                               int lut_rows, int64_t L, void *ws, int64_t ws_bytes, int32_t *wid, int32_t *rows,
+                               int32_t *key, int32_t *idx, int32_t *fix, int32_t *head_fix, int64_t *counts,
+                               hipStream_t st) {
+    SortBufs<uint32_t> b;
+    hipError_t e = b.carve(ws, ws_bytes, nw * 16);
+    if (e != hipSuccess) return e;
+    hipLaunchKernelGGL(k_plan_wid, grid_of(F * 25), dim3(256), 0, st, F * 25, wkey, wrank, wid);
+    if ((e = hipGetLastError()) != hipSuccess) return e;
+    hipLaunchKernelGGL(k_plan_window_rows, grid_of(W9 * 16), dim3(256), 0, st, mark, wrank, lut_rows, rows, b.kin,
+                       b.vin, counts);
+    if ((e = hipGetLastError()) != hipSuccess) return e;
+    if ((e = sort_and_rank(b, key_bits(lut_rows > 1 ? 2 * (int64_t)lut_rows : 2), false, st)) != hipSuccess) return e;
+    hipLaunchKernelGGL((k_plan_list<0, uint32_t>), grid_of(b.n), dim3(256), 0, st, b.n, b.kout, b.vout, nullptr,
+                       (int64_t)16, key, idx, nullptr, nullptr, nullptr);
+    if ((e = hipGetLastError()) != hipSuccess) return e;
+    return launch_segfix(key, b.n, L, fix, head_fix, st);
+}
+
+hipError_t launch_plan_patches(int64_t F, const uint64_t *pkey, int64_t L, void *ws, int64_t ws_bytes, int32_t *kid,
+                               uint64_t *pk, int32_t *key, int32_t *idx, int32_t *fix, int32_t *head_fix,
+                               int64_t *counts, hipStream_t st) {
+    SortBufs<uint64_t> b;
+    hipError_t e = b.carve(ws, ws_bytes, F * 9);
+    if (e != hipSuccess) return e;
+    hipLaunchKernelGGL(k_plan_copy_keys, grid_of(b.n), dim3(256), 0, st, b.n, pkey, b.kin, b.vin);
+    if ((e = hipGetLastError()) != hipSuccess) return e;
+    if ((e = sort_and_rank(b, 59, true, st)) != hipSuccess) return e;
+    hipLaunchKernelGGL((k_plan_list<1, uint64_t>), grid_of(b.n), dim3(256), 0, st, b.n, b.kout, b.vout, b.rank,
+                       (int64_t)1, key, idx, kid, pk, counts + CNT_K);
+    if ((e = hipGetLastError()) != hipSuccess) return e;
+    return launch_segfix(key, b.n, L, fix, head_fix, st);
+}
+
+hipError_t launch_plan_bands(int64_t K, const uint64_t *pk, int64_t L, void *ws, int64_t ws_bytes, uint64_t *ub,
+                             int32_t *key, int32_t *idx, int32_t *fix, int32_t *head_fix, int64_t *counts,
+                             hipStream_t st) {
+    SortBufs<uint64_t> b;
+    hipError_t e = b.carve(ws, ws_bytes, K * 3);
+    if (e != hipSuccess) return e;
+    hipLaunchKernelGGL(k_plan_band_keys, grid_of(b.n), dim3(256), 0, st, K, pk, b.kin, b.vin);
+    if ((e = hipGetLastError()) != hipSuccess) return e;
+    if ((e = sort_and_rank(b, 37, true, st)) != hipSuccess) return e;
+    hipLaunchKernelGGL((k_plan_list<2, uint64_t>), grid_of(b.n), dim3(256), 0, st, b.n, b.kout, b.vout, b.rank, K, key,
+                       idx, nullptr, ub, counts + CNT_NB);
+    if ((e = hipGetLastError()) != hipSuccess) return e;
+    return launch_segfix(key, b.n, L, fix, head_fix, st);
+}
+
+hipError_t launch_plan_dq(int64_t nb, int64_t nw, const uint64_t *ub, const int32_t *mark, const int32_t *wrank,
+                          int64_t L, void *ws, int64_t ws_bytes, int32_t *key, int32_t *idx, int32_t *fix,
+                          int32_t *head_fix, int64_t *counts, hipStream_t st) {
+    SortBufs<uint32_t> b;
+    hipError_t e = b.carve(ws, ws_bytes, nb * 3);
+    if (e != hipSuccess) return e;
+    hipLaunchKernelGGL(k_plan_dq_keys, grid_of(b.n), dim3(256), 0, st, nb, ub, mark, wrank, b.kin, b.vin, counts);
+    if ((e = hipGetLastError()) != hipSuccess) return e;
+    if ((e = sort_and_rank(b, key_bits(nw * 9), false, st)) != hipSuccess) return e;
+    hipLaunchKernelGGL((k_plan_list<3, uint32_t>), grid_of(b.n), dim3(256), 0, st, b.n, b.kout, b.vout, nullptr, nb,
+                       key, idx, nullptr, nullptr, nullptr);
+    if ((e = hipGetLastError()) != hipSuccess) return e;
+    return launch_segfix(key, b.n, L, fix, head_fix, st);
+}
+
+int64_t plan_minibatches_workspace(int64_t N, int64_t key_span) {
+    PlanScratch s;
+    if (N <= 0 || plan_scratch(N, key_bits(key_span), s) != hipSuccess) return -1;
+    return s.total;
+}
+
+hipError_t launch_plan_minibatches(const int64_t *idxs, int64_t N, int64_t P, int64_t mbs, const int64_t *uid,
+                                   int64_t B0, int64_t F, void *ws, int64_t ws_bytes, int64_t *gkey, int64_t *gall,
+                                   int64_t *inv, int32_t *slot, int32_t *order, int32_t *offs, int64_t *goff,
+                                   hipStream_t st) {
+    MbGeom g;
+    g.N = N, g.P = P, g.mbs = mbs, g.F = F, g.B0 = B0;
+    g.per = (P + mbs - 1) / mbs;
+    g.nmb = (int)((N / P) * g.per);
+    const int bits = key_bits((int64_t)g.nmb * F);
+    PlanScratch s;
+    hipError_t e = plan_scratch(N, bits, s);
+    if (e != hipSuccess) return e;
+    if (ws_bytes < s.total) return hipErrorInvalidValue;
+    char *w = (char *)ws;
+    uint32_t *key_in = (uint32_t *)(w + s.key_in), *val_in = (uint32_t *)(w + s.val_in);
+    uint32_t *key_out = (uint32_t *)(w + s.key_out), *val_out = (uint32_t *)(w + s.val_out);
+    int32_t *rank = (int32_t *)(w + s.rank);
+    const dim3 grid((unsigned)((N + 255) / 256));
+    e = hipMemsetAsync(slot, 0xFF, (size_t)g.nmb * F * 4, st);
+    if (e != hipSuccess) return e;
+    e = hipMemsetAsync(goff, 0, (size_t)(g.nmb + 2) * 8, st);
+    if (e != hipSuccess) return e;
+    hipLaunchKernelGGL(k_plan_keys, grid, dim3(256), 0, st, g, idxs, uid, key_in, val_in, goff + g.nmb + 1);
+    if ((e = hipGetLastError()) != hipSuccess) return e;
+    size_t tb = (size_t)s.temp_bytes;
+    e = rocprim::radix_sort_pairs(w + s.temp, tb, key_in, key_out, val_in, val_out, (size_t)N, 0u, (unsigned)bits, st);
+    if (e != hipSuccess) return e;
+    hipLaunchKernelGGL(k_plan_heads, grid, dim3(256), 0, st, N, key_out, (int32_t *)key_in);
+    if ((e = hipGetLastError()) != hipSuccess) return e;
+    tb = (size_t)s.temp_bytes;
+    e = rocprim::inclusive_scan(w + s.temp, tb, (int32_t *)key_in, rank, (size_t)N, rocprim::plus<int32_t>(), st);
+    if (e != hipSuccess) return e;
+    hipLaunchKernelGGL(k_plan_derive, grid, dim3(256), 0, st, g, key_out, val_out, rank, gkey, gall, inv, slot, order,
+                       offs, goff);
+    return hipGetLastError();
+}
+
+}
diff --git a/ppo-2dgrid_amd/merlin/_native.py b/ppo-2dgrid_amd/merlin/_native.py
--- a/ppo-2dgrid_amd/merlin/_native.py
+++ b/ppo-2dgrid_amd/merlin/_native.py
@@ -107,6 +107,16 @@
     L.merlin_tower_window_conv3.argtypes = [vp, i64, vp, vp, i64, vp, i32, vp, vp]
     L.merlin_tower_window_lut_bias_relu.argtypes = [vp, i64, vp, i32, vp, vp, vp]
     L.merlin_minibatch_patch_maps.argtypes = [vp, vp, i64, i64, vp, i32, vp, vp, vp, vp]
+    L.merlin_plan_sort_workspace.argtypes = [i64, i32]
+    L.merlin_plan_sort_workspace.restype = i64
+    L.merlin_plan_frames.argtypes = [vp, i64, u64p, vp, i64, vp, vp, vp, vp, vp, vp, vp, vp]
+    L.merlin_plan_windows.argtypes = [i64, i64, vp, vp, vp, i32, i64, vp, i64, vp, vp, vp, vp, vp, vp, vp, vp]
+    L.merlin_plan_patches.argtypes = [i64, vp, i64, vp, i64, vp, vp, vp, vp, vp, vp, vp, vp]
+    L.merlin_plan_bands.argtypes = [i64, vp, i64, vp, i64, vp, vp, vp, vp, vp, vp, vp]
+    L.merlin_plan_dq.argtypes = [i64, i64, vp, vp, vp, i64, vp, i64, vp, vp, vp, vp, vp, vp]
+    L.merlin_plan_minibatches_workspace.argtypes = [i64, i64, i64, i64]
+    L.merlin_plan_minibatches_workspace.restype = i64
+    L.merlin_plan_minibatches.argtypes = [vp, i64, i64, i64, vp, i64, i64, vp, i64, vp, vp, vp, vp, vp, vp, vp, vp]
     L.merlin_tower_window_conv3_bits.argtypes = [vp, i64, vp, vp, i64, vp, i32, vp, vp, vp, vp]
     L.merlin_tower_window_conv3_reuse.argtypes = [vp, i64, vp, vp, i64, vp, i32, vp, vp, vp, vp, i32, vp]
     L.merlin_tower_all_windows.restype = i64
@@ -261,6 +271,8 @@
     "merlin_env_set_levels", "merlin_env_set_level_cdf", "merlin_env_levels", "merlin_env_set_level_log",
     "merlin_level_draw_host",
     "merlin_level_scores", "merlin_level_scores_host",
+    "merlin_plan_minibatches_workspace", "merlin_plan_minibatches", "merlin_plan_sort_workspace",
+    "merlin_plan_frames", "merlin_plan_windows", "merlin_plan_patches", "merlin_plan_bands", "merlin_plan_dq",
 )
 
 
@@ -987,6 +999,107 @@
                                             ptr(kmap), ptr(rmap), ptr(rep_row), stream_of(group_keys)),
           "merlin_minibatch_patch_maps")
     return kmap, rep_row
+
+
+class PlanWorkspace:
+
+    def __init__(self):
+        self.buf = None
+
+    def get(self, nbytes: int, device) -> torch.Tensor:
+        if self.buf is None or self.buf.device != device or self.buf.numel() < nbytes:
+            self.buf = None
+            self.buf = torch.empty(int(nbytes), dtype=torch.uint8, device=device)
+        return self.buf
+
+
+WINDOW_KEYS = 5 ** 9
+
+
+class PlanLists:
+
+    def __init__(self, codes, mult, workspace: PlanWorkspace):
+        assert codes.dtype == torch.int32 and codes.dim() == 2 and codes.shape[1] == OBS_WORDS
+        self.codes, self.ws, self.dev = codes.contiguous(), workspace, codes.device
+        self.B = B = int(codes.shape[0])
+        e = lambda shape, dt: torch.empty(shape, dtype=dt, device=self.dev)
+        self.uid, self.rep = e(B, torch.int64), e(B, torch.int64)
+        self.wkey, self.pkey = e((B, 25), torch.int32), e((B, 9), torch.int64)
+        self.mark, self.wrank = e(WINDOW_KEYS, torch.int32), e(WINDOW_KEYS, torch.int32)
+        self.counts = e(8, torch.int64)
+        m = (C.c_uint64 * 8)(*[int(x) & (2 ** 64 - 1) for x in mult])
+        ws = self._scratch(B, 8)
+        check(lib().merlin_plan_frames(ptr(self.codes), B, m, ptr(ws), ws.numel(), ptr(self.uid), ptr(self.rep),
+                                       ptr(self.wkey), ptr(self.pkey), ptr(self.mark), ptr(self.wrank),
+                                       ptr(self.counts), stream_of(codes)), "merlin_plan_frames")
+
+    def _scratch(self, n, key_bytes):
+        nbytes = int(lib().merlin_plan_sort_workspace(int(n), key_bytes))
+        if nbytes < 0:
+            check(E_INVALID, "merlin_plan_sort_workspace")
+        return self.ws.get(nbytes, self.dev)
+
+    def _list(self, n, L):
+        nitems = (n + L - 1) // L
+        e = lambda shape: torch.empty(shape, dtype=torch.int32, device=self.dev)
+        return e(n), e(n), e((nitems, 4)), e(nitems)
+
+    def windows(self, F, nw, L):
+        wid, rows = (torch.empty((F, 25), dtype=torch.int32, device=self.dev),
+                     torch.empty((nw, 16), dtype=torch.int32, device=self.dev))
+        lst = self._list(nw * 16, L)
+        ws = self._scratch(nw * 16, 4)
+        check(lib().merlin_plan_windows(F, nw, ptr(self.wkey), ptr(self.mark), ptr(self.wrank), LUT2_ROWS, L, ptr(ws),
+                                        ws.numel(), ptr(wid), ptr(rows), *map(ptr, lst), ptr(self.counts),
+                                        stream_of(self.codes)), "merlin_plan_windows")
+        return wid, rows, lst
+
+    def patches(self, F, L):
+        kid = torch.empty((F, 9), dtype=torch.int32, device=self.dev)
+        self.pk = torch.empty(F * 9, dtype=torch.int64, device=self.dev)
+        lst = self._list(F * 9, L)
+        ws = self._scratch(F * 9, 8)
+        check(lib().merlin_plan_patches(F, ptr(self.pkey), L, ptr(ws), ws.numel(), ptr(kid), ptr(self.pk),
+                                        *map(ptr, lst), ptr(self.counts), stream_of(self.codes)),
+              "merlin_plan_patches")
+        return kid, lst
+
+    def bands(self, K, L):
+        self.ub = torch.empty(K * 3, dtype=torch.int64, device=self.dev)
+        lst = self._list(K * 3, L)
+        ws = self._scratch(K * 3, 8)
+        check(lib().merlin_plan_bands(K, ptr(self.pk), L, ptr(ws), ws.numel(), ptr(self.ub), *map(ptr, lst),
+                                      ptr(self.counts), stream_of(self.codes)), "merlin_plan_bands")
+        return lst
+
+    def dq(self, nb, nw, L):
+        lst = self._list(nb * 3, L)
+        ws = self._scratch(nb * 3, 4)
+        check(lib().merlin_plan_dq(nb, nw, ptr(self.ub), ptr(self.mark), ptr(self.wrank), L, ptr(ws), ws.numel(),
+                                   *map(ptr, lst), ptr(self.counts), stream_of(self.codes)), "merlin_plan_dq")
+        return lst
+
+
+def plan_minibatches(idxs, period, minibatch_size, uid, num_frames, workspace: PlanWorkspace):
+    n, P, mbs, F = int(idxs.numel()), int(period), int(minibatch_size), int(num_frames)
+    assert idxs.dtype == torch.int64 and uid.dtype == torch.int64 and idxs.dim() == 1 and uid.dim() == 1
+    dev = idxs.device
+    nbytes = int(lib().merlin_plan_minibatches_workspace(n, P, mbs, F))
+    if nbytes < 0:
+        check(E_INVALID, "merlin_plan_minibatches_workspace")
+    ws = workspace.get(nbytes, dev)
+    nmb = (n // P) * ((P + mbs - 1) // mbs)
+    gkey = torch.empty(n, dtype=torch.int64, device=dev)
+    groups = torch.empty(n, dtype=torch.int64, device=dev)
+    inv = torch.empty(n, dtype=torch.int64, device=dev)
+    slot = torch.empty((nmb, F), dtype=torch.int32, device=dev)
+    order = torch.empty(n, dtype=torch.int32, device=dev)
+    offs = torch.empty(n + nmb, dtype=torch.int32, device=dev)
+    goff = torch.empty(nmb + 2, dtype=torch.int64, device=dev)
+    check(lib().merlin_plan_minibatches(ptr(idxs), n, P, mbs, ptr(uid), int(uid.numel()), F, ptr(ws), ws.numel(),
+                                        ptr(gkey), ptr(groups), ptr(inv), ptr(slot), ptr(order), ptr(offs), ptr(goff),
+                                        stream_of(idxs)), "merlin_plan_minibatches")
+    return gkey, groups, inv, slot, order, offs, goff
 
 
 def window_conv3_copy_masks(Y3, bits, rep_row):
diff --git a/ppo-2dgrid_amd/merlin/ppo.py b/ppo-2dgrid_amd/merlin/ppo.py
--- a/ppo-2dgrid_amd/merlin/ppo.py
+++ b/ppo-2dgrid_amd/merlin/ppo.py
@@ -435,15 +435,16 @@
         use_codes = codes is not None and self.conv1_from_codes
         groups = plan = None
         if use_codes and self.dedup:
+            from . import windows as W
             from .dedup import FrameGroups
 
-            groups = FrameGroups(codes)
+            native = self.windows and W.NATIVE_PLAN and codes.is_cuda
+            groups, plan = W.WindowPlan.native(codes) if native else (FrameGroups(codes), None)
             if not groups.ok:
                 groups = None
             elif self.windows:
-                from .windows import WindowPlan
-
-                plan = WindowPlan(codes, groups)
+                if plan is None:
+                    plan = W.WindowPlan(codes, groups)
                 self.last_num_windows = plan.num_windows
         distinct = 0
         host_mb = []
diff --git a/ppo-2dgrid_amd/merlin/windows.py b/ppo-2dgrid_amd/merlin/windows.py
--- a/ppo-2dgrid_amd/merlin/windows.py
+++ b/ppo-2dgrid_amd/merlin/windows.py
@@ -1,6 +1,7 @@
 from __future__ import annotations
 
 import contextlib
+import os
 import threading
 
 import torch
@@ -157,6 +158,28 @@
         if self._lazy is not None:
             self._derive()
         return self._offs
+
+
+class _BulkViews:
+
+    _NAMES = ("groups", "inv", "slot", "order", "offs", "kmap", "rep_row", "n_reps")
+
+    def __init__(self, arrays, m, g0, c, lo, hi):
+        self._cut = (arrays, m, g0, c, lo, hi)
+
+    def __getattr__(self, name):
+        if name not in _BulkViews._NAMES:
+            raise AttributeError(name)
+        (gall, inv, slot, order, offs, kmap, rep_row, n_reps), m, g0, c, lo, hi = self._cut
+        self.groups, self.inv, self.slot = gall[g0:g0 + c], inv[lo:hi], slot[m]
+        self.order, self.offs = order[lo:hi], offs[g0 + m:g0 + m + c + 1]
+        self.kmap, self.rep_row = kmap[m], rep_row[g0 * 9:(g0 + c) * 9]
+        self.n_reps = n_reps[m] if n_reps is not None else None
+        return self.__dict__[name]
+
+
+NATIVE_PLAN = os.environ.get("MERLIN_NATIVE_PLAN", "1") != "0"
+_PLAN_WORKSPACE = nat.PlanWorkspace()
 
 
 def _frame_csr(starts: torch.Tensor, n: int) -> torch.Tensor:
@@ -208,11 +231,76 @@
         dk, do = torch.sort(torch.cat(ddst).to(torch.int32), stable=True)
         self.dq_plan = SegmentPlan(dk, torch.cat(dsrc)[do], item_len)
 
+    @classmethod
+    def native(cls, codes: torch.Tensor, item_len: int | None = None, hist_item_len: int | None = None):
+        from . import dedup
+
+        pl = nat.PlanLists(codes, dedup._MULT, _PLAN_WORKSPACE)
+        F, bad, nw = pl.counts.tolist()[:3]
+        fg = dedup.FrameGroups.__new__(dedup.FrameGroups)
+        fg.uid, fg.rep, fg.num_groups, fg.ok = pl.uid, pl.rep[:F], F, not bad
+        if bad:
+            return fg, None
+
+        def L(n, given):
+            return auto_item_len(n) if given is None else int(given)
+
+        def seg(n, item, lst):
+            sp = SegmentPlan.__new__(SegmentPlan)
+            sp.nnz, sp.item_len, sp.nitems = n, item, (n + item - 1) // item
+            sp.key, sp.idx, sp.fix, sp.head_fix = lst
+            sp.counters = torch.zeros(sp.nitems, dtype=torch.int32, device=codes.device)
+            return sp
+
+        plan = cls.__new__(cls)
+        plan.frame_groups, plan.num_frames, plan.num_windows = fg, F, nw
+        Lh = L(16 * nw, hist_item_len)
+        plan.wid, plan.rows, hist = pl.windows(F, nw, Lh)
+        Lp = L(9 * F, item_len)
+        plan.kid, patch = pl.patches(F, Lp)
+        c = pl.counts.tolist()
+        assert not c[3], "a window reads a conv2 table row past LUT2_ROWS"
+        K = plan.num_patches = c[4]
+        Lb = L(3 * K, item_len)
+        band = pl.bands(K, Lb)
+        nb = plan.num_bands = pl.counts.tolist()[5]
+        Ld = L(3 * nb, item_len)
+        dq = pl.dq(nb, nw, Ld)
+        plan.hist, plan.patch_plan = seg(16 * nw, Lh, hist), seg(9 * F, Lp, patch)
+        plan.band_plan, plan.dq_plan = seg(3 * K, Lb, band), seg(3 * nb, Ld, dq)
+        plan.native_counts = pl.counts
+        return fg, plan
+
     def update_minibatches(self, perms: list, minibatch_size: int, bulk: bool = False) -> list:
         B = int(perms[0].numel())
-        flat = self.epoch_minibatches(torch.cat(perms), minibatch_size, period=B, bulk=bulk)
         nmb = (B + minibatch_size - 1) // minibatch_size
+        if (bulk and NATIVE_PLAN and perms[0].is_cuda and B * len(perms) < 2 ** 31
+                and nmb * len(perms) * self.num_frames < 2 ** 31):
+            flat = self._native_minibatches(torch.cat(perms), minibatch_size, B)
+        else:
+            flat = self.epoch_minibatches(torch.cat(perms), minibatch_size, period=B, bulk=bulk)
         return [flat[e * nmb:(e + 1) * nmb] for e in range(len(perms))]
+
+    def _native_minibatches(self, idxs: torch.Tensor, minibatch_size: int, P: int) -> list:
+        F, K = self.num_frames, self.num_patches
+        uid = self.frame_groups.uid
+        gkey, gall, inv, slot, order, offs, goff = nat.plan_minibatches(idxs.contiguous(), P, minibatch_size,
+                                                                        uid.long().contiguous(), F, _PLAN_WORKSPACE)
+        goff_h = goff.tolist()
+        nmb = len(goff_h) - 2
+        if goff_h[nmb + 1]:
+            raise nat.MerlinNativeError("merlin_plan_minibatches: a sample index or a frame id is out of range")
+        G = goff_h[nmb]
+        kmap, rep_row = nat.minibatch_patch_maps(self.kid, gkey[:G], F, goff, nmb, K)
+        n_reps = (kmap >= 0).sum(dim=1) if nat.KernelTimer.active() else None
+        arrays = (gall, inv, slot, order, offs, kmap, rep_row, n_reps)
+        per = (P + minibatch_size - 1) // minibatch_size
+        out = []
+        for m in range(nmb):
+            e, k = divmod(m, per)
+            out.append(_BulkViews(arrays, m, goff_h[m], goff_h[m + 1] - goff_h[m], e * P + k * minibatch_size,
+                                  e * P + min(P, (k + 1) * minibatch_size)))
+        return out
 
     def _bulk_minibatches(self, uniq, inv, perm, starts, mb_of, counts, P, per, minibatch_size) -> list:
         dev, F, K = uniq.device, self.num_frames, self.num_patches
```
